# burritojustice/reporter

Measured on AMD Instinct MI355X. Metric: GPS points matched/sec (whole node) at 1/2/4/8 MI355X; % segment-ID agreement vs meili, higher is better.
Workload: dtype f32

## Files before the change

### reporter_amd/csrc/engine.cpp

```cpp
#include "engine.h"

#include "flush.h"

#include <algorithm>
#include <chrono>
#include <cmath>
#include <cstdlib>

#include <cstring>

namespace otm {

#define HIPCHK(x)                                                              \
  do {                                                                         \
    hipError_t e_ = (x);                                                       \
    if (e_ != hipSuccess) {                                                    \
      *err = std::string(#x) + ": " + hipGetErrorString(e_);                   \
      return OTM_EDEVICE;                                                      \
    }                                                                          \
  } while (0)

#define TRY(x)                    \
  do {                            \
    if (int rc_ = (x)) return rc_; \
// ... 374 lines not shown
  HIPCHK(hipMemcpyAsync(cnt.data(), row_cnt, (size_t)N * 4, hipMemcpyDeviceToHost, s));
  HIPCHK(hipStreamSynchronize(s));
  E->graph_allocs.push_back(rows_b.release());
  E->graph_allocs.push_back(slot_b.release());
  E->graph_allocs.push_back(src_b.release());
  for (int32_t c : cnt) {
    out.incomplete += c < 0;
    out.entries += c > 0 ? c : 0;
  }
  out.slots = total;
  out.X.rmax = *r;
  out.X.cmax = index_cost_bound(*r);
  out.X.row = rows;
  out.X.src = src;
  out.src_bytes = (int64_t)E->g.n_edges * (int64_t)sizeof(SrcRec);
  out.X.slot = slot;
  out.X.load_pct = pct;
  return OTM_OK;
}

size_t index_budget() {
  if (const char* bm = std::getenv("OTM_INDEX_BUDGET_MB")) return (size_t)std::strtoull(bm, nullptr, 0) << 20;
  size_t fr = 0, tot = 0;
  if (hipMemGetInfo(&fr, &tot) != hipSuccess) return 0;
  return fr / 2;
}
}

int build_index(otm_engine* E, std::string* err) {
  E->idx = DevIndex{};
  for (auto& x : E->idxn) x = DevIndex{};
  E->idx.rmax = 0.0f;
  if (E->index_rmax < 0.0f) E->index_rmax = auto_index_radius(E);
  E->index_rmax = std::min(E->index_rmax, INDEX_RMAX_CAP);
  if (!(E->index_rmax > 0.0f)) return OTM_OK;
  hipStream_t s = E->stream;
  hipEvent_t a, z;
  HIPCHK(hipEventCreate(&a));
  HIPCHK(hipEventCreate(&z));
  HIPCHK(hipEventRecord(a, s));
  IndexBuilt full;
  TRY(build_index_at(E, &E->index_rmax, true, index_budget(), full, err));
  E->idx = full.X;
  E->index_entries = full.entries;
  E->index_slots = full.slots;
  E->index_src_bytes = full.src_bytes;
  E->index_incomplete_rows = full.incomplete;
  std::vector<float> radii;
  if (E->index_near_set) {
    radii = E->index_near_m;
  } else if ((double)full.slots * IDX_SLOT_BYTES >= OTM_INDEX_NEAR_MIN_GB * 1e9) {
    for (float f : std::initializer_list<float> OTM_INDEX_NEAR_FRACS) radii.push_back(E->index_rmax * f);
  }
  for (float& r : radii) r = (float)(std::floor(r / 50.0) * 50.0);
  std::sort(radii.begin(), radii.end());
  radii.erase(std::unique(radii.begin(), radii.end()), radii.end());
  int nl = 0;
  for (float rn : radii) {
    if (nl == NEAR_LEVELS || !(E->idx.rmax > 0.0f) || rn < 100.0f || rn >= E->idx.rmax) continue;
    IndexBuilt near;
    TRY(build_index_at(E, &rn, false, index_budget(), near, err));
    if (rn > 0.0f) {
      E->index_near_level_entries[nl] = near.entries;
      E->index_near_slots += near.slots;
      E->index_src_bytes += near.src_bytes;
      E->idxn[nl++] = near.X;
    }
  }
  HIPCHK(hipEventRecord(z, s));
  HIPCHK(hipEventSynchronize(z));
  HIPCHK(hipEventElapsedTime(&E->index_build_ms, a, z));
  (void)hipEventDestroy(a);
  (void)hipEventDestroy(z);
  return OTM_OK;
}

void engine_free(otm_engine* E) {
  if (E->device >= 0) (void)hipSetDevice(E->device);
  for (void* p : E->graph_allocs) (void)hipFree(p);
  E->graph_allocs.clear();
  pairs_drop(E);
  if (E->win_counts) (void)hipFree(E->win_counts);
  if (E->win_sums) (void)hipFree(E->win_sums);
  E->win_counts = E->win_sums = nullptr;
  E->win_open = false;
  if (E->sync_ev) (void)hipEventDestroy(E->sync_ev);
  E->sync_ev = nullptr;
  for (hipEvent_t ev : E->req_ev) (void)hipEventDestroy(ev);
  E->req_ev.clear();
  if (E->req_copy) (void)hipStreamDestroy(E->req_copy);
  E->req_copy = nullptr;
  for (auto& e : E->kev) {
    if (e) (void)hipEventDestroy(e);
    e = nullptr;
  }
  if (E->stream) (void)hipStreamDestroy(E->stream);
  E->stream = nullptr;
}

static int max_log2(const char* env, int dflt) {
  const char* v = std::getenv(env);
  return v ? std::min(dflt, std::atoi(v)) : dflt;
}


static int ensure_cand(otm_engine* E, DevWork& w, std::string* err) {
  const size_t n = E->cand_log2 > 0 ? (size_t)CAND_BIG_SLOTS << E->cand_log2 : 0;
  w.cand_final = E->cand_final;
  w.cand_log2 = E->cand_log2;
  TRY(bind_grow(w.cbig_key, E->cbig_key, n, err));
  TRY(bind_grow(w.cbig_val, E->cbig_val, n, err));
  TRY(bind_grow(w.cbig_skey, E->cbig_skey, n / 2, err));
  return OTM_OK;
}

static int ensure_huge(otm_engine* E, DevWork& w, std::string* err) {
  const size_t n = E->huge_log2 > 0 ? (size_t)HUGE_SLOTS << E->huge_log2 : 0;
  w.huge_log2 = E->huge_log2;
  w.huge_final = E->huge_final;
  TRY(bind_grow(w.huge_key, E->huge_key, n, err));
  TRY(bind_grow(w.huge_lab, E->huge_lab, n, err));
  TRY(bind_grow(w.huge_inq, E->huge_inq, n, err));
  TRY(bind_grow(w.huge_fr, E->huge_fr, n * 2, err));
  TRY(bind_grow(w.huge_ins, E->huge_ins, n ? (size_t)HUGE_SLOTS * huge_limit(E->huge_log2) : 0, err));
  TRY(bind_grow(w.huge_prev, E->huge_prev, n ? (size_t)HUGE_SLOTS : 0, err));
  if (n && E->huge_ready_log2 != E->huge_log2) {
    E->huge_ready_log2 = E->huge_log2;
    HIPCHK(hipMemsetAsync(w.huge_key, 0xFF, n * sizeof *w.huge_key, E->stream));
    HIPCHK(hipMemsetAsync(w.huge_lab, 0xFF, n * sizeof *w.huge_lab, E->stream));
    HIPCHK(hipMemsetAsync(w.huge_inq, 0, n * sizeof *w.huge_inq, E->stream));
    HIPCHK(hipMemsetAsync(w.huge_prev, 0xFF, (size_t)HUGE_SLOTS * sizeof *w.huge_prev, E->stream));
  }
  return OTM_OK;
}

static int ensure_big(otm_engine* E, DevWork& w, std::string* err) {
  const size_t n = (size_t)BIG_SLOTS * BIG_TABLE_CAP;
  bool fresh;
  TRY(bind_buf(w.big_key, E->big_key, n, err));
  TRY(bind_buf(w.big_lab, E->big_lab, n, err));
  TRY(bind_buf(w.big_inq, E->big_inq, n, err));
  TRY(bind_buf(w.big_fr, E->big_fr, n * 2, err));
  TRY(bind_buf(w.big_ins, E->big_ins, (size_t)BIG_SLOTS * SEARCH_LIMIT, err));
  TRY(bind_buf(w.big_prev, E->big_prev, (size_t)BIG_SLOTS, err, &fresh));
  if (fresh) {
    HIPCHK(hipMemsetAsync(w.big_key, 0xFF, n * sizeof *w.big_key, E->stream));
    HIPCHK(hipMemsetAsync(w.big_lab, 0xFF, n * sizeof *w.big_lab, E->stream));
    HIPCHK(hipMemsetAsync(w.big_inq, 0, n * sizeof *w.big_inq, E->stream));
    HIPCHK(hipMemsetAsync(w.big_prev, 0, (size_t)BIG_SLOTS * sizeof *w.big_prev, E->stream));
  }
  return OTM_OK;
}

static int bind_point_work(otm_engine* E, int64_t NP, int32_t NT, DevWork& w, std::string* err) {
  const size_t Pn = (size_t)NP + 1;
  TRY(bind_buf(w.pt_trace, E->pt_trace, Pn, err));
  TRY(bind_buf(w.is_col, E->is_col, Pn, err));
  TRY(bind_buf(w.prevc, E->prevc, Pn, err));
  TRY(bind_buf(w.nextc, E->nextc, Pn, err));
  TRY(bind_buf(w.gc, E->gc, Pn, err));
  TRY(bind_buf(w.ncand, E->ncand, Pn, err));
  TRY(bind_buf(w.cand_eo, E->cand_eo, Pn * KIN, err));
  TRY(bind_buf(w.cand_em, E->cand_em, Pn * KIN, err));
  TRY(bind_buf(w.cand_xeo, E->cand_xeo, Pn * KX, err));
  TRY(bind_buf(w.cand_xem, E->cand_xem, Pn * KX, err));
  TRY(bind_buf(w.probe, E->probe, Pn, err));
  TRY(bind_buf(w.col_prev, E->col_prev, Pn, err));
  TRY(bind_buf(w.kq_prev, E->kq_prev, Pn, err));
  TRY(bind_buf(w.vmeta, E->vmeta, Pn, err));
  TRY(bind_buf(w.colrec, E->colrec, Pn, err));
  TRY(bind_buf(w.colrec_pos, E->colrec_pos, Pn, err));
  TRY(bind_buf(w.trans_off, E->trans_off, Pn, err));
  TRY(bind_buf(w.bp, E->bp, Pn * KMAX, err));
  TRY(bind_buf(w.state, E->state, Pn, err));
  TRY(bind_buf(w.chosen, E->chosen, Pn, err));
  TRY(bind_buf(w.chain_start, E->chain_start, Pn, err));
  TRY(bind_buf(w.route_dist, E->route_dist, Pn, err));
  TRY(bind_buf(w.ipos, E->ipos, Pn, err));
  TRY(bind_buf(w.path_off, E->path_off, Pn, err));
  TRY(bind_buf(w.path_len, E->path_len, Pn, err));
  TRY(bind_buf(w.trace_err, E->trace_err, (size_t)NT + 1, err));
  TRY(bind_buf(w.spill_list1, E->spill_list1, Pn, err));
  TRY(bind_buf(w.spill_list2, E->spill_list2, Pn, err));
  TRY(bind_buf(w.spill_list3, E->spill_list3, Pn, err));
  TRY(bind_buf(w.counters_i32, E->counters_i32, CTR_WORDS, err));
  TRY(E->snap.ensure(1, err));
  w.snap = &E->snap.p->stage[0][0];
  TRY(bind_buf(w.abort, E->abort_flag, 4, err));
  if (!E->caps_read) {
    E->caps_read = true;
    if (const char* v = std::getenv("OTM_TRANS_CAP")) E->trans_cap = std::max<int64_t>(1, std::atoll(v)), E->caps_pinned = true;
    if (const char* v = std::getenv("OTM_POOL_CAP")) E->pool_cap = (int32_t)std::max(1, std::atoi(v)), E->caps_pinned = true;
  }
  if (!E->caps_pinned) {
    E->trans_cap = std::max<int64_t>(E->trans_cap, (int64_t)Pn * 48 + 4096);
    E->pool_cap = std::max<int32_t>(E->pool_cap, (int32_t)std::min<size_t>(Pn * 8, (size_t)1 << 30));
  }
  TRY(E->scan_tmp.ensure(scan_tmp_bytes(NP > NT ? NP : NT) + 256, err));
  TRY(bind_buf(w.path_pool, E->path_pool, (size_t)E->pool_cap, err));
  w.pool_cap = E->pool_cap;
  w.idx = E->idx;
  for (int l = 0; l < NEAR_LEVELS; ++l) w.idxn[l] = E->idxn[l];
  return OTM_OK;
}

static int bind_order(otm_engine* E, int64_t NP, bool ordered, DevOrder& ord, std::string* err) {
  const size_t Pn = (size_t)NP + 1;
  TRY(bind_buf(ord.tile, E->ord_tile, Pn, err));
  TRY(bind_buf(ord.tile_cnt, E->ord_cnt, ORDER_TILES, err));
  TRY(bind_buf(ord.cursor, E->ord_cursor, ORDER_TILES, err));
  TRY(bind_buf(ord.grp, E->ord_grp, ORDER_GROUPS + 1, err));
  TRY(bind_buf(ord.item, E->ord_item, Pn, err));
  if (!ordered) ord.tile_cnt = nullptr;
  return OTM_OK;
}

static int bind_trans(otm_engine* E, DevWork& w, hipStream_t s, std::string* err) {
  bool fresh;
  TRY(bind_buf(w.trans, E->trans, (size_t)E->trans_cap + 1, err, &fresh));
  if (fresh) HIPCHK(hipMemsetAsync(E->trans.p, 0, E->trans.bytes(), s));
  w.trans_cap = E->trans_cap;
  return OTM_OK;
}

static size_t out_region_cap(const otm_engine* E, int64_t NP) { return 2 * (size_t)NP + (size_t)E->pool_cap + 1; }

static int bind_out(otm_engine* E, int32_t NT, int64_t NP, DevOut& o, std::string* err) {
  const size_t Tn = (size_t)NT + 1, cap = out_region_cap(E, NP);
  TRY(bind_buf(o.traces, E->o_traces, Tn, err));
  TRY(bind_buf(o.seg_cnt, E->o_seg_cnt, Tn, err));
  TRY(bind_buf(o.way_cnt, E->o_way_cnt, Tn, err));
  TRY(bind_buf(o.seg_base, E->seg_ub, Tn, err));
  TRY(bind_buf(o.segments, E->o_segments, cap, err));
  TRY(bind_buf(o.seg_gidx, E->o_seg_gidx, cap, err));
  TRY(bind_buf(o.reports, E->o_reports, cap, err));
  TRY(bind_buf(o.way_ids, E->o_way_ids, cap, err));
  TRY(bind_buf(o.rep_cnt, E->o_rep_cnt, Tn, err));
  return OTM_OK;
}

static int bind_trav(otm_engine* E, int32_t NT, int64_t NP, DevTrav& tv, std::string* err) {
  TRY(bind_buf(tv.rec, E->tv_rec, out_region_cap(E, NP), err));
  TRY(bind_buf(tv.cnt, E->tv_cnt, (size_t)NT + 1, err));
  return OTM_OK;
}

static int bind_scores(otm_engine* E, int32_t NT, int64_t NP, DevScores& sc, std::string* err) {
  const size_t Pn = (size_t)NP + 1;
  TRY(bind_buf(sc.rec, E->scores.dev, Pn, err));
  TRY(bind_buf(sc.alpha, E->sc_alpha, Pn * KIN, err));
  TRY(bind_buf(sc.alpha_x, E->sc_alpha_x, Pn * KX, err));
  TRY(bind_buf(sc.rej, E->sc_rej, (size_t)NT + 2, err));
  sc.rej_n = sc.rej + NT + 1;
  return OTM_OK;
}

static int engine_match_once(otm_engine* E, const DevBatch& b, hipStream_t s, std::string* err,
                             int from = RESUME_ALL) {
  const int64_t NP = b.n_points;
  const int32_t NT = b.n_traces;
  end_records(E, REC_BATCH_BEGINS);
  DevWork w{};
  TRY(bind_point_work(E, NP, NT, w, err));

  DevParams dp = E->dp;
  if (NP < E->small_points) {
    dp.order_mask = 0;
    dp.cand_wave_all = 1;
  }
  {
    const char* ce = std::getenv("OTM_CAND_CHUNK");
    const int ch = ce ? std::atoi(ce) : 64;
    dp.cand_chunk = ch < 1 ? 1 : (ch > 64 ? 64 : ch);
  }
  w.ctr = E->counting ? E->ctr.p : nullptr;
  if (E->counting && from == RESUME_ALL) HIPCHK(hipMemsetAsync(E->ctr.p, 0, sizeof(DevCounters), s));
  Marks mk;
  mk.ev = E->timing ? E->kev : nullptr;
  TRY(bind_order(E, NP, dp.order_mask != 0, w.ord, err));
  if (from == RESUME_ALL) {
    launch_columns(E->g, b, dp, w, s, mk);
    if (dp.order_mask) {
      launch_order(b, w, s, mk);
    } else if (E->timing) {
      mk.begin(KN_ORDER, s);
      mk.end(KN_ORDER, s);
    }
  }
  TRY(ensure_cand(E, w, err));
  if (from <= RESUME_CAND_BIG) launch_candidates(E->g, b, dp, w, s, mk, from);
  if (from <= RESUME_CAND_BIG) {
    launch_links(b, dp, w, s, mk);
    mk.begin(KN_SCAN_TRANS, s);
    scan_i64(w.trans_off, NP, E->scan_tmp.p, E->scan_tmp.cap(), s);
    mk.end(KN_SCAN_TRANS, s);
  }
  TRY(bind_trans(E, w, s, err));
  TRY(ensure_big(E, w, err));
  TRY(ensure_huge(E, w, err));
  if (from <= RESUME_TRANS_HUGE) launch_transitions(E->g, b, dp, w, s, mk, E->trans_lanes, from);
  if (from <= RESUME_TRANS_HUGE) launch_viterbi(b, w, s, mk);
  launch_route(E->g, b, dp, w, s, mk, from);

  if (out_region_cap(E, NP) >= (size_t)INT32_MAX) {
    *err = "batch too large for one launch (segment regions exceed 2^31)";
    return OTM_EINVAL;
  }
  DevOut o{};
  TRY(bind_out(E, NT, NP, o, err));
  {
    otm_engine* H = E->parent ? const_cast<otm_engine*>(E->parent) : E;
    std::lock_guard<std::mutex> lk(H->hist_mu);
    o.hist = H->hist;
    o.speed_sum = H->speed_sum;
    o.nbins = H->nbins;
    o.bin_kph = H->bin_kph;
    o.pairs = H->pairs_tab;
  }
  HIPCHK(hipMemsetAsync(o.seg_base, 0, ((size_t)NT + 1) * sizeof *o.seg_base, s));
  launch_seg_bound(E->g, b, dp, w, o.seg_base, s, mk);
  mk.begin(KN_SEG_SCAN, s);
  scan_i64(o.seg_base, NT, E->scan_tmp.p, E->scan_tmp.cap(), s);
  mk.end(KN_SEG_SCAN, s);
  launch_segments(E->g, b, w, o, s, mk);
  if (E->queue_kph > 0.0f) launch_queue(b, w, o, E->queue_kph, s);
  end_records(E, REC_BATCH_OUTPUTS);
  if (records_wanted(E, E->points)) {
    TRY(E->points.dev.ensure((size_t)NP + 1, err));
    launch_points(E->g, b, dp, w, E->points.dev.p, s);
    E->points.n = NP;
  }
  if (records_wanted(E, E->scores)) {
    DevScores sc{};
    TRY(bind_scores(E, NT, NP, sc, err));
    launch_scores(b, w, sc, s);
    E->scores.n = NP;
  }
  const bool for_route = records_wanted(E, E->route), for_shape = records_wanted(E, E->shape);
  if (for_route || for_shape) {
    DevTrav tv{};
    TRY(bind_trav(E, NT, NP, tv, err));
    HIPCHK(hipMemsetAsync(tv.cnt + NT, 0, sizeof *tv.cnt, s));
    launch_traversals(E->g, b, w, o, tv, s);
    if (for_route) E->tv_T = NT;
    if (for_shape) E->sh_T = NT;
  }
  launch_report(b, E->drc, w, o, s, mk);
  HIPCHK(hipGetLastError());
  E->last_T = NT;
  E->last_P = NP;
  E->last_S = -1;
  E->last_W = -1;
  return OTM_OK;
}

int engine_match(otm_engine* E, const DevBatch& b, hipStream_t s, std::string* err) {
  if (!s) s = E->stream;
  const int64_t NP = b.n_points;
  struct OomGuard {
    otm_engine* E;
    bool huge = false, cand = false;
    ~OomGuard() {
      if (huge) E->huge_final = 0;
      if (cand) E->cand_final = 0;
    }
  } oom{E};
  struct FailGuard {
    otm_engine* E;
    bool ok = false;
    ~FailGuard() {
      if (!ok) end_records(E, REC_BATCH_FAILED);
    }
  } failed{E};
  int from = RESUME_ALL;
  DevWork grown{};
  E->last_resumes = 0;
  for (int attempt = 0;; ++attempt) {
    TRY(engine_match_once(E, b, s, err, from));
    TRY(E->h_status.ensure(1, err));
    BatchStatus* dst = &E->snap.p->status;
    launch_status(E->abort_flag.p, E->trans_off.p + NP, E->counters_i32.p, dst, s);
    HIPCHK(hipMemcpyAsync(E->h_status.p, dst, sizeof(BatchStatus), hipMemcpyDeviceToHost, s));
    HIPCHK(wait_batch(E, s, NP));
    const BatchStatus st = *E->h_status.p;
    const int32_t ab = st.abort;
    const int64_t ttotal = st.ttotal;
    E->last_trans = ttotal;
    E->last_attempts = attempt + 1;
    if (!ab) break;
    if (attempt == 16) {
      *err = "batch capacities could not be sized";
      return OTM_EDEVICE;
    }
    if (ttotal > E->trans_cap) E->trans_cap = ttotal + ttotal / 4 + 4096;
    if (st.grow & GROW_HUGE) {
      const int32_t next = E->huge_log2 ? E->huge_log2 + 2 : 19;
      const int32_t prev = E->huge_log2;
      if (next > max_log2("OTM_HUGE_MAX_LOG2", HUGE_MAX_LOG2)) {
        E->huge_final = 1;
      } else {
        E->huge_log2 = next;
        if (ensure_huge(E, grown, err) != OTM_OK) {
          E->huge_log2 = prev;
          E->huge_final = 1;
          oom.huge = true;
          E->huge_ready_log2 = 0;
          err->clear();
        }
      }
    }
    if (st.grow & GROW_CAND) {
      const int32_t next = E->cand_log2 ? E->cand_log2 + 2 : 13;
      const int32_t prev = E->cand_log2;
      if (next > max_log2("OTM_CAND_MAX_LOG2", CAND_MAX_LOG2)) {
        E->cand_final = 1;
      } else {
        E->cand_log2 = next;
        if (ensure_cand(E, grown, err) != OTM_OK) {
          E->cand_log2 = prev;
          E->cand_final = 1;
          oom.cand = true;
          err->clear();
        }
      }
    }
    if (st.pool_over)
      E->pool_cap = (int32_t)std::min<size_t>((size_t)st.pool_used * 2 + 1024, (size_t)INT32_MAX / 2);
    const char* nr = std::getenv("OTM_NO_RESUME");
    const bool whole = ttotal > E->trans_cap || st.pool_over || !(st.grow & (GROW_HUGE | GROW_CAND)) ||
                       (nr && *nr && *nr != '0');
    from = whole ? RESUME_ALL
                 : (st.grow & GROW_CAND) ? RESUME_CAND_BIG : (st.route_huge ? RESUME_ROUTE_HUGE : RESUME_TRANS_HUGE);
    if (from != RESUME_ALL) {
      const SnapId snap = from == RESUME_CAND_BIG ? SNAP_AFTER_CAND
                                                  : (from == RESUME_TRANS_HUGE ? SNAP_AFTER_TRANS : SNAP_AFTER_ROUTE);
      int32_t* ctr = E->counters_i32.p;
      HIPCHK(hipMemcpyAsync(ctr, E->snap.p->stage[snap], CTR_STAGE_WORDS * sizeof(int32_t),
                            hipMemcpyDeviceToDevice, s));
      HIPCHK(hipMemsetAsync(ctr + CTR_GROW_HUGE, 0, 4, s));
      HIPCHK(hipMemsetAsync(ctr + CTR_GROW_CAND, 0, 4, s));
      HIPCHK(hipMemsetAsync(E->abort_flag.p, 0, 4, s));
      E->last_resumes += 1;
    }
  }
  if (E->timing) {
    HIPCHK(hipEventSynchronize(E->kev[2 * KN_REPORT + 1]));
    for (int k = 0; k < KN_COUNT; ++k)
      HIPCHK(hipEventElapsedTime(&E->kernel_ms[k], E->kev[2 * k], E->kev[2 * k + 1]));
    const int first[8] = {KN_COLUMNS, KN_ORDER, KN_LINKS, KN_TRANS_INDEX, KN_VITERBI, KN_ROUTE_INDEX, KN_SEG_BOUND,
                          KN_SEG_WRITE};
    const int last[8] = {KN_COLUMNS, KN_CAND_WAVE, KN_SCAN_TRANS, KN_TRANS_GLOBAL, KN_VITERBI, KN_ROUTE_GLOBAL,
                         KN_SEG_SCAN, KN_REPORT};
    for (int k = 0; k < 8; ++k) {
      E->stage_ms[k] = 0.0f;
      for (int q = first[k]; q <= last[k]; ++q) E->stage_ms[k] += E->kernel_ms[q];
    }
  }
  failed.ok = true;
  return OTM_OK;
}

static hipError_t big_copy(void* dst, const void* src, size_t n, hipMemcpyKind k, hipStream_t s) {
  return hipMemcpyAsync(dst, src, n, k, s);
}

static int validate_offsets(int32_t NT, const int64_t* trace_off, int64_t n_points, std::string* err) {
  const int64_t NP = trace_off[NT];
  if (trace_off[0] != 0 || NP < 0 || (n_points && n_points != NP)) {
    *err = "batch trace_off inconsistent with n_points";
    return OTM_EINVAL;
  }
  for (int32_t t = 0; t < NT; ++t)
    if (trace_off[t + 1] < trace_off[t]) {
      *err = "batch trace_off not monotonic";
      return OTM_EINVAL;
    }
  return OTM_OK;
}

int engine_match_host(otm_engine* E, const otm_batch* in, std::string* err) {
  const int32_t NT = in->n_traces;
  if (NT < 0 || !in->trace_off) {
    *err = "invalid batch";
    return OTM_EINVAL;
  }
  TRY(validate_offsets(NT, in->trace_off, in->n_points, err));
  const int64_t NP = in->trace_off[NT];
  DevBatch b;
  b.n_traces = NT;
  b.n_points = NP;
  TRY(bind_buf(b.trace_off, E->in_off, (size_t)NT + 1, err));
  TRY(bind_buf(b.lat, E->in_lat, (size_t)NP, err));
  TRY(bind_buf(b.lon, E->in_lon, (size_t)NP, err));
  TRY(bind_buf(b.time, E->in_time, (size_t)NP, err));
  TRY(bind_buf(b.acc, E->in_acc, (size_t)NP, err));
  hipStream_t s = E->stream;
  const size_t b_off = ((size_t)NT + 1) * 8, b_pt = (size_t)NP * 4, b_tm = (size_t)NP * 8;
  if (NP <= (int64_t)1 << 18) {
    const size_t total = b_off + b_tm + 3 * b_pt;
    TRY(E->h_in.ensure(total, err));
    TRY(E->in_blob.ensure(total, err));
    char* h = E->h_in.p;
    std::memcpy(h, in->trace_off, b_off);
    if (NP) {
      std::memcpy(h + b_off, in->time, b_tm);
      std::memcpy(h + b_off + b_tm, in->lat, b_pt);
      std::memcpy(h + b_off + b_tm + b_pt, in->lon, b_pt);
      std::memcpy(h + b_off + b_tm + 2 * b_pt, in->accuracy, b_pt);
    }
    HIPCHK(hipMemcpyAsync(E->in_blob.p, h, total, hipMemcpyHostToDevice, s));
    const char* d = E->in_blob.p;
    b.trace_off = (const int64_t*)d;
    b.time = (const double*)(d + b_off);
    b.lat = (const float*)(d + b_off + b_tm);
    b.lon = (const float*)(d + b_off + b_tm + b_pt);
    b.acc = (const float*)(d + b_off + b_tm + 2 * b_pt);
    return engine_match(E, b, s, err);
  }
  const hipMemcpyKind h2d = hipMemcpyHostToDevice;
  HIPCHK(hipMemcpyAsync(E->in_off.p, in->trace_off, b_off, hipMemcpyHostToDevice, s));
  HIPCHK(big_copy(E->in_lat.p, in->lat, b_pt, h2d, s));
  HIPCHK(big_copy(E->in_lon.p, in->lon, b_pt, h2d, s));
  HIPCHK(big_copy(E->in_time.p, in->time, b_tm, h2d, s));
  HIPCHK(big_copy(E->in_acc.p, in->accuracy, b_pt, h2d, s));
  return engine_match(E, b, s, err);
}

int validate_compact(const otm_batch_compact* in, int64_t* np, std::string* err) {
  const int32_t NT = in->n_traces;
  if (NT < 0 || !in->trace_off || (NT > 0 && !in->time_base)) {
    *err = "invalid batch";
    return OTM_EINVAL;
  }
  TRY(validate_offsets(NT, in->trace_off, in->n_points, err));
  const int64_t NP = in->trace_off[NT];
// ... 232 lines not shown
  TRY(E->f_traces.ensure((size_t)NT + 1, err));
  if (NT) {
    DevOut o{};
    TRY(bind_out(E, NT, E->last_P, o, err));
    launch_compact(NT, o, so, wo, ro, E->f_segs.p, E->f_ways.p, E->f_reps.p, E->f_traces.p, s);
    HIPCHK(hipGetLastError());
  }
  E->last_S = NS;
  E->last_W = NW;
  *NS_ = NS;
  *NW_ = NW;
  *NR_ = NR;
  return OTM_OK;
}

int engine_fetch(otm_engine* E, otm_results* out, std::string* err) {
  hipStream_t s = E->stream;
  const int32_t NT = E->last_T;
  int32_t NS, NW, NR;
  TRY(fetch_compact(E, &NS, &NW, &NR, err));
  TRY(bind_buf(out->traces, E->h_traces, (size_t)NT + 1, err));
  TRY(bind_buf(out->segments, E->h_segs, (size_t)NS + 1, err));
  TRY(bind_buf(out->reports, E->h_reps_dense, (size_t)NR + 1, err));
  TRY(bind_buf(out->way_ids, E->h_ways, (size_t)NW + 1, err));
  const hipMemcpyKind d2h = hipMemcpyDeviceToHost;
  hipStream_t c = s;
  if (NT) HIPCHK(big_copy(E->h_traces.p, E->f_traces.p, (size_t)NT * sizeof(otm_trace_result), d2h, c));
  if (NS) HIPCHK(big_copy(E->h_segs.p, E->f_segs.p, (size_t)NS * sizeof(otm_segment), d2h, c));
  if (NR) HIPCHK(big_copy(E->h_reps_dense.p, E->f_reps.p, (size_t)NR * sizeof(otm_report_rec), d2h, c));
  if (NW) HIPCHK(big_copy(E->h_ways.p, E->f_ways.p, (size_t)NW * 8, d2h, c));
  HIPCHK(wait_batch(E, c, E->last_P));
  out->n_traces = NT;
  out->n_segments = NS;
  out->n_reports = NR;
  out->n_way_ids = NW;
  return OTM_OK;
}

int engine_write_responses(otm_engine* E, const int64_t** off, const uint8_t** host,
                           const otm_trace_result** traces, int64_t* total, std::string* err) {
  hipStream_t s = E->stream;
  const int32_t NT = E->last_T;
  int32_t NS, NW, NR;
  TRY(fetch_compact(E, &NS, &NW, &NR, err));
  const size_t hdr_b = (size_t)NT * RESP_HDR_SLOT + 64, seg_b = resp_seg_scratch(NS, NW),
               rep_b = (size_t)NR * RESP_REP_SLOT + 64;
  RespWork w{};
  TRY(bind_buf(w.hdr, E->resp_hdr, hdr_b, err));
  TRY(bind_buf(w.seg, E->resp_seg, seg_b, err));
  TRY(bind_buf(w.rep, E->resp_rep, rep_b, err));
  TRY(bind_buf(w.hlen, E->resp_hlen, (size_t)NT + 1, err));
  TRY(bind_buf(w.slen, E->resp_slen, (size_t)NS + 1, err));
  TRY(bind_buf(w.rlen, E->resp_rlen, (size_t)NR + 1, err));
  TRY(bind_buf(w.blen, E->resp_blen, (size_t)NT + 1, err));
  TRY(bind_buf(w.host, E->resp_host, (size_t)NT + 1, err));
  const size_t blob_b = hdr_b + seg_b + rep_b + (size_t)NT * 97 + (size_t)NS + (size_t)NR;
  TRY(E->resp_blob.ensure(blob_b, err));
  TRY(E->scan_tmp.ensure(scan_tmp_bytes(NT) + 256, err));
  const RespIn in{NT, NS, NR, E->f_traces.p, E->f_segs.p, E->f_ways.p, E->f_reps.p};
  if (NT) {
    launch_resp_items(in, w, s);
    launch_resp_len(in, w, s);
    scan_i64(w.blen, NT, E->scan_tmp.p, E->scan_tmp.cap(), s);
    launch_resp_copy(in, w, w.blen, E->resp_blob.p, s);
  }
  const size_t off_b = ((size_t)NT + 1) * 8;
  TRY(E->h_resp_meta.ensure(off_b + (size_t)NT + 8, err));
  TRY(bind_buf(*traces, E->h_traces, (size_t)NT + 1, err));
  char* meta = E->h_resp_meta.p;
  std::memset(meta, 0, off_b);
  if (NT) {
    HIPCHK(hipMemcpyAsync(meta, w.blen, off_b, hipMemcpyDeviceToHost, s));
    HIPCHK(hipMemcpyAsync(meta + off_b, w.host, (size_t)NT, hipMemcpyDeviceToHost, s));
    HIPCHK(big_copy(E->h_traces.p, E->f_traces.p, (size_t)NT * sizeof(otm_trace_result), hipMemcpyDeviceToHost, s));
  }
  HIPCHK(hipGetLastError());
  HIPCHK(wait_batch(E, s, E->last_P));
  *total = ((const int64_t*)meta)[NT];
  *off = (const int64_t*)meta;
  *host = (const uint8_t*)(meta + off_b);
  return OTM_OK;
}

int engine_copy_responses(otm_engine* E, char* dst, int64_t total, const char** blob, std::string* err) {
  if (!dst) {
    TRY(E->h_resp.ensure((size_t)total + 16, err));
    dst = E->h_resp.p;
  }
  if (total) {
    HIPCHK(big_copy(dst, E->resp_blob.p, (size_t)total, hipMemcpyDeviceToHost, E->stream));
    HIPCHK(wait_batch(E, E->stream, E->last_P));
  }
  *blob = dst;
  return OTM_OK;
}

int engine_report_segments(otm_engine* E, int32_t T, const int64_t* trace_off, const double* time,
                           const int32_t* seg_off, const otm_segment* segs, otm_trace_result* traces,
                           otm_report_rec* reports, std::string* err) {
  const int64_t NP = trace_off[T];
  const int32_t NS = seg_off[T];
  for (int32_t t = 0; t < T; ++t)
    if (trace_off[t + 1] <= trace_off[t]) {
      *err = "every trace needs at least one point (its end time)";
      return OTM_EINVAL;
    }
  const size_t b_off = ((size_t)T + 1) * 8, b_sb = ((size_t)T + 1) * 8, b_tm = (size_t)NP * 8;
  const size_t b_seg = ((size_t)NS + 1) * sizeof(otm_segment), b_cnt = ((size_t)T + 1) * 4;
  const size_t b_gidx = ((size_t)NS + 1) * 4, b_err = b_cnt, b_ab = 16;
  const size_t b_tr = ((size_t)T + 1) * sizeof(otm_trace_result), b_rep = ((size_t)NS + 1) * sizeof(otm_report_rec);
  size_t off[12];
  size_t tot = 0;
  const size_t sz[11] = {b_off, b_sb, b_tm, b_seg, b_cnt, b_gidx, b_err, b_ab, b_tr, b_rep, b_cnt};
  for (int k = 0; k < 11; ++k) {
    off[k] = tot;
    tot += (sz[k] + 255) & ~(size_t)255;
  }
  off[11] = tot;
  TRY(E->rs_blob.ensure(tot, err));
  std::vector<char> h(off[8], 0);
  std::memcpy(h.data() + off[0], trace_off, b_off);
  int64_t* sb = (int64_t*)(h.data() + off[1]);
  int32_t* cnt = (int32_t*)(h.data() + off[4]);
  for (int32_t t = 0; t < T; ++t) {
    sb[t] = seg_off[t];
    cnt[t] = seg_off[t + 1] - seg_off[t];
  }
  if (NP) std::memcpy(h.data() + off[2], time, b_tm);
  if (NS) std::memcpy(h.data() + off[3], segs, (size_t)NS * sizeof(otm_segment));
  int32_t* gidx = (int32_t*)(h.data() + off[5]);
  for (int32_t k = 0; k < NS; ++k) gidx[k] = -1;
  hipStream_t s = E->stream;
  char* d = E->rs_blob.p;
  HIPCHK(hipMemcpyAsync(d, h.data(), off[8], hipMemcpyHostToDevice, s));
  DevBatch b{};
  b.n_traces = T;
  b.n_points = NP;
  b.trace_off = (const int64_t*)(d + off[0]);
  b.time = (const double*)(d + off[2]);
  DevWork w{};
  w.trace_err = (int32_t*)(d + off[6]);
  w.abort = (int32_t*)(d + off[7]);
  w.ctr = nullptr;
  DevOut o{};
  o.traces = (otm_trace_result*)(d + off[8]);
  o.seg_cnt = (int32_t*)(d + off[4]);
  o.rep_cnt = (int32_t*)(d + off[10]);
  o.seg_base = (int64_t*)(d + off[1]);
  o.segments = (otm_segment*)(d + off[3]);
  o.seg_gidx = (int32_t*)(d + off[5]);
  o.reports = (otm_report_rec*)(d + off[9]);
  o.hist = nullptr;
  o.speed_sum = nullptr;
  launch_report(b, E->drc, w, o, s, Marks{});
  HIPCHK(hipGetLastError());
  if (T) HIPCHK(hipMemcpyAsync(traces, d + off[8], (size_t)T * sizeof(otm_trace_result), hipMemcpyDeviceToHost, s));
  if (NS) HIPCHK(hipMemcpyAsync(reports, d + off[9], (size_t)NS * sizeof(otm_report_rec), hipMemcpyDeviceToHost, s));
  HIPCHK(hipStreamSynchronize(s));
  return OTM_OK;
}

int engine_debug_fetch(otm_engine* E, int what, void* dst, size_t bytes, size_t* needed, std::string* err) {
  const size_t Pn = (size_t)E->last_P;
  const void* src = nullptr;
  size_t n = 0;
  auto of = [&](const auto& buf, size_t count) {
    src = buf.p;
    n = count * sizeof(*buf.p);
  };
  switch (what) {
    case 0: of(E->ncand, Pn); break;
    case 1:
    case 2:
    case 3: {
      n = Pn * KMAX * 4;
      if (needed) *needed = n;
      if (!dst) return OTM_OK;
      if (bytes < n) {
        *err = "debug buffer too small";
        return OTM_EINVAL;
      }
      if (!n) return OTM_OK;
      const bool rec = what != 3;
      const size_t el = rec ? sizeof(*E->cand_eo.p) : sizeof(*E->cand_em.p);
      std::vector<char> in(Pn * KIN * el), ov(Pn * KX * el);
      const void *din = E->cand_em.p, *dov = E->cand_xem.p;
      if (rec) din = E->cand_eo.p, dov = E->cand_xeo.p;
      HIPCHK(hipMemcpyAsync(in.data(), din, in.size(), hipMemcpyDeviceToHost, E->stream));
      HIPCHK(hipMemcpyAsync(ov.data(), dov, ov.size(), hipMemcpyDeviceToHost, E->stream));
      HIPCHK(hipStreamSynchronize(E->stream));
      int32_t* d = (int32_t*)dst;
      for (size_t p = 0; p < Pn; ++p)
        for (int j = 0; j < KMAX; ++j) {
          const int32_t* src = j < KIN ? (const int32_t*)in.data() + (rec ? 2 : 1) * (p * KIN + j)
                                       : (const int32_t*)ov.data() + (rec ? 2 : 1) * (p * KX + (j - KIN));
          d[p * KMAX + j] = rec ? src[what - 1] : src[0];
        }
      return OTM_OK;
    }
    case 4: of(E->trans_off, Pn + 1); break;
    case 5: of(E->trans, (size_t)E->last_trans); break;
    case 6: of(E->state, Pn); break;
    case 7: of(E->col_prev, Pn); break;
    case 8: of(E->route_dist, Pn); break;
    case 9: of(E->gc, Pn); break;
    case 10: of(E->ipos, Pn); break;
    case 11: of(E->in_off, (size_t)E->last_T + 1); break;
    case 12: of(E->in_lat, Pn); break;
    case 13: of(E->in_lon, Pn); break;
    case 14: of(E->in_time, Pn); break;
    case 15: of(E->in_acc, Pn); break;
    case 16: of(E->chain_start, Pn); break;
    case 17: of(E->is_col, Pn); break;
    case 18: {
      int32_t total = 0;
      if (E->ord_grp.p && E->ord_item.p) {
        HIPCHK(hipMemcpyAsync(&total, E->ord_grp.p + ORDER_GROUPS, 4, hipMemcpyDeviceToHost, E->stream));
        HIPCHK(hipStreamSynchronize(E->stream));
      }
      of(E->ord_item, total < 0 || (size_t)total > Pn ? 0 : (size_t)total);
      break;
    }
    case 19: of(E->ord_tile, E->ord_tile.p ? Pn : 0); break;
    case 20: of(E->ord_grp, E->ord_grp.p ? ORDER_GROUPS + 1 : 0); break;
    default: *err = "unknown debug buffer"; return OTM_EINVAL;
  }
  if (needed) *needed = n;
  if (!dst) return OTM_OK;
  if (bytes < n) {
    *err = "debug buffer too small";
    return OTM_EINVAL;
  }
  if (n) HIPCHK(hipMemcpyAsync(dst, src, n, hipMemcpyDeviceToHost, E->stream));
  HIPCHK(hipStreamSynchronize(E->stream));
  return OTM_OK;
}

template <class Rec>
static void end_if(BatchRecords<Rec>& r, RecEvent event) {
  if (kRecDesc<Rec>.ends & event) r.n = r.joined_n = -1;
}

void end_records(otm_engine* E, RecEvent event) {
  end_if(E->points, event);
  end_if(E->route, event);
  end_if(E->scores, event);
  end_if(E->shape, event);
  if (kRecDesc<otm_traversal>.ends & event) E->tv_T = E->tv_off_T = -1;
  if (kRecDesc<otm_shape_vertex>.ends & event) E->sh_T = -1;
}

template <class Rec>
int engine_fetch_records(otm_engine* E, BatchRecords<Rec>& r, Rec* dst, int64_t cap, int64_t* n, std::string* err) {
  constexpr const RecDesc& d = kRecDesc<Rec>;
  if (!r.on) {
    *err = d.off;
    return OTM_EINVAL;
  }
  if (r.n < 0) {
    *err = d.none;
    return OTM_EINVAL;
  }
  if (n) *n = r.n;
  if (!dst && cap == 0) return OTM_OK;
  if (!dst || cap < r.n) {
    *err = d.cap;
    return OTM_EINVAL;
  }
  const size_t bytes = (size_t)r.n * sizeof(Rec);
  if (!bytes) return OTM_OK;
  TRY(r.pin.ensure((size_t)r.n, err));
  HIPCHK(big_copy(r.pin.p, r.dev.p, bytes, hipMemcpyDeviceToHost, E->stream));
  HIPCHK(wait_batch(E, E->stream, r.n));
  std::memcpy(dst, r.pin.p, bytes);
  return OTM_OK;
}
template int engine_fetch_records(otm_engine*, BatchRecords<otm_matched_point>&, otm_matched_point*, int64_t, int64_t*,
                                  std::string*);
template int engine_fetch_records(otm_engine*, BatchRecords<otm_traversal>&, otm_traversal*, int64_t, int64_t*,
                                  std::string*);
template int engine_fetch_records(otm_engine*, BatchRecords<otm_point_score>&, otm_point_score*, int64_t, int64_t*,
                                  std::string*);

static int trav_offsets(otm_engine* E, int32_t NT, std::string* err, bool wait = true) {
  if (E->tv_off_T == NT) return OTM_OK;
  hipStream_t s = E->stream;
  TRY(E->tv_off.ensure((size_t)NT + 1, err));
  TRY(E->h_tv_off.ensure((size_t)NT + 1, err));
  HIPCHK(hipMemcpyAsync(E->tv_off.p, E->tv_cnt.p, ((size_t)NT + 1) * 8, hipMemcpyDeviceToDevice, s));
  if (NT) scan_i64(E->tv_off.p, NT, E->scan_tmp.p, E->scan_tmp.cap(), s);
  HIPCHK(hipMemcpyAsync(E->h_tv_off.p, E->tv_off.p, ((size_t)NT + 1) * 8, hipMemcpyDeviceToHost, s));
  if (!wait) return OTM_OK;
  HIPCHK(wait_batch(E, s, E->last_P));
  E->tv_off_T = NT;
  return OTM_OK;
}

int engine_traversals_dense(otm_engine* E, std::string* err) {
  if (!E->route.on) {
    *err = kRecDesc<otm_traversal>.off;
    return OTM_EINVAL;
  }
  if (E->tv_T < 0) {
    *err = kRecDesc<otm_traversal>.none;
    return OTM_EINVAL;
  }
  if (E->route.n >= 0) return OTM_OK;
// ... 678 lines not shown
```

### reporter_amd/csrc/kernels.h

```cpp
#pragma once
#include <hip/hip_runtime.h>

#include <cstddef>
#include <cstdint>

#include "otmatch.h"
#include "pairs.h"

namespace otm {

constexpr int KMAX = 32;
constexpr int KIN = 8;
static_assert(KIN == 4 || KIN == 8, "inline blocks of 4 or 8 slots (whole 16-B emission pieces)");
constexpr int KX = KMAX - KIN;
constexpr int MAX_HITS = 256;
constexpr int SEARCH_LIMIT = 98304;
constexpr int LDS_TABLE_CAP = 256;
constexpr int LDS_TABLE_LIMIT = 192;
constexpr int BIG_TABLE_LOG2 = 17;
constexpr int BIG_TABLE_CAP = 1 << BIG_TABLE_LOG2;
#ifndef OTM_BIG_SLOTS
#define OTM_BIG_SLOTS 512
#endif
constexpr int BIG_SLOTS = OTM_BIG_SLOTS;
// ... 10 lines not shown
  const int32_t* e_shape_off;
  const int64_t* e_way;
  const int32_t *e_seg, *e_seg_pos;
  const uint8_t* e_flags;
  const float *s_lat, *s_lon, *s_cum;
  const uint64_t* g_id;
  const float* g_len;
  const uint32_t* cell_off;
  const uint32_t* cell_ent;
  const float4* ent_geo;
  const uint16_t *e_head_out, *e_head_in;
  const uint32_t* e_len64;
  const uint4* e_rec;
  const int2* e_fl;
  const int4* e_proj;
  const float4* s_pt;
  const int64_t* way_tab;
  int32_t n_nodes, n_edges, n_segments, grid_rows, grid_cols;
  double lat0, lon0, cell;
  float bb_lat0, bb_lon0, bb_inv_h, bb_inv_w;
};

#ifndef OTM_ORDER_BITS
#define OTM_ORDER_BITS 6
#endif
constexpr int ORDER_BITS = OTM_ORDER_BITS;
constexpr int ORDER_SIDE = 1 << ORDER_BITS;
constexpr int ORDER_TILES = ORDER_SIDE * ORDER_SIDE;
constexpr int ORDER_GROUPS = 8;
struct DevOrder {
  int32_t* item;
  int32_t* grp;
  uint16_t* tile;
  int32_t* tile_cnt;
  int32_t* cursor;
};

struct IdxRow {
  int64_t off;
  int32_t cnt;
  uint32_t cap;
};
#ifndef OTM_SRC_REC_BYTES
#define OTM_SRC_REC_BYTES 48
#endif
struct alignas(16) SrcRec {
  IdxRow edge;
  IdxRow node;
  int32_t from;
  int32_t len;
  int32_t pad[(OTM_SRC_REC_BYTES - 40) / 4];
};
static_assert(sizeof(SrcRec) == OTM_SRC_REC_BYTES && (OTM_SRC_REC_BYTES == 48 || OTM_SRC_REC_BYTES == 64),
              "source records of 48 or 64 bytes");
struct DevIndex {
  float rmax;
  uint32_t cmax;
  const IdxRow* row;
  const SrcRec* src;
  const uint4* slot;
  int load_pct;
};
constexpr int IDX_SLOT_BYTES = 16;
constexpr float INDEX_RMAX_CAP = 200000.0f;
constexpr uint32_t NODE_KEY = 0x80000000u;
constexpr uint32_t NONE_PRED = 0xFFFFFFFFu;
constexpr int NEAR_LEVELS = 3;
#ifndef OTM_INDEX_NEAR_FRACS
#define OTM_INDEX_NEAR_FRACS {0.45f}
#endif
#ifndef OTM_INDEX_NEAR_MIN_GB
#define OTM_INDEX_NEAR_MIN_GB 16.0
#endif
constexpr int INDEX_BUILD_LOG2 = 11;
constexpr int INDEX_BUILD_CAP = 1 << INDEX_BUILD_LOG2;
constexpr int INDEX_BUILD_LIMIT = 1536;
__host__ __device__ inline uint32_t index_cost_bound(float B) { return (uint32_t)floor((double)B * 64.0); }

constexpr int ORDER_CAND = 1, ORDER_TRANS = 2, ORDER_ROUTE = 4;
constexpr int TURN_TABLE = 181;
constexpr uint32_t TURN_UNITS_MAX = 0xFFFFFFu;
constexpr uint32_t NO_TURNS = 0xFFFFFFFFu;
struct DevParams {
  float sigma_z, beta, factor, breakage, interp, search_radius, max_search_radius, gps_accuracy;
  const uint32_t* turn_units;
  int max_candidates;
  int order_mask;
  int cand_wave_all;
  int cand_chunk;
};

struct DevReportCfg {
  int n_report, n_transition;
  int64_t report_levels[16];
  int64_t transition_levels[16];
  double threshold_sec;
};

struct DevBatch {
  int32_t n_traces;
  int64_t n_points;
  const int64_t* trace_off;
  const float *lat, *lon;
  const double* time;
  const float* acc;
};

struct DevCounters {
  unsigned long long points, columns, cells_visited, cell_entries_scanned, candidates;
  unsigned long long searches, nodes_settled, edges_relaxed, transitions;
  unsigned long long route_searches, route_nodes_settled, route_edges_relaxed, route_edges;
  unsigned long long segments_out, reports_out;
};

enum CtrSlot : int {
  CTR_UNUSED = 0,
  CTR_POOL_USED = 1,
  CTR_POOL_OVER = 2,
  CTR_SEARCH_GLOBAL = 3,
  CTR_INDEX_MISS = 4,
  CTR_CAND_WAVE = 5,
  CTR_TRANS_WIDE = 6,
  CTR_SEG_LARGE = 8,
  CTR_VIT_16 = 20,
  CTR_TRANS_HUGE = 21,
  CTR_ROUTE_HUGE = 22,
  CTR_GROW_HUGE = 23,
  CTR_CAND_BIG = 24,
  CTR_GROW_CAND = 25,
  CTR_VIT_WAVE = 26,
};
constexpr int CTR_STAGE_WORDS = 16;
constexpr int CTR_ZEROED_WORDS = 32;
constexpr int CTR_WORDS = 64;
enum SnapId : int { SNAP_AFTER_CAND = 0, SNAP_AFTER_TRANS = 1, SNAP_AFTER_ROUTE = 2, SNAP_COUNT = 3 };
constexpr int ctr_list(CtrSlot c) {
  switch (c) {
    case CTR_INDEX_MISS: case CTR_CAND_WAVE: case CTR_SEG_LARGE: case CTR_VIT_16: return 1;
    case CTR_SEARCH_GLOBAL: case CTR_TRANS_WIDE: case CTR_VIT_WAVE: return 2;
    case CTR_TRANS_HUGE: case CTR_ROUTE_HUGE: case CTR_CAND_BIG: return 3;
    default: return 0;
  }
}
constexpr bool ctr_per_stage(CtrSlot c) { return c >= 0 && c < CTR_STAGE_WORDS; }
constexpr bool ctr_per_batch(CtrSlot c) { return c >= CTR_STAGE_WORDS && c < CTR_ZEROED_WORDS; }
static_assert(ctr_per_stage(CTR_UNUSED) && ctr_per_stage(CTR_POOL_USED) && ctr_per_stage(CTR_POOL_OVER) &&
                  ctr_per_stage(CTR_SEARCH_GLOBAL) && ctr_per_stage(CTR_INDEX_MISS) && ctr_per_stage(CTR_CAND_WAVE) &&
                  ctr_per_stage(CTR_TRANS_WIDE) && ctr_per_stage(CTR_SEG_LARGE),
              "per-stage slots lie in the snapshot range");
static_assert(ctr_per_batch(CTR_VIT_16) && ctr_per_batch(CTR_TRANS_HUGE) && ctr_per_batch(CTR_ROUTE_HUGE) &&
                  ctr_per_batch(CTR_GROW_HUGE) && ctr_per_batch(CTR_CAND_BIG) && ctr_per_batch(CTR_GROW_CAND) &&
                  ctr_per_batch(CTR_VIT_WAVE),
              "per-batch slots lie past the snapshot range, within what K1 zeroes");

struct DevWork {
  int32_t* pt_trace;
  uint8_t* is_col;
  int32_t* prevc;
  int32_t* nextc;
  float* gc;
  int32_t* ncand;
  float4* probe;
  int2* cand_eo;
  float* cand_em;
  int2* cand_xeo;
  float* cand_xem;
  int32_t* col_prev;
  int32_t* kq_prev;
  uint8_t* vmeta;
  int64_t* trans_off;
  float* trans;
  uint8_t* bp;
  int32_t* state;
  int2* chosen;
  uint8_t* chain_start;
  float* route_dist;
  float* ipos;
  int32_t* path_off;
  int32_t* path_len;
  int32_t* path_pool;
  int32_t pool_cap;
  int32_t* trace_err;
  int32_t* spill_list1;
  int32_t* spill_list2;
  int32_t* snap;
  int32_t* counters_i32;
  int32_t* abort;
  int64_t trans_cap;
  int4* colrec;
  int32_t* colrec_pos;
  DevIndex idx;
  DevIndex idxn[NEAR_LEVELS];
  DevOrder ord;
  uint32_t* big_key;
  unsigned long long* big_lab;
  uint32_t* big_inq;
  uint32_t* big_fr;
  uint32_t* big_ins;
  int32_t* big_prev;
  uint32_t* huge_key;
  unsigned long long* huge_lab;
  uint32_t* huge_inq;
  uint32_t* huge_fr;
  uint32_t* huge_ins;
  int32_t* huge_prev;
  int32_t huge_log2;
  int32_t huge_final;
  uint32_t* cbig_key;
  unsigned long long* cbig_val;
  unsigned long long* cbig_skey;
  int32_t cand_log2;
  int32_t cand_final;
  int32_t* spill_list3;
  DevCounters* ctr;
};
struct SpillRef {
  int32_t* list;
  int32_t* count;
};
template <CtrSlot C>
__host__ __device__ __forceinline__ int32_t* spill_list(const DevWork& w) {
  constexpr int L = ctr_list(C);
  static_assert(L != 0, "this slot counts no list");
  return L == 1 ? w.spill_list1 : (L == 2 ? w.spill_list2 : w.spill_list3);
}
template <CtrSlot C>
__host__ __device__ __forceinline__ SpillRef spill_of(const DevWork& w) {
  return SpillRef{spill_list<C>(w), w.counters_i32 + C};
}

struct DevOut {
  otm_trace_result* traces;
  int32_t* seg_cnt;
  int32_t* way_cnt;
  int32_t* rep_cnt;
  int64_t* seg_base;
  otm_segment* segments;
  int32_t* seg_gidx;
  int64_t* way_ids;
  otm_report_rec* reports;
  uint32_t* hist;
  unsigned long long* speed_sum;
  int nbins;
  float bin_kph;
  PairTab pairs;
};

struct DevTrav {
  otm_traversal* rec;
  int64_t* cnt;
};

struct DevShape {
  const int64_t* trav_off;
  int64_t* vtx_off;
  int64_t* poly_off;
  otm_shape_vertex* vtx;
  otm_shape_span* span;
  char* poly;
};

enum KernelId {
  KN_COLUMNS,
  KN_ORDER,
  KN_CAND_LANE,
  KN_CAND_WAVE,
  KN_LINKS,
  KN_SCAN_TRANS,
  KN_TRANS_INDEX,
  KN_TRANS_WIDE,
  KN_TRANS_WAVE,
  KN_TRANS_GLOBAL,
  KN_VITERBI,
  KN_ROUTE_INDEX,
  KN_ROUTE_WAVE,
  KN_ROUTE_GLOBAL,
  KN_SEG_BOUND,
  KN_SEG_SCAN,
  KN_SEG_WRITE,
  KN_REPORT,
  KN_COUNT
};
extern const char* const kKernelNames[KN_COUNT];
struct Marks {
  hipEvent_t* ev = nullptr;
  void begin(int k, hipStream_t s) const {
    if (ev) (void)hipEventRecord(ev[2 * k], s);
  }
  void end(int k, hipStream_t s) const {
    if (ev) (void)hipEventRecord(ev[2 * k + 1], s);
  }
};

void launch_columns(const DevGraph& g, const DevBatch& b, const DevParams& p, DevWork& w, hipStream_t s,
                    const Marks& mk);
enum Resume { RESUME_ALL = 0, RESUME_CAND_BIG = 1, RESUME_TRANS_HUGE = 2, RESUME_ROUTE_HUGE = 3 };
void launch_candidates(const DevGraph& g, const DevBatch& b, const DevParams& p, DevWork& w, hipStream_t s,
                       const Marks& mk, int from = RESUME_ALL);
void launch_links(const DevBatch& b, const DevParams& p, DevWork& w, hipStream_t s, const Marks& mk);
void launch_transitions(const DevGraph& g, const DevBatch& b, const DevParams& p, DevWork& w, hipStream_t s,
                        const Marks& mk, int sub, int from = RESUME_ALL);
void launch_viterbi(const DevBatch& b, DevWork& w, hipStream_t s, const Marks& mk);
void launch_route(const DevGraph& g, const DevBatch& b, const DevParams& p, DevWork& w, hipStream_t s,
                  const Marks& mk, int from = RESUME_ALL);
void launch_segments(const DevGraph& g, const DevBatch& b, DevWork& w, DevOut& o, hipStream_t s, const Marks& mk);
void launch_queue(const DevBatch& b, DevWork& w, DevOut& o, float kph, hipStream_t s);
void launch_points(const DevGraph& g, const DevBatch& b, const DevParams& p, DevWork& w, otm_matched_point* out,
                   hipStream_t s);
void launch_traversals(const DevGraph& g, const DevBatch& b, DevWork& w, DevOut& o, const DevTrav& tv, hipStream_t s);
void launch_trav_compact(int32_t n_traces, const int64_t* seg_base, const int64_t* off, const otm_traversal* reg,
                         otm_traversal* dst, hipStream_t s);
struct DevScores {
  otm_point_score* rec;
  float* alpha;
  float* alpha_x;
  int32_t* rej;
  int32_t* rej_n;
};
void launch_scores(const DevBatch& b, DevWork& w, const DevScores& sc, hipStream_t s);
void launch_shape(const DevGraph& g, int32_t n_traces, const int64_t* seg_base, const DevTrav& tv, const DevShape& sh,
                  bool write, hipStream_t s);
void launch_report(const DevBatch& b, const DevReportCfg& rc, DevWork& w, DevOut& o, hipStream_t s, const Marks& mk);
void launch_order(const DevBatch& b, DevWork& w, hipStream_t s, const Marks& mk);
void launch_seg_bound(const DevGraph& g, const DevBatch& b, const DevParams& p, DevWork& w, int64_t* tb, hipStream_t s,
                      const Marks& mk);
void launch_compact(int32_t n_traces, const DevOut& o, const int32_t* seg_off, const int32_t* way_off,
                    const int32_t* rep_off, otm_segment* segs_out, int64_t* ways_out, otm_report_rec* reps_out,
                    otm_trace_result* traces_out,
                    hipStream_t s);
void launch_index_build(const DevGraph& g, const uint32_t* turn_units, uint32_t cmax, int32_t* row_cnt,
                        const IdxRow* rows, uint4* slot, bool write, hipStream_t s);
int index_load_fast();
int index_load_dense();
void launch_row_sizes(const int32_t* row_cnt, int64_t* row_sizes, int32_t n, int pct, hipStream_t s);
constexpr int32_t GROW_HUGE = 1, GROW_CAND = 2;
struct BatchStatus {
  int32_t abort, grow;
  int64_t ttotal;
  int32_t pool_used, pool_over;
  int32_t route_huge;
};
struct SnapBuf {
  int32_t stage[SNAP_COUNT][CTR_STAGE_WORDS];
  BatchStatus status;
};
static_assert(offsetof(SnapBuf, status) == 192 && sizeof(SnapBuf) == 192 + 32, "snapshot buffer layout");
void launch_expand_compact(const int64_t* trace_off, const int64_t* tbase, const int32_t* dt, const int16_t* acc16,
                           double* time, float* acc, int32_t n_traces, hipStream_t s);
void launch_status(const int32_t* abort, const int64_t* ttotal, const int32_t* counters, BatchStatus* out,
                   hipStream_t s);
void launch_row_pack(const int32_t* row_cnt, const int64_t* row_off, IdxRow* rows, int32_t n, hipStream_t s);
void launch_src_pack(const DevGraph& g, const IdxRow* rows, SrcRec* src, hipStream_t s);
size_t req_sparse_slots(int32_t n, size_t bytes);
void launch_req_read(const unsigned char* blob, const int64_t* off, int32_t r0, int32_t r1, int32_t n, int64_t* cnt,
                     uint8_t* ok, const DevBatch& sparse, hipStream_t s);
void launch_req_compact(const int64_t* off, int32_t n, const int64_t* pre, const uint8_t* ok, const DevBatch& sparse,
                        const DevBatch& out, int64_t* trace_off, hipStream_t s);
constexpr int RESP_HDR_SLOT = 512;
constexpr int RESP_SEG_SLOT = 320;
constexpr int RESP_REP_SLOT = 192;
struct RespIn {
  int32_t nt, ns, nr;
  const otm_trace_result* traces;
  const otm_segment* segs;
  const int64_t* ways;
  const otm_report_rec* reps;
};
struct RespWork {
  char *hdr, *seg, *rep;
  int32_t *hlen, *slen, *rlen;
  int64_t* blen;
  uint8_t* host;
};
size_t resp_seg_scratch(int32_t ns, int32_t nw);
void launch_resp_items(const RespIn& in, const RespWork& w, hipStream_t s);
void launch_resp_len(const RespIn& in, const RespWork& w, hipStream_t s);
void launch_resp_copy(const RespIn& in, const RespWork& w, const int64_t* boff, char* blob, hipStream_t s);
void scan_i64(int64_t* d, int64_t n, void* tmp, size_t tmp_bytes, hipStream_t s);
constexpr int FETCH_SCAN_MAX = 1 << 16;
void launch_fetch_scan(int32_t n, const int32_t* c0, const int32_t* c1, const int32_t* c2, int32_t* o0, int32_t* o1,
                       int32_t* o2, hipStream_t s);
void scan_i32(int32_t* d, int64_t n, void* tmp, size_t tmp_bytes, hipStream_t s);
size_t scan_tmp_bytes(int64_t n);

}
```

### reporter_amd/csrc/kernels.hip

```cpp
#include <hip/hip_runtime.h>

#include <algorithm>
#include <cstdlib>
#include <type_traits>

#include <hipcub/hipcub.hpp>

#include "kernels.h"
#include "otmatch.h"

namespace otm {

namespace {

#define MPD_F 111319.4954833f
constexpr uint32_t EMPTY = 0xFFFFFFFFu;
constexpr unsigned long long LAB_NONE = ~0ull;
constexpr int TB = 64;
__device__ __forceinline__ void wave_sync() {
  __builtin_amdgcn_wave_barrier();
  asm volatile("" ::: "memory");
}

__device__ __forceinline__ float cos_deg(float deg) {
// ... 127 lines not shown
  bool at_end;
  project(g, e, k, lat, lon, ls, sqd, off_out, at_end);
}
__device__ __forceinline__ float probe_radius(const DevParams& P, float acc) {
  const float a = acc > 0.0f ? acc : P.gps_accuracy;
  const float r = a > P.search_radius ? a : P.search_radius;
  return r < P.max_search_radius ? r : P.max_search_radius;
}

__device__ __forceinline__ uint32_t fbits(float f) { return __float_as_uint(f); }
__device__ __forceinline__ float bitsf(uint32_t u) { return __uint_as_float(u); }
__device__ __forceinline__ uint32_t hash32(uint32_t x) { return x * 2654435761u; }

__device__ __forceinline__ void cadd(unsigned long long* c, unsigned long long v) {
  if (c && v) atomicAdd(c, v);
}

__device__ __forceinline__ int2 crec(const DevWork& w, int64_t p, int j) {
  return j < KIN ? w.cand_eo[p * KIN + j] : w.cand_xeo[p * KX + (j - KIN)];
}
__device__ __forceinline__ float cemis(const DevWork& w, int64_t p, int j) {
  return j < KIN ? w.cand_em[p * KIN + j] : w.cand_xem[p * KX + (j - KIN)];
}
__device__ __forceinline__ void cput(const DevWork& w, int64_t p, int j, int32_t e, float off, float em) {
  if (j < KIN) {
    w.cand_eo[p * KIN + j] = make_int2(e, __float_as_int(off));
    w.cand_em[p * KIN + j] = em;
  } else {
    w.cand_xeo[p * KX + (j - KIN)] = make_int2(e, __float_as_int(off));
    w.cand_xem[p * KX + (j - KIN)] = em;
  }
}

__device__ __forceinline__ uint32_t turn_deg(uint32_t hin, uint32_t hout) {
  int d = (int)hout - (int)hin;
  d += d < 0 ? 360 : 0;
  return (uint32_t)(d <= 180 ? d : 360 - d);
}
__device__ __forceinline__ float trans_cost(uint32_t units, float r, float gcv, float beta) {
  units = units > TURN_UNITS_MAX ? TURN_UNITS_MAX : units;
  const float tc = (float)units * 0.015625f;
  const float diff = fabsf(r - gcv);
  return (tc + diff) / beta;
}

constexpr uint32_t NO_HEAD = 0xFFFFu;
__device__ __forceinline__ bool cand_node(float off) { return off == 0.0f; }
__device__ __forceinline__ int32_t src_node(const DevGraph& g, int32_t e, float off) {
  return cand_node(off) ? g.e_from[e] : g.e_to[e];
}
__device__ __forceinline__ float src_start(const DevGraph& g, int32_t e, float off) {
  return cand_node(off) ? 0.0f : g.e_len[e] - off;
}
__device__ __forceinline__ uint32_t src_head(const DevGraph& g, int32_t e, float off) {
  return cand_node(off) ? NO_HEAD : (uint32_t)g.e_head_in[e];
}
__device__ __forceinline__ uint32_t dst_head(const DevGraph& g, int32_t e, float off) {
  return cand_node(off) ? NO_HEAD : (uint32_t)g.e_head_out[e];
}
__device__ __forceinline__ bool same_edge_step(int32_t ei, float oi, int32_t ej, float oj) {
  return ei == ej && (oj >= oi || (!cand_node(oj) && !cand_node(oi)));
}
__device__ __forceinline__ float same_edge_dist(float oi, float oj) { return oj >= oi ? oj - oi : 0.0f; }
__device__ __forceinline__ uint32_t turn_units(const uint32_t* TU, uint32_t hin, uint32_t hout) {
  return (hin == NO_HEAD || hout == NO_HEAD) ? 0u : TU[turn_deg(hin, hout)];
}

__device__ __forceinline__ int wave_incl_scan(int v, int lane) {
#pragma unroll
  for (int o = 1; o < 64; o <<= 1) {
    int n = __shfl_up(v, o, 64);
    if (lane >= o) v += n;
  }
  return v;
}

__device__ __forceinline__ void fold_snap(DevWork& w, int k, bool reset) {
  for (int t = 0; t < CTR_STAGE_WORDS; ++t) {
    w.snap[CTR_STAGE_WORDS * k + t] = w.counters_i32[t];
    if (reset) w.counters_i32[t] = 0;
  }
}
template <CtrSlot C>
__device__ __forceinline__ void spill_push(const DevWork& w, int32_t p) {
  const SpillRef s = spill_of<C>(w);
  s.list[atomicAdd(s.count, 1)] = p;
}
__device__ __forceinline__ bool trans_over_cap(const DevBatch& b, const DevWork& w) {
  if (w.trans_off[b.n_points] <= w.trans_cap) return false;
  *w.abort = 1;
  return true;
}

__device__ __forceinline__ int hilbert_d(int x, int y) {
  int d = 0;
  for (int sft = ORDER_SIDE / 2; sft > 0; sft >>= 1) {
    const int rx = (x & sft) > 0;
    const int ry = (y & sft) > 0;
    d += sft * sft * ((3 * rx) ^ ry);
    if (ry == 0) {
      if (rx == 1) {
        x = ORDER_SIDE - 1 - x;
        y = ORDER_SIDE - 1 - y;
      }
      const int tmp = x;
      x = y;
      y = tmp;
    }
  }
  return d;
}

__device__ __forceinline__ int tile_of(const DevGraph& g, float lat, float lon) {
  int ty = (int)((lat - g.bb_lat0) * g.bb_inv_h);
  int tx = (int)((lon - g.bb_lon0) * g.bb_inv_w);
  ty = ty < 0 ? 0 : (ty >= ORDER_SIDE ? ORDER_SIDE - 1 : ty);
  tx = tx < 0 ? 0 : (tx >= ORDER_SIDE ? ORDER_SIDE - 1 : tx);
  return hilbert_d(tx, ty);
}

struct AggMatch {
  int leader;
  int rank;
  int count;
};
__device__ __forceinline__ AggMatch agg_match(int key, bool active) {
  const int lane = threadIdx.x & 63;
  unsigned long long pending = __ballot(active);
  AggMatch m{lane, 0, 0};
  while (pending) {
    const int leader = __ffsll((long long)pending) - 1;
    const int k = __shfl(key, leader, 64);
    const unsigned long long grp = __ballot(((pending >> lane) & 1ull) && key == k);
    if ((grp >> lane) & 1ull) {
      m.leader = leader;
      m.rank = (int)__popcll(grp & ((1ull << lane) - 1ull));
      m.count = (int)__popcll(grp);
    }
    pending &= ~grp;
  }
  return m;
}
__device__ __forceinline__ int wave_agg_slot(int32_t* ctr, int key, bool active) {
  const AggMatch m = agg_match(key, active);
  int base = 0;
  if (active && m.leader == (int)(threadIdx.x & 63)) base = atomicAdd(&ctr[key], m.count);
  return __shfl(base, m.leader, 64) + m.rank;
}
__device__ __forceinline__ void wave_agg_count(int32_t* ctr, int key, bool active) {
  const AggMatch m = agg_match(key, active);
  if (active && m.leader == (int)(threadIdx.x & 63)) atomicAdd(&ctr[key], m.count);
}

__global__ __launch_bounds__(1024) void k_order_plan(const int32_t* tile_cnt, int32_t* cursor, int32_t* grp) {
  __shared__ int32_t part[1024];
  __shared__ int32_t cut[ORDER_GROUPS + 1];
  constexpr int PER = ORDER_TILES / 1024;
  const int tid = threadIdx.x;
  int32_t v[PER], sum = 0;
  for (int k = 0; k < PER; ++k) {
    v[k] = tile_cnt[tid * PER + k];
    sum += v[k];
  }
  part[tid] = sum;
  if (tid <= ORDER_GROUPS) cut[tid] = 0x7fffffff;
  __syncthreads();
  for (int o = 1; o < 1024; o <<= 1) {
    const int32_t x = tid >= o ? part[tid - o] : 0;
    __syncthreads();
    part[tid] += x;
    __syncthreads();
  }
  const int32_t total = part[1023];
  int32_t run = part[tid] - sum;
  int32_t prev_start = tid == 0 ? -1 : run - tile_cnt[tid * PER - 1];
  for (int k = 0; k < PER; ++k) {
    cursor[tid * PER + k] = run;
    for (int gi = 1; gi < ORDER_GROUPS; ++gi) {
      const int64_t want = ((int64_t)total * gi + ORDER_GROUPS - 1) / ORDER_GROUPS;
      if (run >= want && prev_start < want) cut[gi] = run;
    }
    prev_start = run;
    run += v[k];
  }
  __syncthreads();
  if (tid == 0) {
    grp[0] = 0;
    int32_t prev = 0;
    for (int gi = 1; gi < ORDER_GROUPS; ++gi) {
      const int32_t c = cut[gi] > total ? total : cut[gi];
      prev = c > prev ? c : prev;
      grp[gi] = prev;
    }
    grp[ORDER_GROUPS] = total;
  }
}

__global__ __launch_bounds__(256) void k_order_scatter(DevBatch b, DevWork w, const uint16_t* tile, int32_t* cursor,
                                                       int32_t* item) {
  for (int64_t p0 = (int64_t)blockIdx.x * 256; p0 < b.n_points; p0 += (int64_t)gridDim.x * 256) {
    const int64_t p = p0 + threadIdx.x;
    const bool col = p < b.n_points && w.is_col[p];
    const int t = col ? (int)tile[p] : 0;
    const int pos = wave_agg_slot(cursor, t, col);
    if (col) item[pos] = (int32_t)p;
    if (col && w.colrec_pos) w.colrec_pos[p] = pos;
  }
}

#ifndef OTM_COL_PTS
#define OTM_COL_PTS 256
#endif
constexpr int COL_PTS = OTM_COL_PTS;
__global__ __launch_bounds__(TB) void k_columns(DevGraph g, DevBatch b, DevParams P, DevWork w) {
  __shared__ float sLat[COL_PTS], sLon[COL_PTS], sGc[COL_PTS];
  __shared__ int32_t sPrev[COL_PTS];
  __shared__ uint8_t sCol[COL_PTS];
  const int lane = threadIdx.x;
  if (blockIdx.x == 0) {
    if (lane < CTR_ZEROED_WORDS) w.counters_i32[lane] = 0;
    if (lane == 0) *w.abort = 0;
  }
  for (int32_t t = blockIdx.x; t < b.n_traces; t += gridDim.x) {
    const int64_t a = b.trace_off[t], e = b.trace_off[t + 1];
    const int n = (int)(e - a);
    int ncols = 0;
    if (n > COL_PTS) {
      if (lane == 0) {
        int64_t last = -1;
        for (int64_t p = a; p < e; ++p) {
          float gcv = 0.0f;
          if (last >= 0) gcv = gc_dist(b.lat[last], b.lon[last], b.lat[p], b.lon[p]);
          const bool col = last < 0 || gcv >= P.interp;
          w.is_col[p] = col ? 1 : 0;
          w.gc[p] = col ? gcv : 0.0f;
          w.prevc[p] = (int32_t)last;
          if (col) {
            last = p;
            ++ncols;
            if (w.ord.tile_cnt) {
              const int tl = tile_of(g, b.lat[p], b.lon[p]);
              w.ord.tile[p] = (uint16_t)tl;
              atomicAdd(&w.ord.tile_cnt[tl], 1);
            }
          }
        }
      }
      for (int64_t p = a + lane; p < e; p += TB) {
        w.probe[p] = make_float4(b.lat[p], b.lon[p], b.acc[p], 0.0f);
        w.pt_trace[p] = t;
        w.ncand[p] = 0;
        w.route_dist[p] = 0.0f;
        w.ipos[p] = -1.0f;
        w.nextc[p] = -1;
      }
    } else {
      for (int pl = lane; pl < n; pl += TB) {
        sLat[pl] = b.lat[a + pl];
        sLon[pl] = b.lon[a + pl];
      }
      __syncthreads();
      bool near = false;
      for (int pl = lane; pl < n; pl += TB) {
        const float d = pl > 0 ? gc_dist(sLat[pl - 1], sLon[pl - 1], sLat[pl], sLon[pl]) : 0.0f;
        sGc[pl] = d;
        near = near || (pl > 0 && !(d >= P.interp));
      }
      __syncthreads();
      if (__ballot(near) == 0ull) {
        for (int pl = lane; pl < n; pl += TB) {
          sCol[pl] = 1;
          sPrev[pl] = pl > 0 ? (int32_t)(a + pl - 1) : -1;
        }
        ncols = n;
      } else if (lane == 0) {
        int last = -1;
        for (int pl = 0; pl < n; ++pl) {
          float gcv = 0.0f;
          if (last >= 0) gcv = last == pl - 1 ? sGc[pl] : gc_dist(sLat[last], sLon[last], sLat[pl], sLon[pl]);
          const bool col = last < 0 || gcv >= P.interp;
          sCol[pl] = col ? 1 : 0;
          sGc[pl] = col ? gcv : 0.0f;
          sPrev[pl] = last >= 0 ? (int32_t)(a + last) : -1;
          if (col) {
            last = pl;
            ++ncols;
          }
        }
      }
      __syncthreads();
      for (int c0 = 0; c0 < n; c0 += TB) {
        const int pl = c0 + lane;
        const bool in = pl < n;
        const bool col = in && sCol[pl];
        if (in) {
          const int64_t p = a + pl;
          w.probe[p] = make_float4(sLat[pl], sLon[pl], b.acc[p], 0.0f);
          w.pt_trace[p] = t;
          w.is_col[p] = sCol[pl];
          w.gc[p] = sGc[pl];
          w.prevc[p] = sPrev[pl];
          w.ncand[p] = 0;
          w.route_dist[p] = 0.0f;
          w.ipos[p] = -1.0f;
          w.nextc[p] = -1;
        }
        if (w.ord.tile_cnt) {
          const int tl = col ? tile_of(g, sLat[pl], sLon[pl]) : 0;
          if (col) w.ord.tile[a + pl] = (uint16_t)tl;
          wave_agg_count(w.ord.tile_cnt, tl, col);
        }
      }
      __syncthreads();
    }
    if (lane == 0) {
      w.trace_err[t] = 0;
      if (w.ctr) {
        cadd(&w.ctr->points, (unsigned long long)n);
        cadd(&w.ctr->columns, (unsigned long long)ncols);
      }
    }
  }
}

struct ItemRange {
  int64_t i0, i1, stride;
  bool ordered;
};
__device__ __forceinline__ ItemRange item_range(const DevWork& w, const DevBatch& b, bool ordered, int per_block) {
  ItemRange r;
  r.ordered = ordered;
  const int tid = per_block > 1 ? (int)threadIdx.x : 0;
  if (ordered) {
    const int grp = blockIdx.x % ORDER_GROUPS;
    r.i0 = w.ord.grp[grp] + (int64_t)(blockIdx.x / ORDER_GROUPS) * per_block + tid;
    r.i1 = w.ord.grp[grp + 1];
    r.stride = (int64_t)(gridDim.x / ORDER_GROUPS) * per_block;
  } else {
    r.i0 = (int64_t)blockIdx.x * per_block + tid;
    r.i1 = b.n_points;
    r.stride = (int64_t)gridDim.x * per_block;
  }
  return r;
}

constexpr int HCAP = 512;
constexpr uint32_t NODE_ENT = 0x80000000u;
#ifndef OTM_CAND_LANE_CAP
#define OTM_CAND_LANE_CAP 8
#endif
constexpr int CAND_LANE_CAP = OTM_CAND_LANE_CAP;
#ifndef OTM_CAND_TB
#define OTM_CAND_TB 256
#endif
#ifndef OTM_CAND_WAVES
#define OTM_CAND_WAVES 8
#endif
constexpr int CAND_TB = OTM_CAND_TB;
#ifndef OTM_CAND_INFL
#define OTM_CAND_INFL 2
#endif
constexpr int CAND_INFL = OTM_CAND_INFL;
#ifndef OTM_SNAP_B
#define OTM_SNAP_B 2
#endif
constexpr int SNAP_B = OTM_SNAP_B;
__device__ __forceinline__ void wave_cadd(unsigned long long* c, unsigned long long v) {
  for (int o = 32; o > 0; o >>= 1) v += __shfl_xor(v, o, 64);
  if ((threadIdx.x & 63) == 0 && v) atomicAdd(c, v);
}

template <bool CTR>
__global__ __launch_bounds__(CAND_TB, OTM_CAND_WAVES) void k_cand_lane(DevGraph g, DevBatch b, DevParams P, DevWork w) {
  __shared__ uint32_t sE[CAND_LANE_CAP * CAND_TB];
  __shared__ float sQ[CAND_LANE_CAP * CAND_TB];
  uint32_t* E = sE + threadIdx.x;
  float* Q = sQ + threadIdx.x;
  static_assert(CAND_LANE_CAP <= 8 && CAND_LANE_CAP % SNAP_B == 0, "3-bit slots; whole snap steps");
  constexpr int S = CAND_TB;
  unsigned long long c_cells = 0, c_ent = 0, c_cand = 0;
  const ItemRange R = item_range(w, b, (P.order_mask & ORDER_CAND) != 0, CAND_TB);
  for (int64_t it = R.i0; it < R.i1; it += R.stride) {
    const int64_t p = R.ordered ? (int64_t)w.ord.item[it] : it;
    if (!R.ordered && !w.is_col[p]) continue;
    if (P.cand_wave_all) {
      spill_push<CTR_CAND_WAVE>(w, (int32_t)p);
      continue;
    }
    const float4 pr = w.probe[p];
    const float lat = pr.x, lon = pr.y;
    const float r = probe_radius(P, pr.z);
    const float r2 = r * r;
    const float ls = MPD_F * cos_deg(lat);
    const float dlat = r / MPD_F;
    const float dlon = r / ls;
    const double la_lo = ((double)lat - (double)dlat - g.lat0) / g.cell;
    const double la_hi = ((double)lat + (double)dlat - g.lat0) / g.cell;
    const double lo_lo = ((double)lon - (double)dlon - g.lon0) / g.cell;
    const double lo_hi = ((double)lon + (double)dlon - g.lon0) / g.cell;
    const double R = g.grid_rows, Cn = g.grid_cols;
    int r0 = 0, r1 = -1, c0 = 0, c1 = -1;
    if (!(la_hi < 0.0 || lo_hi < 0.0 || la_lo >= R || lo_lo >= Cn)) {
      r0 = la_lo < 0.0 ? 0 : (int)floor(la_lo);
      r1 = la_hi >= R ? (int)R - 1 : (int)floor(la_hi);
      c0 = lo_lo < 0.0 ? 0 : (int)floor(lo_lo);
      c1 = lo_hi >= Cn ? (int)Cn - 1 : (int)floor(lo_hi);
    }
    int n = 0;
    bool spill = false;
    const unsigned long long cells = (unsigned long long)(r1 - r0 + 1) * (unsigned long long)(c1 - c0 + 1);
    unsigned long long ents = 0;
    auto insert = [&](uint32_t ent, float sqd) {
      const uint32_t e = ent >> 4;
      uint32_t ev[CAND_LANE_CAP];
#pragma unroll
      for (int m = 0; m < CAND_LANE_CAP; ++m) ev[m] = E[m * S];
      int f = -1;
#pragma unroll
      for (int m = 0; m < CAND_LANE_CAP; ++m) f = (m < n && (ev[m] >> 4) == e) ? m : f;
      if (f < 0) {
        if (n == CAND_LANE_CAP) {
          spill = true;
          return;
        }
        E[n * S] = ent;
        Q[n * S] = sqd;
        ++n;
      } else {
        const float qf = Q[f * S];
        if (sqd < qf || (sqd == qf && (ent & 15u) < (E[f * S] & 15u))) {
          Q[f * S] = sqd;
          E[f * S] = ent;
        }
      }
    };
    const float2_t pll = {lat, lon}, psc = {MPD_F, ls};
    const uint32_t W = (((uint32_t)P.cand_chunk - 1u) & 63u) + 1u;
    for (int rg = r0; rg <= r1 && !spill; rg += 3) {
      uint32_t qa[3], qb[3];
#pragma unroll
      for (int j = 0; j < 3; ++j) {
        const size_t rbase = (size_t)(rg + j <= r1 ? rg + j : r1) * (size_t)g.grid_cols;
        qa[j] = g.cell_off[rbase + c0];
        qb[j] = g.cell_off[rbase + c1 + 1];
      }
      const uint32_t e1 = qb[0] - qa[0];
      const uint32_t e2 = e1 + (rg + 1 <= r1 ? qb[1] - qa[1] : 0u);
      const uint32_t tot = e2 + (rg + 2 <= r1 ? qb[2] - qa[2] : 0u);
      const uint32_t b2 = qa[2] - e2, d1 = qa[1] - e1 - b2, d0 = qa[0] - (qa[1] - e1);
      if (CTR) ents += (unsigned long long)tot;
      auto entry_of = [&](uint32_t i) { return (size_t)(uint32_t)(i + b2 + (i < e2 ? d1 : 0u) + (i < e1 ? d0 : 0u)); };
      for (uint32_t done = 0, cn; done < tot && !spill; done += cn) {
        cn = tot - done < W ? tot - done : W;
        unsigned long long hit = 0ull;
        for (uint32_t k = 0; k < cn; k += CAND_INFL) {
          float4 G[CAND_INFL];
#pragma unroll
          for (int u = 0; u < CAND_INFL; ++u) G[u] = g.ent_geo[entry_of(done + k + (u == 0 || k + u < cn ? u : 0))];
          __builtin_amdgcn_sched_barrier(0);
          uint32_t bits = 0u;
#pragma unroll
          for (int u = 0; u < CAND_INFL; ++u) {
            const float sq = seg_sqdist_pk(G[u], pll, psc);
            bits |= ((uint32_t)(u == 0 || k + u < cn) & (uint32_t)(sq <= r2)) << u;
          }
          hit |= (unsigned long long)bits << k;
        }
        while (hit != 0ull && !spill) {
          const size_t qx = entry_of(done + (uint32_t)(__ffsll(hit) - 1));
// ... 133 lines not shown
    }
  }
  if (CTR) {
    wave_cadd(&w.ctr->cells_visited, c_cells);
    wave_cadd(&w.ctr->cell_entries_scanned, c_ent);
    wave_cadd(&w.ctr->candidates, c_cand);
  }
}

template <bool BIG>
struct Mem;
template <>
struct Mem<false> {
  template <class T>
  __device__ static T ld(const T* p) {
    return *p;
  }
  template <class T>
  __device__ static void st(T* p, T v) {
    *p = v;
  }
};
template <>
struct Mem<true> {
  template <class T>
  __device__ static T ld(const T* p) {
    return __hip_atomic_load(p, __ATOMIC_RELAXED, __HIP_MEMORY_SCOPE_AGENT);
  }
  template <class T>
  __device__ static void st(T* p, T v) {
    __hip_atomic_store(p, v, __ATOMIC_RELAXED, __HIP_MEMORY_SCOPE_AGENT);
  }
};

template <bool BIG>
__global__ __launch_bounds__(TB) void k_candidates(DevGraph g, DevBatch b, DevParams P, DevWork w) {
  __shared__ uint32_t l_hkey[BIG ? 1 : HCAP];
  __shared__ unsigned long long l_hval[BIG ? 1 : HCAP];
  __shared__ unsigned long long l_skey[BIG ? 1 : MAX_HITS];
  __shared__ int64_t cstart[64];
  __shared__ int cexcl[64];
  __shared__ int s_count, s_over, s_n;
  const int lane = threadIdx.x;
  const SpillRef work = BIG ? spill_of<CTR_CAND_BIG>(w) : spill_of<CTR_CAND_WAVE>(w);
  const int64_t nwork = *work.count;
  const int32_t* list = work.list;
  if (BIG && nwork > 0 && w.cand_log2 == 0) {
    for (int64_t it = (int64_t)blockIdx.x * TB + lane; it < nwork; it += (int64_t)gridDim.x * TB) {
      w.ncand[list[it]] = 0;
      if (w.cand_final) atomicCAS(&w.trace_err[w.pt_trace[list[it]]], 0, OTM_TERR_CAND_OVERFLOW);
    }
    if (!w.cand_final && blockIdx.x == 0 && lane == 0) {
      w.counters_i32[CTR_GROW_CAND] = 1;
      *w.abort = 1;
    }
    return;
  }
  const int hlog2 = BIG ? w.cand_log2 : 9;
  const int hcap = 1 << hlog2;
  const int max_hits = hcap / 2;
  uint32_t* hkey = BIG ? w.cbig_key + (size_t)blockIdx.x * hcap : l_hkey;
  unsigned long long* hval = BIG ? w.cbig_val + (size_t)blockIdx.x * hcap : l_hval;
  unsigned long long* skey = BIG ? w.cbig_skey + (size_t)blockIdx.x * max_hits : l_skey;
  for (int64_t it = blockIdx.x; it < nwork; it += gridDim.x) {
    const int64_t p = list[it];
    const float4 pr = w.probe[p];
    const float lat = pr.x, lon = pr.y;
    const float r = probe_radius(P, pr.z);
    const float r2 = r * r;
    const float ls = MPD_F * cos_deg(lat);
    const float dlat = r / MPD_F;
    const float dlon = r / ls;
    const double la_lo = ((double)lat - (double)dlat - g.lat0) / g.cell;
    const double la_hi = ((double)lat + (double)dlat - g.lat0) / g.cell;
    const double lo_lo = ((double)lon - (double)dlon - g.lon0) / g.cell;
    const double lo_hi = ((double)lon + (double)dlon - g.lon0) / g.cell;
    const double R = g.grid_rows, Cn = g.grid_cols;
    int r0 = 0, r1 = -1, c0 = 0, c1 = -1;
    if (!(la_hi < 0.0 || lo_hi < 0.0 || la_lo >= R || lo_lo >= Cn)) {
      r0 = la_lo < 0.0 ? 0 : (int)floor(la_lo);
      r1 = la_hi >= R ? (int)R - 1 : (int)floor(la_hi);
      c0 = lo_lo < 0.0 ? 0 : (int)floor(lo_lo);
      c1 = lo_hi >= Cn ? (int)Cn - 1 : (int)floor(lo_hi);
    }
    const int ncols = c1 - c0 + 1;
    const int ncells = (r1 - r0 + 1) * ncols;
    for (int i = lane; i < hcap; i += TB) {
      Mem<BIG>::st(&hkey[i], (uint32_t)EMPTY);
      Mem<BIG>::st(&hval[i], (unsigned long long)LAB_NONE);
    }
    if (lane == 0) {
      s_count = 0;
      s_over = 0;
      s_n = 0;
    }
    __syncthreads();
    unsigned long long scanned = 0;
    for (int cb = 0; cb < ncells; cb += TB) {
      const int c = cb + lane;
      int cnt = 0;
      int64_t cs = 0;
      if (c < ncells) {
        const int rr = r0 + c / ncols, cc = c0 + c % ncols;
        const size_t cidx = (size_t)rr * (size_t)g.grid_cols + (size_t)cc;
        cs = g.cell_off[cidx];
        cnt = (int)(g.cell_off[cidx + 1] - cs);
      }
      const int incl = wave_incl_scan(cnt, lane);
      const int total = __shfl(incl, 63, 64);
      cexcl[lane] = incl - cnt;
      cstart[lane] = cs;
      __syncthreads();
      const int nc_here = min(TB, ncells - cb);
      for (int gi = lane; gi < total; gi += TB) {
        int lo = 0, hi = nc_here - 1;
        while (lo < hi) {
          const int mid = (lo + hi + 1) >> 1;
          if (cexcl[mid] <= gi) lo = mid;
          else hi = mid - 1;
        }
        const int64_t q = cstart[lo] + (gi - cexcl[lo]);
        const uint32_t ent = g.cell_ent[q];
        const float4 G = g.ent_geo[q];
        const int32_t e = (int32_t)(ent >> 4), k = (int32_t)(ent & 15u);
        const float sqd = seg_sqdist(G.x, G.y, G.z, G.w, lat, lon, ls);
        if (!(sqd <= r2)) continue;
        uint32_t slot = hash32((uint32_t)e) >> (32 - hlog2);
        bool placed = false;
        for (int probe = 0; probe < hcap; ++probe) {
          const uint32_t old = atomicCAS(&hkey[slot], EMPTY, (uint32_t)e);
          if (old == EMPTY) {
            if (atomicAdd(&s_count, 1) >= max_hits) s_over = 1;
            placed = true;
            break;
          }
          if (old == (uint32_t)e) {
            placed = true;
            break;
          }
          slot = (slot + 1) & (uint32_t)(hcap - 1);
        }
        if (!placed) {
          s_over = 1;
          continue;
        }
        atomicMin(&hval[slot], ((unsigned long long)fbits(sqd) << 32) | (unsigned long long)k);
      }
      scanned += (unsigned long long)total;
      __syncthreads();
    }
    if (s_over) {
      if (lane == 0) {
        if (!BIG) {
          spill_push<CTR_CAND_BIG>(w, (int32_t)p);
        } else if (w.cand_final) {
          w.ncand[p] = 0;
          atomicCAS(&w.trace_err[w.pt_trace[p]], 0, OTM_TERR_CAND_OVERFLOW);
        } else {
          w.ncand[p] = 0;
          w.counters_i32[CTR_GROW_CAND] = 1;
          *w.abort = 1;
        }
      }
      __syncthreads();
      continue;
    }
    for (int i = lane; i < hcap; i += TB) {
      const uint32_t hk = Mem<BIG>::ld(&hkey[i]);
      if (hk != EMPTY) {
        const unsigned long long hv = Mem<BIG>::ld(&hval[i]);
        const int idx = atomicAdd(&s_n, 1);
        Mem<BIG>::st(&skey[idx],
                     (hv & 0xFFFFFFFF00000000ull) | ((unsigned long long)hk << 5) | ((hv & 15ull) << 1));
      }
    }
    __syncthreads();
    for (int i = lane; i < hcap; i += TB) {
      Mem<BIG>::st(&hkey[i], (uint32_t)EMPTY);
      Mem<BIG>::st(&hval[i], (unsigned long long)LAB_NONE);
    }
    if (lane == 0) s_count = 0;
    __syncthreads();
    const int n0 = s_n;
    for (int idx = lane; idx < n0; idx += TB) {
      const unsigned long long key = Mem<BIG>::ld(&skey[idx]);
      const int32_t e = (int32_t)(((uint32_t)key) >> 5);
      float sqd, off;
      bool at_end;
      const ProjIn pin = proj_load(g, e, (int32_t)((key >> 1) & 15ull));
      proj_calc(pin, lat, lon, ls, sqd, off, at_end);
      const int32_t v = snap_rep(pin, off, at_end);
      if (v < 0) {
        Mem<BIG>::st(&skey[idx], key | 1ull);
        atomicAdd(&s_count, 1);
      } else {
        Mem<BIG>::st(&skey[idx], (unsigned long long)LAB_NONE);
        const uint32_t rep = (uint32_t)v;
        uint32_t slot = hash32(rep) >> (32 - hlog2);
        while (true) {
          const uint32_t old = atomicCAS(&hkey[slot], EMPTY, rep);
          if (old == EMPTY || old == rep) break;
          slot = (slot + 1) & (uint32_t)(hcap - 1);
        }
        atomicMin(&hval[slot], (key & 0xFFFFFFFF00000000ull) | (unsigned long long)idx);
      }
    }
    __syncthreads();
    for (int i = lane; i < hcap; i += TB) {
      const uint32_t hk = Mem<BIG>::ld(&hkey[i]);
      if (hk != EMPTY) {
        const unsigned long long hv = Mem<BIG>::ld(&hval[i]);
        Mem<BIG>::st(&skey[(int)(hv & 0xFFFFFFFFull)], (hv & 0xFFFFFFFF00000000ull) | ((unsigned long long)hk << 5));
        atomicAdd(&s_count, 1);
      }
    }
    __syncthreads();
    const int ns = n0;
    const int n = s_count;
    int N = 1;
    while (N < ns) N <<= 1;
    for (int i = ns + lane; i < N; i += TB) Mem<BIG>::st(&skey[i], (unsigned long long)LAB_NONE);
    __syncthreads();
    for (int kk = 2; kk <= N; kk <<= 1) {
      for (int j = kk >> 1; j > 0; j >>= 1) {
        for (int i = lane; i < N; i += TB) {
          const int ixj = i ^ j;
          if (ixj > i) {
            const unsigned long long x = Mem<BIG>::ld(&skey[i]), y = Mem<BIG>::ld(&skey[ixj]);
            const bool up = (i & kk) == 0;
            if ((x > y) == up) {
              Mem<BIG>::st(&skey[i], y);
              Mem<BIG>::st(&skey[ixj], x);
            }
          }
        }
        __syncthreads();
      }
    }
    const int K = n < P.max_candidates ? n : P.max_candidates;
    if (lane < K) {
      const unsigned long long key = Mem<BIG>::ld(&skey[lane]);
      const int32_t e = (int32_t)(((uint32_t)key) >> 5);
      float sqd = bitsf((uint32_t)(key >> 32)), off = 0.0f;
      if (key & 1ull) project(g, e, (int32_t)((key >> 1) & 15ull), lat, lon, ls, sqd, off);
      const float ds = (2.0f * P.sigma_z) * P.sigma_z;
      cput(w, p, lane, e, off, sqd / ds);
    } else if (lane < KIN) {
      cput(w, p, lane, -1, 0.0f, INFINITY);
    }
    if (lane == 0) {
      w.ncand[p] = K;
      if (w.ctr) {
        cadd(&w.ctr->cells_visited, (unsigned long long)ncells);
        cadd(&w.ctr->cell_entries_scanned, scanned);
        cadd(&w.ctr->candidates, (unsigned long long)K);
      }
    }
    __syncthreads();
  }
}

__global__ __launch_bounds__(256) void k_links(DevBatch b, DevParams P, DevWork w) {
  const int64_t p = (int64_t)blockIdx.x * blockDim.x + threadIdx.x;
  if (p > b.n_points) return;
  if (p == b.n_points) {
    w.trans_off[p] = 0;
    fold_snap(w, SNAP_AFTER_CAND, true);
    return;
  }
  int32_t cp = -1, kq = 0;
  int64_t cnt = 0;
  if (w.is_col[p]) {
    const int32_t q = w.prevc[p];
    if (q >= 0 && p - q > 1) w.nextc[q] = (int32_t)p;
    if (q >= 0 && w.ncand[p] > 0 && w.ncand[q] > 0 && w.gc[p] <= P.breakage) {
      cp = q;
      kq = w.ncand[q];
      cnt = (int64_t)kq * (int64_t)w.ncand[p];
    }
  }
  w.col_prev[p] = cp;
  w.kq_prev[p] = kq;
  w.trans_off[p] = cnt;
  if (w.colrec && (P.order_mask & ORDER_TRANS) && w.is_col[p])
    w.colrec[w.colrec_pos[p]] = make_int4((int32_t)p, cp, kq | (w.ncand[p] << 8), __float_as_int(w.gc[p]));
  w.vmeta[p] = (uint8_t)((w.is_col[p] ? (w.ncand[p] | 0x40) : 0) | (cp >= 0 ? 0x80 : 0));
}

__global__ void k_status(const int32_t* abort, const int64_t* ttotal, const int32_t* counters, BatchStatus* out) {
  if (threadIdx.x == 0) {
    out->abort = *abort;
    out->grow = (counters[CTR_GROW_HUGE] != 0 ? GROW_HUGE : 0) | (counters[CTR_GROW_CAND] != 0 ? GROW_CAND : 0);
    out->ttotal = *ttotal;
    out->pool_used = counters[CTR_POOL_USED];
    out->pool_over = counters[CTR_POOL_OVER];
    out->route_huge = counters[CTR_ROUTE_HUGE];
  }
}

struct Table {
  uint32_t* key;
  unsigned long long* lab;
  uint32_t* inq;
  uint32_t* fr0;
  uint32_t* fr1;
  int cap_log2;
  int limit;
  uint32_t* ins = nullptr;
  int32_t* prev = nullptr;
};

struct SearchShared {
  int nfr, nnext, count, over;
};

template <bool BIG>
__device__ __forceinline__ int table_find(const Table& T, uint32_t v) {
  const uint32_t mask = (1u << T.cap_log2) - 1u;
  uint32_t slot = hash32(v) >> (32 - T.cap_log2);
  for (int i = 0; i <= (int)mask; ++i) {
    const uint32_t k = Mem<BIG>::ld(&T.key[slot]);
    if (k == v) return (int)slot;
    if (k == EMPTY) return -1;
    slot = (slot + 1) & mask;
  }
  return -1;
}

template <bool BIG>
__device__ __forceinline__ void ta_relax(const Table& T, SearchShared& S, uint32_t* nxt, uint32_t key,
                                         unsigned long long nl) {
  const uint32_t mask = (1u << T.cap_log2) - 1u;
  uint32_t slot = hash32(key) >> (32 - T.cap_log2);
  int found = -1;
  for (int i = 0; i <= (int)mask; ++i) {
    const uint32_t old = atomicCAS(&T.key[slot], EMPTY, key);
    if (old == EMPTY) {
      const int c = atomicAdd(&S.count, 1);
      if (c >= T.limit) S.over = 1;
      else if (BIG) Mem<true>::st(&T.ins[c], slot);
      found = (int)slot;
      break;
    }
    if (old == key) {
      found = (int)slot;
      break;
    }
    slot = (slot + 1) & mask;
  }
  if (found < 0) {
    S.over = 1;
    return;
  }
  const unsigned long long old = atomicMin(&T.lab[found], nl);
  if (!(key & NODE_KEY) && nl < old && (uint32_t)(old >> 32) != (uint32_t)(nl >> 32)) {
    if (atomicExch(&T.inq[found], 1u) == 0u) {
      const int idx = atomicAdd(&S.nnext, 1);
      Mem<BIG>::st(&nxt[idx], (uint32_t)found);
    }
  }
}

template <bool BIG>
__device__ int ta_search(const DevGraph& g, const uint32_t* TU, const Table& T, SearchShared& S, int32_t u,
                         uint32_t hin, uint32_t cmax, int lane) {
  const int cap = 1 << T.cap_log2;
  const int pc = BIG ? Mem<true>::ld(T.prev) : -1;
  if (pc < 0) {
    for (int i = lane; i < cap; i += TB) {
      Mem<BIG>::st(&T.key[i], EMPTY);
      Mem<BIG>::st(&T.lab[i], LAB_NONE);
      Mem<BIG>::st(&T.inq[i], 0u);
    }
  } else {
    for (int i = lane; i < pc; i += TB) {
      const uint32_t sl = Mem<true>::ld(&T.ins[i]);
      Mem<BIG>::st(&T.key[sl], EMPTY);
      Mem<BIG>::st(&T.lab[sl], LAB_NONE);
      Mem<BIG>::st(&T.inq[sl], 0u);
    }
  }
  if (lane == 0) {
    S.nfr = 0;
    S.nnext = 0;
    S.count = 0;
    S.over = 0;
  }
  __syncthreads();
  uint32_t* cur = T.fr0;
  uint32_t* nxt = T.fr1;
  if (lane == 0) ta_relax<BIG>(T, S, nxt, NODE_KEY | (uint32_t)u, (unsigned long long)NONE_PRED);
  const int32_t e0 = g.out_off[u], e1 = g.out_off[u + 1];
  for (int32_t e = e0 + lane; e < e1; e += TB) {
    const uint32_t c = turn_units(TU, hin, g.e_head_out[e]);
    if (c <= cmax) ta_relax<BIG>(T, S, nxt, (uint32_t)e, ((unsigned long long)c << 32) | NONE_PRED);
  }
  __syncthreads();
  while (true) {
    if (lane == 0) {
      S.nfr = S.nnext;
      S.nnext = 0;
    }
    uint32_t* tmp = cur;
    cur = nxt;
    nxt = tmp;
    __syncthreads();
    const int nfr = S.nfr;
    if (nfr == 0 || S.over) break;
    for (int f = lane; f < nfr; f += TB) {
      const uint32_t sl = Mem<BIG>::ld(&cur[f]);
      if (BIG) atomicExch(&T.inq[sl], 0u);
      else T.inq[sl] = 0u;
      const int32_t e = (int32_t)Mem<BIG>::ld(&T.key[sl]);
      const unsigned long long ca =
          (unsigned long long)(uint32_t)(Mem<BIG>::ld(&T.lab[sl]) >> 32) + (unsigned long long)g.e_len64[e];
      if (ca > cmax) continue;
      const int32_t v = g.e_to[e];
      ta_relax<BIG>(T, S, nxt, NODE_KEY | (uint32_t)v, (ca << 32) | (uint32_t)e);
      const uint32_t hv = g.e_head_in[e];
      for (int32_t h = g.out_off[v]; h < g.out_off[v + 1]; ++h) {
        const unsigned long long c = ca + turn_units(TU, hv, g.e_head_out[h]);
        if (c <= cmax) ta_relax<BIG>(T, S, nxt, (uint32_t)h, (c << 32) | (uint32_t)e);
      }
    }
    __syncthreads();
  }
  const bool over = S.over != 0;
  const int count = S.count;
  if (BIG && lane == 0) Mem<true>::st(T.prev, over || count > T.limit ? -1 : count);
  __syncthreads();
  return over ? -1 : count;
}

template <bool BIG>
__device__ void ta_counts(const DevGraph& g, const Table& T, uint32_t cmax, int lane, unsigned long long& settled,
                          unsigned long long& relaxed) {
  unsigned long long st = 0, rl = 0;
  const int cap = 1 << T.cap_log2;
  for (int i = lane; i < cap; i += TB) {
    const uint32_t k = Mem<BIG>::ld(&T.key[i]);
    if (k == EMPTY || (k & NODE_KEY)) continue;
    ++st;
    const unsigned long long ca = (Mem<BIG>::ld(&T.lab[i]) >> 32) + (unsigned long long)g.e_len64[k];
    if (ca <= cmax) rl += (unsigned long long)(g.out_off[g.e_to[k] + 1] - g.out_off[g.e_to[k]]);
  }
  for (int o = 32; o > 0; o >>= 1) {
    st += __shfl_xor(st, o, 64);
    rl += __shfl_xor(rl, o, 64);
  }
  settled = st;
// ... 414 lines not shown
      cadd(&w.ctr->searches, c_search);
      cadd(&w.ctr->nodes_settled, c_settled);
      cadd(&w.ctr->edges_relaxed, c_relaxed);
      cadd(&w.ctr->transitions, c_trans);
    }
  }
}

#ifndef OTM_ROUTE_WAVES
#define OTM_ROUTE_WAVES 1
#endif
__global__ __launch_bounds__(256, OTM_ROUTE_WAVES) void k_route_index(DevGraph g, DevBatch b, DevParams P, DevWork w) {
  if (*w.abort) return;
  const DevIndex& X = w.idx;
  unsigned long long c_search = 0, c_settled = 0, c_relaxed = 0, c_edges = 0;
  const ItemRange R = item_range(w, b, (P.order_mask & ORDER_ROUTE) != 0, 256);
  const bool rec = R.ordered && w.colrec && (P.order_mask & ORDER_TRANS);
  for (int64_t it = R.i0; it < R.i1; it += R.stride) {
    int64_t p;
    int32_t q = -1;
    float gcv = 0.0f;
    if (rec) {
      const int4 A = w.colrec[it];
      p = A.x;
      q = A.y;
      gcv = __int_as_float(A.w);
    } else {
      p = R.ordered ? (int64_t)w.ord.item[it] : it;
    }
    if (!R.ordered && !w.is_col[p]) continue;
    w.route_dist[p] = 0.0f;
    w.path_len[p] = 0;
    w.path_off[p] = 0;
    const int2 cq0 = w.chosen[q >= 0 ? q : p];
    if (w.state[p] < 0 || w.chain_start[p]) continue;
    if (!rec) {
      q = w.col_prev[p];
      gcv = w.gc[p];
    }
    const int2 ci = rec ? cq0 : w.chosen[q], cj = w.chosen[p];
    const int32_t ei = ci.x, ej = cj.x;
    const float oi = __int_as_float(ci.y), oj = __int_as_float(cj.y);
    if (same_edge_step(ei, oi, ej, oj)) {
      w.route_dist[p] = same_edge_dist(oi, oj);
      continue;
    }
    const float bound = P.factor * gcv;
    const uint32_t cq = index_cost_bound(bound);
    IdxRow Rw{};
    int64_t sv = -1;
    uint4 lab{};
    int lvl = -1;
#pragma unroll
    for (int l = NEAR_LEVELS - 1; l >= 0; --l)
      if (w.idxn[l].rmax > 0.0f && cq <= w.idxn[l].cmax) lvl = l;
    const DevIndex& Xc = lvl >= 0 ? w.idxn[lvl] : X;
    int32_t leni = 0;
    if (X.rmax > 0.0f && cq <= X.cmax) {
      Rw = src_row(Xc.src, ei, cand_node(oi));
      leni = Xc.src[ei].len;
      sv = idx_find(Xc.slot, Rw, dst_key(g, ej, oj), lab);
    }
    if (sv < 0 || idx_slot_cost(lab) > cq) {
      spill_push<CTR_INDEX_MISS>(w, (int32_t)p);
      continue;
    }
    int len = 0;
    for (int32_t ps = idx_slot_pred(lab); ps >= 0 && len <= Rw.cnt; ps = idx_slot_pred(Xc.slot[Rw.off + ps])) ++len;
    const int off = len ? atomicAdd(&w.counters_i32[CTR_POOL_USED], len) : 0;
    if (off + len > w.pool_cap) {
      w.counters_i32[CTR_POOL_OVER] = 1;
      *w.abort = 1;
      w.path_len[p] = -1;
    } else {
      int k = len;
      for (int32_t ps = idx_slot_pred(lab); ps >= 0 && k > 0;) {
        const uint4 sl = Xc.slot[Rw.off + ps];
        w.path_pool[off + (--k)] = (int32_t)sl.x;
        ps = idx_slot_pred(sl);
      }
      w.path_off[p] = off;
      w.path_len[p] = len;
    }
    const float start = cand_node(oi) ? 0.0f : __int_as_float(leni) - oi;
    const float sd = start + bitsf(lab.z);
    w.route_dist[p] = sd + oj;
    if (w.ctr) {
      unsigned long long st = 0, rl = 0;
      for (int64_t k = 0; k < (int64_t)Rw.cap; ++k) {
        const uint4 sl = Xc.slot[Rw.off + k];
        if (sl.x == EMPTY || (sl.x & NODE_KEY) || idx_slot_cost(sl) > cq) continue;
        ++st;
        if ((unsigned long long)idx_slot_cost(sl) + g.e_len64[sl.x] <= cq) {
          const int32_t v = g.e_to[sl.x];
          rl += (unsigned long long)(g.out_off[v + 1] - g.out_off[v]);
        }
      }
      ++c_search;
      c_settled += st;
      c_relaxed += rl;
      c_edges += (unsigned long long)len;
    }
  }
  if (w.ctr) {
    cadd(&w.ctr->route_searches, c_search);
    cadd(&w.ctr->route_nodes_settled, c_settled);
    cadd(&w.ctr->route_edges_relaxed, c_relaxed);
    cadd(&w.ctr->route_edges, c_edges);
  }
}

template <int TIER>
__device__ __forceinline__ Table tier_table(const DevWork& w, uint32_t* lkey, unsigned long long* llab, uint32_t* linq,
                                            uint32_t* lfr0, uint32_t* lfr1) {
  if (TIER == 1) {
    const size_t base = (size_t)blockIdx.x * BIG_TABLE_CAP;
    return Table{w.big_key + base, w.big_lab + base, w.big_inq + base, w.big_fr + 2 * base,
                 w.big_fr + 2 * base + BIG_TABLE_CAP, BIG_TABLE_LOG2, SEARCH_LIMIT,
                 w.big_ins + (size_t)blockIdx.x * SEARCH_LIMIT, w.big_prev + blockIdx.x};
  }
  if (TIER == 2) {
    const size_t cap = (size_t)1 << w.huge_log2;
    const size_t base = (size_t)blockIdx.x * cap;
    const int lim = huge_limit(w.huge_log2);
    return Table{w.huge_key + base, w.huge_lab + base, w.huge_inq + base, w.huge_fr + 2 * base,
                 w.huge_fr + 2 * base + cap, w.huge_log2, lim, w.huge_ins + (size_t)blockIdx.x * lim,
                 w.huge_prev + blockIdx.x};
  }
  return Table{lkey, llab, linq, lfr0, lfr1, 8, LDS_TABLE_LIMIT};
}
__device__ __forceinline__ bool huge_unready(DevWork& w, int64_t nwork, const int32_t* list) {
  if (nwork <= 0 || w.huge_log2 > 0) return false;
  if (w.huge_final) {
    for (int64_t it = (int64_t)blockIdx.x * blockDim.x + threadIdx.x; it < nwork; it += (int64_t)gridDim.x * blockDim.x)
      atomicCAS(&w.trace_err[w.pt_trace[list[it]]], 0, OTM_TERR_SEARCH_OVERFLOW);
  } else if (blockIdx.x == 0 && threadIdx.x == 0) {
    w.counters_i32[CTR_GROW_HUGE] = 1;
    *w.abort = 1;
  }
  return true;
}
__device__ __forceinline__ void huge_overflow(DevWork& w, int64_t p) {
  if (w.huge_final) {
    atomicCAS(&w.trace_err[w.pt_trace[p]], 0, OTM_TERR_SEARCH_OVERFLOW);
  } else {
    w.counters_i32[CTR_GROW_HUGE] = 1;
    *w.abort = 1;
  }
}

template <int TIER>
__global__ __launch_bounds__(TB) void k_transitions(DevGraph g, DevBatch b, DevParams P, DevWork w) {
  constexpr bool BIG = TIER > 0;
  if (*w.abort || trans_over_cap(b, w)) return;
  __shared__ uint32_t lkey[BIG ? 1 : LDS_TABLE_CAP];
  __shared__ unsigned long long llab[BIG ? 1 : LDS_TABLE_CAP];
  __shared__ uint32_t linq[BIG ? 1 : LDS_TABLE_CAP];
  __shared__ uint32_t lfr0[BIG ? 1 : LDS_TABLE_CAP];
  __shared__ uint32_t lfr1[BIG ? 1 : LDS_TABLE_CAP];
  __shared__ int32_t cbuf[CHAIN_BUF * TB];
  __shared__ uint32_t TU[TURN_TABLE];
  __shared__ int32_t eq[KMAX], ep[KMAX];
  __shared__ float oq[KMAX], op[KMAX];
  __shared__ SearchShared S;
  const int lane = threadIdx.x;
  for (int k = lane; k < TURN_TABLE; k += TB) TU[k] = P.turn_units[k];
  Table T = tier_table<TIER>(w, lkey, llab, linq, lfr0, lfr1);
  auto predof = [&](uint32_t e) {
    const int sx = table_find<BIG>(T, e);
    return sx < 0 ? NONE_PRED : (uint32_t)(Mem<BIG>::ld(&T.lab[sx]) & 0xFFFFFFFFull);
  };
  const SpillRef work = TIER == 2 ? spill_of<CTR_TRANS_HUGE>(w)
                                  : (BIG ? spill_of<CTR_SEARCH_GLOBAL>(w) : spill_of<CTR_INDEX_MISS>(w));
  const int32_t* list = work.list;
  const int64_t nwork = (int64_t)*work.count;
  if (TIER == 2 && huge_unready(w, nwork, list)) return;
  __syncthreads();
  for (int64_t it = blockIdx.x; it < nwork; it += gridDim.x) {
    const int64_t p = (int64_t)list[it];
    const int32_t q = w.col_prev[p];
    if (q < 0) continue;
    const int Kq = w.ncand[q], Kp = w.ncand[p];
    const float gcv = w.gc[p];
    const float bound = P.factor * gcv;
    const uint32_t cq = index_cost_bound(bound);
    if (lane < Kq) {
      const int2 c = crec(w, q, lane);
      eq[lane] = c.x;
      oq[lane] = __int_as_float(c.y);
    }
    if (lane < Kp) {
      const int2 c = crec(w, p, lane);
      ep[lane] = c.x;
      op[lane] = __int_as_float(c.y);
    }
    __syncthreads();
    const int32_t u_l = lane < Kq ? src_node(g, eq[lane], oq[lane]) : -1;
    const uint32_t h_l = lane < Kq ? src_head(g, eq[lane], oq[lane]) : 0u;
    bool first = lane < Kq;
    for (int k = 0; k < Kq; ++k) {
      const int32_t uk = __shfl(u_l, k, 64);
      const uint32_t hk = __shfl(h_l, k, 64);
      if (k < lane && uk == u_l && hk == h_l) first = false;
    }
    unsigned long long srcmask = __ballot(first);
    float* Tm = w.trans + w.trans_off[p];
    bool failed = false;
    unsigned long long c_search = 0, c_settled = 0, c_relaxed = 0, c_trans = 0;
    while (srcmask) {
      const int sl = __ffsll((long long)srcmask) - 1;
      srcmask &= srcmask - 1;
      const int32_t u = __shfl(u_l, sl, 64);
      const uint32_t hin = __shfl(h_l, sl, 64);
      const int labels = ta_search<BIG>(g, TU, T, S, u, hin, cq, lane);
      if (labels < 0) {
        failed = true;
        break;
      }
      unsigned long long ntr = 0;
      for (int idx = lane; idx < Kq * Kp; idx += TB) {
        const int i = idx / Kp, j = idx - (idx / Kp) * Kp;
        if (src_node(g, eq[i], oq[i]) != u || src_head(g, eq[i], oq[i]) != hin) continue;
        const int32_t ei = eq[i], ej = ep[j];
        const float start = src_start(g, ei, oq[i]);
        float r = 0.0f;
        uint32_t units = 0;
        bool ok = true;
        if (same_edge_step(ei, oq[i], ej, op[j])) {
          r = same_edge_dist(oq[i], op[j]);
        } else {
          const uint32_t key = dst_key(g, ej, op[j]);
          const int slot = table_find<BIG>(T, key);
          if (slot < 0) {
            ok = false;
          } else {
            float d;
            int n;
            chain_sums(g, TU, predof, (uint32_t)(Mem<BIG>::ld(&T.lab[slot]) & 0xFFFFFFFFull), hin,
                       (key & NODE_KEY) ? NO_HEAD : (uint32_t)g.e_head_out[ej], cbuf + lane, d, units, n);
            const float sd = start + d;
            r = sd + op[j];
          }
        }
        float cost = INFINITY;
        if (ok && r <= bound) {
          cost = trans_cost(units, r, gcv, P.beta);
          ++ntr;
        }
        Tm[i * Kp + j] = cost;
      }
      if (w.ctr) {
        unsigned long long st, rl;
        ta_counts<BIG>(g, T, cq, lane, st, rl);
        for (int o = 32; o > 0; o >>= 1) ntr += __shfl_xor(ntr, o, 64);
        c_search += 1;
        c_settled += st;
        c_relaxed += rl;
        c_trans += ntr;
      }
      __syncthreads();
    }
    if (w.ctr && !failed && lane == 0) {
      cadd(&w.ctr->searches, c_search);
      cadd(&w.ctr->nodes_settled, c_settled);
      cadd(&w.ctr->edges_relaxed, c_relaxed);
      cadd(&w.ctr->transitions, c_trans);
    }
    if (failed && lane == 0) {
      if (TIER == 0) {
        spill_push<CTR_SEARCH_GLOBAL>(w, (int32_t)p);
      } else if (TIER == 1) {
        spill_push<CTR_TRANS_HUGE>(w, (int32_t)p);
      } else {
        huge_overflow(w, p);
      }
    }
    __syncthreads();
  }
}

__device__ __forceinline__ void wave_argmin(float v, int idx, float& bv, int& bi) {
  bv = v;
  bi = idx;
  for (int o = 32; o > 0; o >>= 1) {
    const float ov = __shfl_xor(bv, o, 64);
    const int oi = __shfl_xor(bi, o, 64);
    if (ov < bv || (ov == bv && oi < bi)) {
      bv = ov;
      bi = oi;
    }
  }
}

__device__ void viterbi_trace_global(int64_t a, int64_t e, DevWork& w) {
  const int lane = threadIdx.x;
  {
    float prev = INFINITY;
    bool open = false;
    int64_t last = -1;
    auto backtrack = [&](int64_t endp) {
      const int Ke = w.ncand[endp];
      float bv;
      int bi;
      wave_argmin(lane < Ke ? prev : INFINITY, lane, bv, bi);
      __syncthreads();
      if (lane == 0) {
        int64_t pp = endp;
        int jj = bi;
        while (true) {
          w.state[pp] = jj;
          w.chosen[pp] = crec(w, pp, jj);
          if (w.chain_start[pp]) break;
          jj = w.bp[pp * KMAX + jj];
          pp = w.col_prev[pp];
        }
      }
    };
    for (int64_t p = a; p < e; ++p) {
      if (!w.is_col[p]) continue;
      const int Kp = w.ncand[p];
      if (Kp == 0) {
        if (open) backtrack(last);
        open = false;
        continue;
      }
      bool started = false;
      float cur = INFINITY;
      if (open && w.col_prev[p] == (int32_t)last) {
        const int Kq = w.ncand[last];
        const float* Tm = w.trans + w.trans_off[p];
        float best = INFINITY;
        int bi = -1;
        for (int i = 0; i < Kq; ++i) {
          const float pi = __shfl(prev, i, 64);
          if (lane < Kp) {
            const float v = pi + Tm[i * Kp + lane];
            if (v < best) {
              best = v;
              bi = i;
            }
          }
        }
        const bool alive = lane < Kp && bi >= 0;
        if (lane < Kp) {
          cur = alive ? best + cemis(w, p, lane) : INFINITY;
          w.bp[p * KMAX + lane] = alive ? (uint8_t)bi : (uint8_t)0xFF;
        }
        if (__ballot(alive) == 0ull) {
          backtrack(last);
        } else {
          started = true;
        }
      } else if (open) {
        backtrack(last);
      }
      if (!started) {
        cur = lane < Kp ? cemis(w, p, lane) : INFINITY;
        if (lane == 0) w.chain_start[p] = 1;
      }
      prev = cur;
      open = true;
      last = p;
    }
    __syncthreads();
    if (open) backtrack(last);
    __syncthreads();
  }
}
#ifndef OTM_VIT_TW
#define OTM_VIT_TW 448
#endif
#ifndef OTM_VIT_BP
#define OTM_VIT_BP 768
#endif
#ifndef OTM_VIT_PTS
#define OTM_VIT_PTS 128
#endif
constexpr int VIT_PTS = OTM_VIT_PTS;
constexpr int VIT_BP = OTM_VIT_BP;
constexpr int VIT_TW = OTM_VIT_TW;
#ifndef OTM_VIT_EW
#define OTM_VIT_EW 256
#endif
constexpr int VIT_EW = OTM_VIT_EW;
static_assert(VIT_EW >= KMAX, "one column's emissions fit a window");

#ifndef OTM_VIT_WAVES
#define OTM_VIT_WAVES 8
#endif
__global__ __launch_bounds__(TB, OTM_VIT_WAVES) void k_viterbi(DevBatch b, DevWork w, const int32_t* list,
                                                               const int32_t* list_n, int snap) {
  if (snap && blockIdx.x == 0 && threadIdx.x == 0) fold_snap(w, SNAP_AFTER_TRANS, true);
  if (*w.abort) return;
  __shared__ float sT[VIT_TW];
  __shared__ float sEm[VIT_EW];
  __shared__ uint8_t sBp[VIT_BP];
  __shared__ int8_t sState[VIT_PTS];
  __shared__ uint8_t sCs[VIT_PTS];
  __shared__ int32_t sToff[VIT_PTS + 1];
  __shared__ int16_t sEoff[VIT_PTS + 1];
  __shared__ int16_t sCprev[VIT_PTS];
  __shared__ int8_t sKc[VIT_PTS];
  const int lane = threadIdx.x;
  const int32_t nwork = list ? *list_n : b.n_traces;
  for (int32_t it = blockIdx.x; it < nwork; it += gridDim.x) {
    const int32_t t = list ? list[it] : it;
    const int64_t a = b.trace_off[t], e = b.trace_off[t + 1];
    const int n = (int)(e - a);
    if (w.trace_err[t] != 0) {
      for (int64_t p = a + lane; p < e; p += TB) {
        w.state[p] = -1;
        w.chain_start[p] = 0;
      }
      continue;
    }
    const int64_t t0 = w.trans_off[a];
    int etot = 0;
    bool fits = n <= VIT_PTS;
    if (fits) {
      bool big = false;
      for (int c = 0; c < n; c += TB) {
        const int pl = c + lane;
        int kc = -1, cp = -1, to = 0;
        if (pl < n) {
          const int64_t p = a + pl;
          const uint8_t ic = w.is_col[p];
          const int32_t nc = w.ncand[p];
          const int32_t q = w.col_prev[p];
          const int64_t tp = w.trans_off[p];
          const int64_t tn = w.trans_off[p + 1];
          if (ic) {
// ... 641 lines not shown
        em_c[k] = pE[k];
        mw[k] = sM[g][c * CH + k];
      }
      wave_sync();
      lo_n = hi_c;
      hi_n = rng_end(c + 1);
      ld_data(c + 1, lo_n, hi_n);
      const bool big = hi_c - lo_c > win;
#pragma unroll
      for (int k = 0; k < CH; ++k) {
        const int pl = c * CH + k;
        const int mk = (int)(mw[k] & 0xFFu);
        const bool on = pl < n && (mk & 0x40);
        const int Kp = mk & 0x3F;
        const bool col = on && Kp > 0;
        const bool link = col && open && (mk & 0x80);
        const float em = em_c[k];
        if (fast && __builtin_amdgcn_ballot_w64(on && (!link || big)) == 0ull) {
          const unsigned long long lb = __builtin_amdgcn_ballot_w64(link);
          bool done = true;
          if (lb != 0ull) {
            float best = INFINITY;
            int bi = -1;
            const int pbits = __float_as_int(prev);
            const float* Tm = sTg + (link ? (int)(mw[k] >> 8) - lo_c : 0) + j;
            const int KpL = link ? Kp : 0;
            const int Kq = link ? lastK : 0;
            const bool g1 = __ballot(Kq > 4) != 0ull, g2 = __ballot(Kq > 8) != 0ull, g3 = __ballot(Kq > 12) != 0ull;
            float tv[16];
            vr_load<0>(Tm, KpL, tv);
            if (g1) vr_load<4>(Tm, KpL, tv);
            if (g2) vr_load<8>(Tm, KpL, tv);
            if (g3) vr_load<12>(Tm, KpL, tv);
            vr_four<0>(pbits, tv, best, bi);
            if (g1) vr_four<4>(pbits, tv, best, bi);
            if (g2) vr_four<8>(pbits, tv, best, bi);
            if (g3) vr_four<12>(pbits, tv, best, bi);
            const bool alive = link && j < Kp && bi >= 0;
            const unsigned long long ab = __builtin_amdgcn_ballot_w64(alive);
            const unsigned long long any = ((ab & 0x7FFF7FFF7FFF7FFFull) + 0x7FFF7FFF7FFF7FFFull) | ab;
            done = (lb & ~any & 0x8000800080008000ull) == 0ull;
            if (done) {
              const int nib = alive ? bi : 15;
              const int pair = __builtin_amdgcn_mov_dpp(nib, 0xB1, 0xF, 0xF, false);
              if (link && !(j & 1)) sBp[g][pl * (G / 2) + (j >> 1)] = (uint8_t)(nib | (pair << 4));
              const float cur = alive ? best + em : INFINITY;
              prev = link ? cur : prev;
              last = link ? pl : last;
              lastK = link ? Kp : lastK;
            }
          }
          if (done) continue;
        }
        if (on && open && !link) end_chain();
        int tb = link ? (int)(mw[k] >> 8) - lo_c : 0;
        if (__ballot(big && link) != 0ull) {
          if (big) {
            if (link) {
              const int64_t src = t0 + (int64_t)(mw[k] >> 8);
              for (int f = j; f < lastK * Kp; f += G) sTg[f] = w.trans[src + f];
            }
            tb = 0;
          }
          wave_sync();
        }
        bool started = false;
        float cur = INFINITY;
        const unsigned long long lb = __ballot(link);
        if (lb != 0ull) {
          float best = INFINITY;
          int bi = -1;
          const int pbits = __float_as_int(prev);
          const float* Tm = sTg + tb + j;
          const int KpL = link ? Kp : 0;
          const bool g1 = __ballot(link && lastK > 4) != 0ull, g2 = __ballot(link && lastK > 8) != 0ull,
                     g3 = __ballot(link && lastK > 12) != 0ull;
          float tv[16];
          vr_load<0>(Tm, KpL, tv);
          if (g1) vr_load<4>(Tm, KpL, tv);
          if (g2) vr_load<8>(Tm, KpL, tv);
          if (g3) vr_load<12>(Tm, KpL, tv);
          vr_four<0>(pbits, tv, best, bi);
          if (g1) vr_four<4>(pbits, tv, best, bi);
          if (g2) vr_four<8>(pbits, tv, best, bi);
          if (g3) vr_four<12>(pbits, tv, best, bi);
          const bool alive = link && j < Kp && bi >= 0;
          const int nib = alive ? bi : 15;
          const int pair = __builtin_amdgcn_mov_dpp(nib, 0xB1, 0xF, 0xF, false);
          if (link) {
            cur = alive ? best + em : INFINITY;
            if (!(j & 1)) sBp[g][pl * (G / 2) + (j >> 1)] = (uint8_t)(nib | (pair << 4));
            if (((__ballot(alive) >> gb) & 0xFFFFull) != 0ull) started = true;
            else end_chain();
          }
        }
        if (col && j == 0) sFl[g][pl] = (uint8_t)(started ? VG_COL : (VG_COL | VG_CS));
        cur = started ? cur : (j < Kp ? em : INFINITY);
        prev = col ? cur : prev;
        open = col || (open && !on);
        last = col ? pl : last;
        lastK = col ? Kp : lastK;
      }
      wave_sync();
    }
    if (act && open) end_chain();
    wave_sync();
    if (j == 0) {
      int sv = -1;
      for (int q = ((n + 3) >> 2) - 1; q >= 0; --q) {
        const uint32_t f4 = *(const uint32_t*)&sFl[g][q * 4];
        unsigned long long nb[4];
#pragma unroll
        for (int u = 0; u < 4; ++u) nb[u] = *(const unsigned long long*)&sBp[g][(q * 4 + u) * (G / 2)];
        uint32_t o4 = 0;
#pragma unroll
        for (int u = 3; u >= 0; --u) {
          const uint32_t f = (f4 >> (8 * u)) & 0xFFu;
          if (!(f & VG_COL)) continue;
          if (f & VG_END) sv = (int)(f >> 3);
          o4 |= ((f & VG_CS) | (uint32_t)((sv + 1) << 3)) << (8 * u);
          if (sv >= 0) sv = (f & VG_CS) ? -1 : (int)((nb[u] >> (4 * sv)) & 15ull);
        }
        *(uint32_t*)&sFl[g][q * 4] = o4;
      }
    }
    wave_sync();
    {
      int svs[VR_PTS / G];
      int2 ch[VR_PTS / G];
#pragma unroll
      for (int u = 0; u < VR_PTS / G; ++u) {
        const int pl = u * G + j;
        svs[u] = pl < n ? (int)(sFl[g][pl] >> 3) - 1 : -1;
        if (svs[u] >= 0) ch[u] = crec(w, a + pl, svs[u]);
      }
#pragma unroll
      for (int u = 0; u < VR_PTS / G; ++u) {
        const int pl = u * G + j;
        if (pl < n) {
          const int64_t p = a + pl;
          w.state[p] = svs[u];
          w.chain_start[p] = (uint8_t)((sFl[g][pl] & VG_CS) ? 1 : 0);
          if (svs[u] >= 0) w.chosen[p] = ch[u];
        }
      }
    }
    wave_sync();
  }
}

template <int TIER>
__global__ __launch_bounds__(TB) void k_route(DevGraph g, DevBatch b, DevParams P, DevWork w) {
  constexpr bool BIG = TIER > 0;
  if (*w.abort) return;
  __shared__ uint32_t lkey[BIG ? 1 : LDS_TABLE_CAP];
  __shared__ unsigned long long llab[BIG ? 1 : LDS_TABLE_CAP];
  __shared__ uint32_t linq[BIG ? 1 : LDS_TABLE_CAP];
  __shared__ uint32_t lfr0[BIG ? 1 : LDS_TABLE_CAP];
  __shared__ uint32_t lfr1[BIG ? 1 : LDS_TABLE_CAP];
  __shared__ int32_t cbuf[CHAIN_BUF * TB];
  __shared__ uint32_t TU[TURN_TABLE];
  __shared__ SearchShared S;
  const int lane = threadIdx.x;
  for (int k = lane; k < TURN_TABLE; k += TB) TU[k] = P.turn_units[k];
  Table T = tier_table<TIER>(w, lkey, llab, linq, lfr0, lfr1);
  auto predof = [&](uint32_t e) {
    const int sx = table_find<BIG>(T, e);
    return sx < 0 ? NONE_PRED : (uint32_t)(Mem<BIG>::ld(&T.lab[sx]) & 0xFFFFFFFFull);
  };
  const SpillRef work = TIER == 2 ? spill_of<CTR_ROUTE_HUGE>(w)
                                  : (BIG ? spill_of<CTR_SEARCH_GLOBAL>(w) : spill_of<CTR_INDEX_MISS>(w));
  const int32_t* list = work.list;
  const int64_t nwork = (int64_t)*work.count;
  if (TIER == 2 && huge_unready(w, nwork, list)) return;
  __syncthreads();
  for (int64_t it = blockIdx.x; it < nwork; it += gridDim.x) {
    const int64_t p = (int64_t)list[it];
    const int32_t q = w.col_prev[p];
    const int2 ci = w.chosen[q], cj = w.chosen[p];
    const int32_t ei = ci.x, ej = cj.x;
    const float oi = __int_as_float(ci.y), oj = __int_as_float(cj.y);
    if (same_edge_step(ei, oi, ej, oj)) {
      if (lane == 0) w.route_dist[p] = same_edge_dist(oi, oj);
      continue;
    }
    const float bound = P.factor * w.gc[p];
    const uint32_t cq = index_cost_bound(bound);
    const int32_t u = src_node(g, ei, oi);
    const uint32_t hin = src_head(g, ei, oi);
    const int labels = ta_search<BIG>(g, TU, T, S, u, hin, cq, lane);
    if (labels < 0) {
      if (lane == 0) {
        if (TIER == 0) {
          spill_push<CTR_SEARCH_GLOBAL>(w, (int32_t)p);
        } else if (TIER == 1) {
          spill_push<CTR_ROUTE_HUGE>(w, (int32_t)p);
        } else {
          huge_overflow(w, p);
        }
      }
      __syncthreads();
      continue;
    }
    unsigned long long st = 0, rl = 0;
    if (w.ctr) ta_counts<BIG>(g, T, cq, lane, st, rl);
    if (lane == 0) {
      const uint32_t key = dst_key(g, ej, oj);
      const int vs = table_find<BIG>(T, key);
      if (vs < 0) {
        atomicCAS(&w.trace_err[w.pt_trace[p]], 0, OTM_TERR_SEARCH_OVERFLOW);
      } else {
        const uint32_t pk = (uint32_t)(Mem<BIG>::ld(&T.lab[vs]) & 0xFFFFFFFFull);
        float d;
        uint32_t units;
        int n;
        chain_sums(g, TU, predof, pk, hin, NO_HEAD, cbuf, d, units, n);
        const int off = atomicAdd(&w.counters_i32[CTR_POOL_USED], n);
        if (off + n > w.pool_cap) {
          w.counters_i32[CTR_POOL_OVER] = 1;
          *w.abort = 1;
          w.path_len[p] = -1;
        } else {
          int k = n;
          for (uint32_t pe = pk; pe != NONE_PRED && k > 0; pe = predof(pe)) w.path_pool[off + (--k)] = (int32_t)pe;
          w.path_off[p] = off;
          w.path_len[p] = n;
        }
        const float start = src_start(g, ei, oi);
        const float sd = start + d;
        w.route_dist[p] = sd + oj;
        if (w.ctr) {
          cadd(&w.ctr->route_searches, 1);
          cadd(&w.ctr->route_nodes_settled, st);
          cadd(&w.ctr->route_edges_relaxed, rl);
          cadd(&w.ctr->route_edges, (unsigned long long)n);
        }
      }
    }
    __syncthreads();
  }
}

struct EAttr {
  float len;
  int32_t seg, seg_pos;
  uint32_t flags;
  int64_t way;
  uint64_t gid;
  float glen;
};

__device__ __forceinline__ uint4 edge_rec(const DevGraph& g, int32_t e) { return g.e_rec[e]; }
__device__ __forceinline__ float rec_len(const uint4& r) { return __uint_as_float(r.x); }
__device__ __forceinline__ int32_t rec_seg(const uint4& r) { return (int32_t)r.y; }
__device__ __forceinline__ int32_t rec_pos(const uint4& r) { return (int32_t)(r.z & 0xFFFFFFu); }
__device__ __forceinline__ uint32_t rec_flags(const uint4& r) { return r.z >> 24; }

__device__ __forceinline__ EAttr edge_attr(const DevGraph& g, int32_t e) {
  const uint4 r = edge_rec(g, e);
  EAttr a;
  a.len = rec_len(r);
  a.seg = rec_seg(r);
  a.seg_pos = a.seg >= 0 ? rec_pos(r) : 0;
  a.flags = rec_flags(r);
  a.way = g.way_tab[r.w];
  a.gid = a.seg >= 0 ? g.g_id[a.seg] : 0ull;
  a.glen = a.seg >= 0 ? g.g_len[a.seg] : 0.0f;
  return a;
}

struct Trav {
  int32_t edge;
  float off0, off1;
  double t0, t1;
  int32_t sh0, sh1;
  EAttr at;
};

template <bool WRITE>
struct SegEmitter {
  DevOut* o;
  int32_t seg_base, way_base;
  int32_t nseg = 0, nway = 0;
  bool has = false;
  Trav first, last;
  int32_t way_start = 0;
  int64_t last_way = 0;

  __device__ void add_way(const EAttr& at) {
    const int64_t way = at.way;
    if (nway > way_start && last_way == way) return;
    if (WRITE) o->way_ids[way_base + nway] = way;
    last_way = way;
    ++nway;
  }
  __device__ void flush() {
    if (!has) return;
    if (WRITE) {
      otm_segment s;
      const int32_t sg = first.at.seg;
      bool sv, ev;
      s.flags = 0u;
      if (sg >= 0) {
        sv = first.off0 == 0.0f && (first.at.flags & OTM_EDGE_SEG_BEGIN_D);
        ev = last.off1 == last.at.len && (last.at.flags & OTM_EDGE_SEG_END_D);
        s.segment_id = (int64_t)first.at.gid;
        s.length = (sv && ev) ? (int32_t)floor((double)first.at.glen + 0.5) : -1;
      } else {
        sv = first.off0 == 0.0f;
        ev = last.off1 == last.at.len;
        s.segment_id = -1;
        s.length = -1;
        if (first.at.flags & OTM_EDGE_INTERNAL_D) s.flags |= OTM_SEG_INTERNAL;
      }
      s.start_time = 0.0;
      s.end_time = 0.0;
      if (sv) {
        s.flags |= OTM_SEG_START_VALID;
        s.start_time = first.t0;
      }
      if (ev) {
        s.flags |= OTM_SEG_END_VALID;
        s.end_time = last.t1;
      }
      s.queue_length = 0;
      s.begin_shape_index = first.sh0;
      s.end_shape_index = last.sh1;
      s.way_off = way_base + way_start;
      s.way_cnt = nway - way_start;
      s.pad = 0u;
      ((otm_segment*)o->segments)[seg_base + nseg] = s;
      o->seg_gidx[seg_base + nseg] = sg;
    }
    ++nseg;
    has = false;
  }
  __device__ void push(const Trav& t) {
    bool join = false;
    if (has) {
      const int32_t s = t.at.seg, ps = last.at.seg;
      if (s >= 0) join = ps == s && t.at.seg_pos == last.at.seg_pos + 1;
      else join = ps < 0 && ((t.at.flags ^ last.at.flags) & OTM_EDGE_INTERNAL_D) == 0;
    }
    if (!join) {
      flush();
      has = true;
      first = t;
      way_start = nway;
    }
    last = t;
    add_way(t.at);
  }
  static constexpr uint32_t OTM_EDGE_INTERNAL_D = 0x01, OTM_EDGE_SEG_BEGIN_D = 0x02, OTM_EDGE_SEG_END_D = 0x04;
};

__device__ __forceinline__ double time_at(double ta, double tb, float x, float R) {
  if (R > 0.0f) return ta + (tb - ta) * ((double)x / (double)R);
  return ta;
}

__device__ __forceinline__ void step_bound(const DevBatch& b, const DevWork& w, int64_t a, int lp, int pl, float R,
                                           double ta, double tb, float x, double& t, int& sh) {
  if (pl - lp < 2) {
    t = time_at(ta, tb, x, R);
    sh = x >= R ? pl : lp;
    return;
  }
  int iL = lp, k = lp + 1;
  float xL = 0.0f, xN = R, run = 0.0f;
  double tL = ta, tN = tb;
  for (; k < pl; ++k) {
    const float v = w.ipos[a + k];
    if (!(v >= run)) continue;
    if (!(v <= x)) break;
    iL = k;
    xL = v;
    tL = b.time[a + k];
    run = v;
  }
  for (; k < pl; ++k) {
    const float v = w.ipos[a + k];
    if (v >= run) {
      xN = v;
      tN = b.time[a + k];
      break;
    }
  }
  sh = R <= x ? pl : iL;
  const float den = xN - xL;
  t = den > 0.0f ? tL + (tN - tL) * ((double)(x - xL) / (double)den) : tL;
}

// ... 630 lines not shown
  }
  if (mode != 2) return 0;
  const double r = floor(sum + 0.5);
  return r >= (double)length ? length : (int32_t)r;
}

__global__ __launch_bounds__(TB) void k_queue(DevBatch b, DevWork w, DevOut o, float kph) {
  if (*w.abort) return;
  const int lane = threadIdx.x;
  for (int32_t t = blockIdx.x; t < b.n_traces; t += gridDim.x) {
    if (w.trace_err[t] != 0) continue;
    const int64_t a = b.trace_off[t];
    const int n = (int)(b.trace_off[t + 1] - a);
    const int32_t ns = o.seg_cnt[t];
    otm_segment* SG = o.segments + (int32_t)o.seg_base[t];
    for (int si = lane; si < ns; si += TB) {
      const otm_segment s = SG[si];
      if (s.segment_id < 0 || s.length < 0 || n <= 0) continue;
      SG[si].queue_length =
          queue_walk(b, w, a, n, s.begin_shape_index, s.end_shape_index, s.start_time, s.end_time, s.length, (double)kph);
    }
  }
}

__device__ __forceinline__ bool in_lv(const int64_t* lv, int n, int64_t x) {
  for (int k = 0; k < n; ++k)
    if (lv[k] == x) return true;
  return false;
}

#ifndef OTM_REPORT_WAVES
#define OTM_REPORT_WAVES 1
#endif
constexpr int32_t REPW_MAX_TRACES = 2 * 8 * 4 * 256;
__device__ int report_walk(int32_t t, const DevBatch& b, const DevReportCfg& rc, const DevWork& w,
                           const otm_segment* S, otm_trace_result& r, otm_report_rec* REP) {
  r.code = 200;
  r.rep_cnt = 0;
  r.shape_used = -1;
  r.successful_count = r.unreported_count = r.discontinuities = r.invalid_speeds = r.unassociated = 0;
  r.successful_length = r.unreported_length = -1;
  if (r.error_kind != 0) {
    r.code = 500;
    return 0;
  }
  const double end_time = b.time[b.trace_off[t + 1] - 1];
  auto ST = [&](const otm_segment& s) { return (s.flags & OTM_SEG_START_VALID) ? s.start_time : -1.0; };
  auto ET = [&](const otm_segment& s) { return (s.flags & OTM_SEG_END_VALID) ? s.end_time : -1.0; };
  auto ST_INT = [&](const otm_segment& s) {
    return !(s.flags & OTM_SEG_START_VALID) || (s.flags & OTM_SEG_START_INT) != 0u;
  };
  auto ET_INT = [&](const otm_segment& s) { return !(s.flags & OTM_SEG_END_VALID) || (s.flags & OTM_SEG_END_INT) != 0u; };
  int last_idx = r.seg_cnt - 1;
  while (last_idx >= 0 && end_time - ST(S[last_idx]) < rc.threshold_sec) --last_idx;
  r.shape_used = last_idx >= 0 ? S[last_idx].begin_shape_index : -1;
  bool have = false, first = true;
  int prior = -1;
  int64_t prior_level = -1;
  int nrep = 0;
  int zerodiv = 0;
  for (int idx = 0; idx <= last_idx; ++idx) {
    const otm_segment& s = S[idx];
    const bool internal = (s.flags & OTM_SEG_INTERNAL) != 0;
    if (idx != 0 && ST(s) == -1.0 && ET(S[idx - 1]) == -1.0) r.discontinuities++;
    const int64_t level = s.segment_id >= 0 ? (s.segment_id & 7) : -1;
    if (have && S[prior].segment_id >= 0 && S[prior].length > 0 && !internal) {
      const otm_segment& ps = S[prior];
      if (in_lv(rc.report_levels, rc.n_report, prior_level)) {
        const bool trans = in_lv(rc.transition_levels, rc.n_transition, level);
        const double t0 = ST(ps);
        const double t1 = trans ? ST(s) : ET(ps);
        const bool t0_int = ST_INT(ps);
        const bool t1_int = trans ? ST_INT(s) : ET_INT(ps);
        const double den = t1 - t0;
        if (den == 0.0) {
          zerodiv = t0_int && t1_int ? OTM_TERR_ZERODIV_INT : OTM_TERR_ZERODIV;
          break;
        }
        const double speed = ((double)ps.length / den) * 3.6;
        if (speed < 200.0) {
          otm_report_rec rep;
          rep.id = ps.segment_id;
          rep.next_id = (trans && s.segment_id >= 0) ? s.segment_id : -1;
          rep.t0 = t0;
          rep.t1 = t1;
          rep.flags = (t1_int ? OTM_REP_T1_INT : 0u) | (t0_int ? OTM_REP_T0_INT : 0u);
          rep.length = ps.length;
          rep.queue_length = ps.queue_length;
          rep.pad = (uint32_t)prior;
          REP[nrep++] = rep;
          r.successful_count++;
          r.successful_length = ps.length;
        } else {
          r.invalid_speeds++;
        }
      } else {
        r.unreported_count++;
        r.unreported_length = ps.length;
      }
    }
    if (!(internal && !first)) {
      prior = idx;
      prior_level = level;
      have = true;
    }
    first = false;
    if (s.segment_id < 0 && !internal) r.unassociated++;
  }
  if (zerodiv) {
    r.code = 500;
    r.error_kind = zerodiv;
    r.shape_used = -1;
    r.successful_count = r.unreported_count = r.discontinuities = r.invalid_speeds = r.unassociated = 0;
    r.successful_length = r.unreported_length = -1;
    return 0;
  }
  return nrep;
}

__device__ __forceinline__ void report_hist(const DevOut& o, int32_t seg_off, otm_report_rec& rep) {
  const int32_t ps = (int32_t)rep.pad;
  rep.pad = 0u;
  if (!o.hist) return;
  const double speed = ((double)rep.length / (rep.t1 - rep.t0)) * 3.6;
  const bool t1_minus1 = (rep.flags & OTM_REP_T1_INT) && rep.t1 == -1.0;
  const int32_t gi = o.seg_gidx[seg_off + ps];
  if (t1_minus1 || !(speed >= 0.0) || gi < 0) return;
  int bin = (int)(speed / (double)o.bin_kph);
  bin = bin < 0 ? 0 : (bin >= o.nbins ? o.nbins - 1 : bin);
  atomicAdd(&o.hist[(size_t)gi * o.nbins + bin], 1u);
  if (o.speed_sum) {
    atomicAdd(&o.speed_sum[gi], (unsigned long long)(speed * 1000.0 + 0.5));
  }
}

__device__ __forceinline__ void report_pair(const DevOut& o, int32_t seg_off, int32_t seg_cnt, int32_t ps,
                                            const otm_report_rec& rep) {
  int32_t gn = -1;
  if (rep.next_id >= 0) {
    const otm_segment* S = o.segments + seg_off;
    int32_t j = ps + 1;
    while (j < seg_cnt && (S[j].flags & OTM_SEG_INTERNAL)) ++j;
    if (j < seg_cnt) gn = o.seg_gidx[seg_off + j];
  }
  pair_report(o.pairs, o.seg_gidx[seg_off + ps], gn, rep.t0, rep.t1, rep.length, rep.queue_length, rep.flags);
}

__device__ __forceinline__ void report_pass(const DevOut& o, int32_t seg_off, int32_t seg_cnt, otm_report_rec& rep) {
  const int32_t ps = (int32_t)rep.pad;
  report_hist(o, seg_off, rep);
  if (o.pairs.key) report_pair(o, seg_off, seg_cnt, ps, rep);
}

__global__ __launch_bounds__(256, OTM_REPORT_WAVES) void k_report(DevBatch b, DevReportCfg rc, DevWork w, DevOut o, int32_t n_seg_total) {
  if (*w.abort) return;
  const int32_t t = blockIdx.x * blockDim.x + threadIdx.x;
  if (t >= b.n_traces) return;
  otm_trace_result r;
  r.error_kind = w.trace_err[t];
  r.seg_off = (int32_t)o.seg_base[t];
  r.seg_cnt = o.seg_cnt[t];
  r.rep_off = r.seg_off;
  otm_report_rec* REP = o.reports + r.rep_off;
  const int nrep = report_walk(t, b, rc, w, o.segments + r.seg_off, r, REP);
  for (int k = 0; k < nrep; ++k) report_pass(o, r.seg_off, r.seg_cnt, REP[k]);
  r.rep_cnt = nrep;
  if (w.ctr && r.code == 200) {
    cadd(&w.ctr->segments_out, (unsigned long long)r.seg_cnt);
    cadd(&w.ctr->reports_out, (unsigned long long)nrep);
  }
  o.traces[t] = r;
  o.rep_cnt[t] = r.rep_cnt;
}

constexpr int REPW_CAP = 64;
__global__ __launch_bounds__(TB) void k_report_wave(DevBatch b, DevReportCfg rc, DevWork w, DevOut o, int32_t n_seg_total) {
  if (*w.abort) return;
  __shared__ unsigned long long sSeg[REPW_CAP * sizeof(otm_segment) / 8];
  __shared__ int32_t sN;
  static_assert(sizeof(otm_segment) % 8 == 0, "segment words");
  constexpr int SW = (int)(sizeof(otm_segment) / 8);
  const int lane = threadIdx.x;
  for (int32_t t = blockIdx.x; t < b.n_traces; t += gridDim.x) {
    otm_trace_result r;
    r.error_kind = w.trace_err[t];
    r.seg_off = (int32_t)o.seg_base[t];
    r.seg_cnt = o.seg_cnt[t];
    r.rep_off = r.seg_off;
    const otm_segment* G = o.segments + r.seg_off;
    otm_report_rec* REP = o.reports + r.rep_off;
    const bool fits = r.seg_cnt <= REPW_CAP;
    if (fits && r.error_kind == 0) {
      const unsigned long long* gw = (const unsigned long long*)G;
      for (int k = lane; k < r.seg_cnt * SW; k += TB) sSeg[k] = gw[k];
    }
    __syncthreads();
    if (lane == 0) {
      const int nrep = report_walk(t, b, rc, w, fits ? (const otm_segment*)sSeg : G, r, REP);
      r.rep_cnt = nrep;
      sN = nrep;
      if (w.ctr && r.code == 200) {
        cadd(&w.ctr->segments_out, (unsigned long long)r.seg_cnt);
        cadd(&w.ctr->reports_out, (unsigned long long)nrep);
      }
      o.traces[t] = r;
      o.rep_cnt[t] = nrep;
      __threadfence_block();
    }
    __syncthreads();
    const int nrep = sN;
    for (int k = lane; k < nrep; k += TB) report_pass(o, r.seg_off, r.seg_cnt, REP[k]);
    __syncthreads();
  }
}

struct RoutePiece {
  int32_t edge;
  float o0, o1, xs;
};
struct RoutePlace {
  float pos;
  int32_t edge;
  float off;
};
template <bool FOOT>
__device__ __forceinline__ RoutePlace place_on_route(const DevGraph& g, const DevBatch& b, const DevParams& P,
                                                     const DevWork& w, int64_t q, int64_t p, int64_t k) {
  const int2 ci = w.chosen[q], cj = w.chosen[p];
  const int32_t ei = ci.x, ej = cj.x;
  const float oi = __int_as_float(ci.y), oj = __int_as_float(cj.y);
  const int32_t poff = w.path_off[p], plen = w.path_len[p];
  const bool has0 = !cand_node(oi);
  const int npc = (has0 ? 1 : 0) + plen + (cand_node(oj) ? 0 : 1);
  const float start = src_start(g, ei, oi);
  const float ds = (2.0f * P.sigma_z) * P.sigma_z;
  const float lat = b.lat[k], lon = b.lon[k];
  const float ls = MPD_F * cos_deg(lat);
  const float gcd = gc_dist(b.lat[q], b.lon[q], lat, lon);
  float best = INFINITY, bpos = -1.0f, dd = 0.0f, bo = 0.0f;
  int32_t be = -1;
  for (int m = 0; m < npc; ++m) {
    RoutePiece pc;
    const int pk = m - (has0 ? 1 : 0);
    const bool mid = !(has0 && m == 0) && pk < plen;
    const int32_t e = has0 && m == 0 ? ei : (mid ? w.path_pool[poff + pk] : ej);
    const int4 er = g.e_proj[e];
    const float len = __int_as_float(er.z);
    if (has0 && m == 0) {
      pc = RoutePiece{e, oi, len, 0.0f};
    } else if (mid) {
      pc = RoutePiece{e, 0.0f, len, start + dd};
      dd = dd + len;
    } else {
      pc = RoutePiece{e, 0.0f, oj, start + dd};
    }
    float bsq, boff;
    project_edge(g, er, lat, lon, ls, bsq, boff);
    if (!(boff >= pc.o0 && boff <= pc.o1)) continue;
    const float pos = pc.xs + (boff - pc.o0);
    const float cost = bsq / ds + fabsf(pos - gcd) / P.beta;
    if (cost < best) {
      best = cost;
      if constexpr (FOOT) {
        be = pc.edge;
        bo = boff;
      } else {
        bpos = pos;
      }
    }
  }
  return RoutePlace{bpos, be, bo};
}

__device__ __forceinline__ bool interp_step(const DevWork& w, int64_t k, int32_t& q, int32_t& p) {
  q = w.prevc[k];
  p = q >= 0 ? w.nextc[q] : -1;
  return p >= 0 && w.col_prev[p] == q && !w.chain_start[p] && w.state[p] >= 0 && w.path_len[p] >= 0;
}

__global__ __launch_bounds__(256) void k_seg_bound(DevGraph g, DevBatch b, DevParams P, DevWork w, int64_t* tb) {
  const int64_t k = (int64_t)blockIdx.x * blockDim.x + threadIdx.x;
  if (k == b.n_points) fold_snap(w, SNAP_AFTER_ROUTE, false);
  if (*w.abort) return;
  const int lane = threadIdx.x & 63;
  int64_t v = 0;
  int32_t t = -1;
  if (k < b.n_points) {
    t = w.pt_trace[k];
    if (w.is_col[k]) {
      if (w.state[k] >= 0) {
        const int32_t pl = w.path_len[k];
        v = 2 + (pl > 0 ? pl : 0);
      }
    } else {
      int32_t q, p;
      if (interp_step(w, k, q, p) && w.trace_err[t] == 0) {
        const int2 ci = w.chosen[q], cj = w.chosen[p];
        if (!same_edge_step(ci.x, __int_as_float(ci.y), cj.x, __int_as_float(cj.y)))
          w.ipos[k] = place_on_route<false>(g, b, P, w, q, p, k).pos;
      }
    }
  }
#pragma unroll
  for (int d = 1; d < 64; d <<= 1) {
    const int64_t vn = __shfl_down(v, d, 64);
    const int32_t tn = __shfl_down(t, d, 64);
    if (lane + d < 64 && tn == t) v += vn;
  }
  const int32_t tp = __shfl_up(t, 1, 64);
  if (t >= 0 && (lane == 0 || tp != t) && v != 0) atomicAdd((unsigned long long*)&tb[t], (unsigned long long)v);
}

__global__ __launch_bounds__(TB) void k_compact(int32_t n_traces, DevOut o, const int32_t* seg_off, const int32_t* way_off,
                                                const int32_t* rep_off, otm_segment* so, int64_t* wo,
                                                otm_report_rec* ro, otm_trace_result* to) {
  const int lane = threadIdx.x;
  const otm_trace_result* TR = o.traces;
  const otm_segment* SI = o.segments;
  const otm_report_rec* RI = o.reports;
  for (int32_t t = blockIdx.x; t < n_traces; t += gridDim.x) {
    const int32_t base = TR[t].seg_off;
    const int32_t ns = o.seg_cnt[t], nw = o.way_cnt[t], nr = o.rep_cnt[t];
    const int32_t ds = seg_off[t], dw = way_off[t], dr = rep_off[t];
    for (int k = lane; k < ns; k += TB) {
      otm_segment x = SI[base + k];
      x.way_off = x.way_off - base + dw;
      so[ds + k] = x;
    }
    for (int k = lane; k < nw; k += TB) wo[dw + k] = o.way_ids[base + k];
// ... 646 lines not shown
}

template <bool WRITE>
__global__ __launch_bounds__(TB) void k_shape(DevGraph g, int32_t n_traces, const int64_t* seg_base, DevTrav tv,
                                              DevShape sh) {
  const int lane = threadIdx.x;
  for (int32_t t = blockIdx.x; t < n_traces; t += gridDim.x) {
    const otm_traversal* reg = tv.rec + seg_base[t];
    const int n = (int)tv.cnt[t];
    int64_t vb = 0, vcap = 0, pb = 0, pcap = 0, sb = 0;
    if (WRITE) {
      vb = sh.vtx_off[t];
      vcap = sh.vtx_off[t + 1] - vb;
      pb = sh.poly_off[t];
      pcap = sh.poly_off[t + 1] - pb;
      sb = sh.trav_off[t];
    }
    int64_t c_v = 0, c_b = 0;
    int c_lat = 0, c_lon = 0;
    for (int c0 = 0; c0 < n; c0 += TB) {
      const int r = c0 + lane;
      const bool in = r < n;
      int32_t s0 = 0, m = 0, i0 = 1, nint = 0;
      float bo = 0.0f, zo = 0.0f;
      bool cs = false;
      if (in) {
        const otm_traversal* q = reg + r;
        const int32_t e = q->edge;
        cs = (q->flags & OTM_TV_CHAIN_START) != 0;
        bo = q->begin_offset;
        zo = q->end_offset;
        s0 = g.e_shape_off[e];
        m = g.e_shape_off[e + 1] - s0 - 1;
        int i1 = 1;
        for (int i = 1; i < m; ++i) {
          const float c = g.s_cum[s0 + i];
          if (!(bo < c)) {
            i0 = i1 = i + 1;
            continue;
          }
          if (!(c < zo)) break;
          i1 = i + 1;
        }
        nint = i1 - i0;
      }
      const int nv = in ? (cs ? 1 : 0) + nint + 1 : 0;
      const int incl = wave_incl_scan(nv, lane);
      const int excl = incl - nv;
      const int total = __shfl(incl, 63, 64);
      if (WRITE && in) {
        const int32_t bv = (int32_t)(c_v + excl) - (cs ? 0 : 1), ev = (int32_t)(c_v + incl) - 1;
        ((int2*)sh.span)[sb + r] = make_int2(bv, ev);
      }
      for (int v0 = 0; v0 < total; v0 += TB) {
        const int j = v0 + lane;
        const bool act = j < total;
        int own = 0;
#pragma unroll
        for (int step = 32; step; step >>= 1) {
          const int val = __shfl(incl, own + step - 1, 64);
          if (val <= j) own += step;
        }
        const int o_s0 = __shfl(s0, own, 64), o_m = __shfl(m, own, 64), o_i0 = __shfl(i0, own, 64);
        const int o_nint = __shfl(nint, own, 64), o_ex = __shfl(excl, own, 64), o_cs = __shfl((int)cs, own, 64);
        const float o_b = __shfl(bo, own, 64), o_z = __shfl(zo, own, 64);
        int qlat = 0, qlon = 0;
        if (act) {
          int k = j - o_ex;
          double la, lo;
          if (o_cs && k == 0) {
            shape_coord(g, o_s0, o_m, o_b, la, lo);
          } else {
            k -= o_cs;
            if (k < o_nint) {
              la = (double)g.s_lat[o_s0 + o_i0 + k];
              lo = (double)g.s_lon[o_s0 + o_i0 + k];
            } else {
              shape_coord(g, o_s0, o_m, o_z, la, lo);
            }
          }
          qlat = (int32_t)rint(la * 1e6);
          qlon = (int32_t)rint(lo * 1e6);
        }
        int plat = __shfl_up(qlat, 1, 64), plon = __shfl_up(qlon, 1, 64);
        if (lane == 0) {
          plat = c_lat;
          plon = c_lon;
        }
        const int dla = qlat - plat, dlo = qlon - plon;
        const uint32_t za = ((uint32_t)dla << 1) ^ (uint32_t)(dla >> 31);
        const uint32_t zb = ((uint32_t)dlo << 1) ^ (uint32_t)(dlo >> 31);
        const int na = 1 + (31 - __clz((int)(za | 1u))) / 5, nb = 1 + (31 - __clz((int)(zb | 1u))) / 5;
        const int nby = act ? na + nb : 0;
        const int binc = wave_incl_scan(nby, lane);
        if (WRITE && act) {
          const int64_t vi = c_v + j, bp = c_b + binc - nby;
          if (vi < vcap) ((int2*)sh.vtx)[vb + vi] = make_int2(qlat, qlon);
          if (bp + nby <= pcap) shape_put(shape_put(sh.poly + pb + bp, za, na), zb, nb);
        }
        const int last = (total - v0 < TB ? total - v0 : TB) - 1;
        c_lat = __shfl(qlat, last, 64);
        c_lon = __shfl(qlon, last, 64);
        c_b += __shfl(binc, 63, 64);
      }
      c_v += total;
    }
    if (!WRITE && lane == 0) {
      sh.vtx_off[t] = c_v;
      sh.poly_off[t] = c_b;
    }
  }
}

int grid_for(int64_t n, int per_block, int cap) {
  int64_t g = (n + per_block - 1) / per_block;
  if (g < 1) g = 1;
  return (int)(g > cap ? cap : g);
}

constexpr int WAVE_GRID_CAP = 256 * 64;
#ifndef OTM_TRANS_GRID_CAP
#define OTM_TRANS_GRID_CAP 65536
#endif
constexpr int TRANS_GRID_CAP = OTM_TRANS_GRID_CAP;

}

void launch_fetch_scan(int32_t n, const int32_t* c0, const int32_t* c1, const int32_t* c2, int32_t* o0, int32_t* o1,
                       int32_t* o2, hipStream_t s) {
  hipLaunchKernelGGL(k_fetch_scan, dim3(1), dim3(1024), 0, s, n, c0, c1, c2, o0, o1, o2);
}


const char* const kKernelNames[KN_COUNT] = {
    "k_columns",       "spatial_order",  "k_cand_lane",    "k_candidates",     "k_links",         "scan_trans_off",  "k_trans_sub",
    "k_trans_wide",    "k_transitions",  "k_transitions_big", "k_viterbi",      "k_route_index",
    "k_route",         "k_route_big",    "k_seg_bound",      "scan_seg_bound",  "k_segments",       "k_report"};

namespace {
constexpr int SPILL_GRID = 4096;
#ifndef OTM_WIDE_GRID
#define OTM_WIDE_GRID 8192
#endif
constexpr int WIDE_GRID = OTM_WIDE_GRID;
}

#define TIMED(k, launch) \
  do {                   \
    mk.begin(k, s);      \
    launch;              \
    mk.end(k, s);        \
  } while (0)

void launch_columns(const DevGraph& g, const DevBatch& b, const DevParams& p, DevWork& w, hipStream_t s,
                    const Marks& mk) {
  if (w.ord.tile_cnt) (void)hipMemsetAsync(w.ord.tile_cnt, 0, ORDER_TILES * 4, s);
  TIMED(KN_COLUMNS, hipLaunchKernelGGL(k_columns, dim3(grid_for(b.n_traces, 1, WAVE_GRID_CAP)), dim3(TB), 0, s, g,
                                       b, p, w));
}
static int order_grid(int64_t n, int per_block, int cap) {
  const int64_t per_group = (n + ORDER_GROUPS - 1) / ORDER_GROUPS;
  int64_t gb = (per_group + per_group / 4 + per_block - 1) / per_block;
  if (gb < 1) gb = 1;
  int64_t gtot = gb * ORDER_GROUPS;
  if (gtot > cap) gtot = cap / ORDER_GROUPS * ORDER_GROUPS;
  return (int)gtot;
}

void launch_order(const DevBatch& b, DevWork& w, hipStream_t s, const Marks& mk) {
  mk.begin(KN_ORDER, s);
  hipLaunchKernelGGL(k_order_plan, dim3(1), dim3(1024), 0, s, w.ord.tile_cnt, w.ord.cursor, w.ord.grp);
  hipLaunchKernelGGL(k_order_scatter, dim3(grid_for(b.n_points, 256, 8192)), dim3(256), 0, s, b, w, w.ord.tile,
                     w.ord.cursor, w.ord.item);
  mk.end(KN_ORDER, s);
}

void launch_candidates(const DevGraph& g, const DevBatch& b, const DevParams& p, DevWork& w, hipStream_t s,
                       const Marks& mk, int from) {
  if (from < RESUME_CAND_BIG) {
    if (w.ctr)
      TIMED(KN_CAND_LANE, hipLaunchKernelGGL(k_cand_lane<true>, dim3(order_grid(b.n_points, CAND_TB, 1 << 30)),
                                             dim3(CAND_TB), 0, s, g, b, p, w));
    else
      TIMED(KN_CAND_LANE, hipLaunchKernelGGL(k_cand_lane<false>, dim3(order_grid(b.n_points, CAND_TB, 1 << 30)),
                                             dim3(CAND_TB), 0, s, g, b, p, w));
  }
  mk.begin(KN_CAND_WAVE, s);
#ifndef OTM_CAND_WAVE_GRID
#define OTM_CAND_WAVE_GRID 4096
#endif
  if (from < RESUME_CAND_BIG)
    hipLaunchKernelGGL(k_candidates<false>, dim3(OTM_CAND_WAVE_GRID), dim3(TB), 0, s, g, b, p, w);
  hipLaunchKernelGGL(k_candidates<true>, dim3(CAND_BIG_SLOTS), dim3(TB), 0, s, g, b, p, w);
  mk.end(KN_CAND_WAVE, s);
}
void launch_links(const DevBatch& b, const DevParams& p, DevWork& w, hipStream_t s, const Marks& mk) {
  TIMED(KN_LINKS, hipLaunchKernelGGL(k_links, dim3(grid_for(b.n_points + 1, 256, 1 << 30)), dim3(256), 0, s, b, p,
                                     w));
}
__global__ __launch_bounds__(256) void k_expand_compact(const int64_t* trace_off, const int64_t* tbase,
                                                        const int32_t* dt, const int16_t* acc16, double* time,
                                                        float* acc, int32_t n_traces) {
  const int wv = threadIdx.x >> 6, lane = threadIdx.x & 63;
  for (int64_t t = (int64_t)blockIdx.x * 4 + wv; t < n_traces; t += (int64_t)gridDim.x * 4) {
    const int64_t a = trace_off[t], e = trace_off[t + 1], base = tbase[t];
    for (int64_t i = a + lane; i < e; i += 64) {
      time[i] = (double)(base + (int64_t)dt[i]);
      acc[i] = (float)acc16[i];
    }
  }
}
void launch_expand_compact(const int64_t* trace_off, const int64_t* tbase, const int32_t* dt, const int16_t* acc16,
                           double* time, float* acc, int32_t n_traces, hipStream_t s) {
  if (n_traces <= 0) return;
  hipLaunchKernelGGL(k_expand_compact, dim3(grid_for(((int64_t)n_traces + 3) / 4, 1, 1 << 20)), dim3(256), 0, s,
                     trace_off, tbase, dt, acc16, time, acc, n_traces);
}
void launch_status(const int32_t* abort, const int64_t* ttotal, const int32_t* counters, BatchStatus* out,
                   hipStream_t s) {
  hipLaunchKernelGGL(k_status, dim3(1), dim3(64), 0, s, abort, ttotal, counters, out);
}
void launch_transitions(const DevGraph& g, const DevBatch& b, const DevParams& p, DevWork& w, hipStream_t s,
                        const Marks& mk, int sub, int from) {
  if (from >= RESUME_TRANS_HUGE) {
    mk.begin(KN_TRANS_GLOBAL, s);
    hipLaunchKernelGGL(k_transitions<2>, dim3(HUGE_SLOTS), dim3(TB), 0, s, g, b, p, w);
    mk.end(KN_TRANS_GLOBAL, s);
    return;
  }
  const int per = TB / sub;
  const int grid = order_grid((b.n_points + per - 1) / per, 1, TRANS_GRID_CAP);
  if (sub == 8) {
    TIMED(KN_TRANS_INDEX, hipLaunchKernelGGL((k_trans_sub<8, false>), dim3(grid), dim3(TB), 0, s, g, b, p, w));
    TIMED(KN_TRANS_WIDE, hipLaunchKernelGGL((k_trans_sub<16, true>), dim3(WIDE_GRID), dim3(TB), 0, s, g, b, p, w));
  } else {
    TIMED(KN_TRANS_INDEX, hipLaunchKernelGGL((k_trans_sub<16, false>), dim3(grid), dim3(TB), 0, s, g, b, p, w));
    mk.begin(KN_TRANS_WIDE, s);
    mk.end(KN_TRANS_WIDE, s);
  }
  TIMED(KN_TRANS_WAVE, hipLaunchKernelGGL(k_transitions<0>, dim3(SPILL_GRID), dim3(TB), 0, s, g, b, p, w));
  mk.begin(KN_TRANS_GLOBAL, s);
  hipLaunchKernelGGL(k_transitions<1>, dim3(BIG_SLOTS), dim3(TB), 0, s, g, b, p, w);
  hipLaunchKernelGGL(k_transitions<2>, dim3(HUGE_SLOTS), dim3(TB), 0, s, g, b, p, w);
  mk.end(KN_TRANS_GLOBAL, s);
}
void launch_viterbi(const DevBatch& b, DevWork& w, hipStream_t s, const Marks& mk) {
  const char* fe = std::getenv("OTM_VIT_FORM");
  const int forced = fe ? std::atoi(fe) : 0;
  constexpr int gmin = 32768;
  constexpr int rmin = 4096;
  const int form = forced ? forced : (b.n_traces >= gmin ? 8 : (b.n_traces >= rmin ? 4 : 64));
  const SpillRef to_16 = spill_of<CTR_VIT_16>(w), to_wave = spill_of<CTR_VIT_WAVE>(w);
  if (form == 4) {
    const char* we = std::getenv("OTM_VR_WIN");
    const int vt = OTM_VR_U * 16;
    int win = we ? std::atoi(we) : vt;
    win = win < 0 ? 0 : (win > vt ? vt : win);
    const char* fa = std::getenv("OTM_VR_FAST");
    const int fast = fa ? (std::atoi(fa) != 0 ? 1 : 0) : 1;
    mk.begin(KN_VITERBI, s);
    hipLaunchKernelGGL(k_viterbi_row, dim3(grid_for(b.n_traces, TB / 16, WAVE_GRID_CAP)), dim3(TB), 0, s, b, w,
                       to_wave.list, to_wave.count, win, fast, 1);
    hipLaunchKernelGGL(k_viterbi, dim3(grid_for(b.n_traces, 1, WAVE_GRID_CAP)), dim3(TB), 0, s, b, w,
                       (const int32_t*)to_wave.list, (const int32_t*)to_wave.count, 0);
    mk.end(KN_VITERBI, s);
    return;
  }
  if (form == 64) {
    TIMED(KN_VITERBI, hipLaunchKernelGGL(k_viterbi, dim3(grid_for(b.n_traces, 1, WAVE_GRID_CAP)), dim3(TB), 0, s, b,
                                         w, (const int32_t*)nullptr, (const int32_t*)nullptr, 1));
    return;
  }
  int32_t* l8 = to_16.list;
  int32_t* n8 = to_16.count;
  int32_t* l16 = to_wave.list;
  int32_t* n16 = to_wave.count;
  mk.begin(KN_VITERBI, s);
  if (form == 16) {
    hipLaunchKernelGGL(k_viterbi_g<16>, dim3(grid_for(b.n_traces, TB / 16, WAVE_GRID_CAP)), dim3(TB), 0, s, b, w,
                       (const int32_t*)nullptr, (const int32_t*)nullptr, l16, n16, 1);
  } else {
    hipLaunchKernelGGL(k_viterbi_g<8>, dim3(grid_for(b.n_traces, TB / 8, WAVE_GRID_CAP)), dim3(TB), 0, s, b, w,
                       (const int32_t*)nullptr, (const int32_t*)nullptr, l8, n8, 1);
    hipLaunchKernelGGL(k_viterbi_g<16>, dim3(grid_for(b.n_traces, TB / 16, WAVE_GRID_CAP)), dim3(TB), 0, s, b, w,
                       (const int32_t*)l8, (const int32_t*)n8, l16, n16, 0);
  }
  hipLaunchKernelGGL(k_viterbi, dim3(grid_for(b.n_traces / 64 + 1, 1, 1024)), dim3(TB), 0, s, b, w,
                     (const int32_t*)l16, (const int32_t*)n16, 0);
  mk.end(KN_VITERBI, s);
}
void launch_route(const DevGraph& g, const DevBatch& b, const DevParams& p, DevWork& w, hipStream_t s,
                  const Marks& mk, int from) {
  if (from >= RESUME_ROUTE_HUGE) {
    mk.begin(KN_ROUTE_GLOBAL, s);
    hipLaunchKernelGGL(k_route<2>, dim3(HUGE_SLOTS), dim3(TB), 0, s, g, b, p, w);
    mk.end(KN_ROUTE_GLOBAL, s);
    return;
  }
  TIMED(KN_ROUTE_INDEX, hipLaunchKernelGGL(k_route_index, dim3(order_grid(b.n_points, 256, 1 << 30)), dim3(256), 0,
                                           s, g, b, p, w));
  TIMED(KN_ROUTE_WAVE, hipLaunchKernelGGL(k_route<0>, dim3(SPILL_GRID), dim3(TB), 0, s, g, b, p, w));
  mk.begin(KN_ROUTE_GLOBAL, s);
  hipLaunchKernelGGL(k_route<1>, dim3(BIG_SLOTS), dim3(TB), 0, s, g, b, p, w);
  hipLaunchKernelGGL(k_route<2>, dim3(HUGE_SLOTS), dim3(TB), 0, s, g, b, p, w);
  mk.end(KN_ROUTE_GLOBAL, s);
}
void launch_segments(const DevGraph& g, const DevBatch& b, DevWork& w, DevOut& o, hipStream_t s, const Marks& mk) {
  const dim3 grid(grid_for(b.n_traces, 1, WAVE_GRID_CAP));
  const SpillRef large = spill_of<CTR_SEG_LARGE>(w);
  int32_t* lst = large.list;
  int32_t* cnt = large.count;
  mk.begin(KN_SEG_WRITE, s);
  hipLaunchKernelGGL((k_segments<SEGP_PTS_S, SEGP_TRAV_S>), grid, dim3(TB), 0, s, g, b, w, o, (const int32_t*)nullptr,
                     (const int32_t*)nullptr, lst, cnt);
  hipLaunchKernelGGL((k_segments<SEGP_PTS, SEGP_TRAV>), dim3(grid_for(b.n_traces, 1, 2048)), dim3(TB), 0, s, g, b, w,
                     o, (const int32_t*)lst, (const int32_t*)cnt, (int32_t*)nullptr, (int32_t*)nullptr);
  mk.end(KN_SEG_WRITE, s);
}
void launch_queue(const DevBatch& b, DevWork& w, DevOut& o, float kph, hipStream_t s) {
  hipLaunchKernelGGL(k_queue, dim3(grid_for(b.n_traces, 1, WAVE_GRID_CAP)), dim3(TB), 0, s, b, w, o, kph);
}
void launch_points(const DevGraph& g, const DevBatch& b, const DevParams& p, DevWork& w, otm_matched_point* out,
                   hipStream_t s) {
  hipLaunchKernelGGL(k_points, dim3(grid_for(b.n_traces, 1, WAVE_GRID_CAP)), dim3(TB), 0, s, g, b, p, w, out);
}
void launch_scores(const DevBatch& b, DevWork& w, const DevScores& sc, hipStream_t s) {
  if (b.n_traces <= 0 || b.n_points <= 0) return;
  const char* fe = std::getenv("OTM_SCORE_FORM");
  const int forced = fe ? std::atoi(fe) : 0;
  constexpr int rmin = 4096;
  const int form = forced == 1 || forced == 4 ? forced : (b.n_traces >= rmin ? 4 : 1);
  if (form == 1) {
    hipLaunchKernelGGL(k_scores<64>, dim3(grid_for(b.n_traces, 1, WAVE_GRID_CAP)), dim3(TB), 0, s, b, w, sc,
                       (const int32_t*)nullptr, (const int32_t*)nullptr, (int32_t*)nullptr, (int32_t*)nullptr);
    return;
  }
  (void)hipMemsetAsync(sc.rej_n, 0, sizeof *sc.rej_n, s);
  hipLaunchKernelGGL(k_scores<16>, dim3(grid_for(b.n_traces, TB / 16, WAVE_GRID_CAP)), dim3(TB), 0, s, b, w, sc,
                     (const int32_t*)nullptr, (const int32_t*)nullptr, sc.rej, sc.rej_n);
  hipLaunchKernelGGL(k_scores<64>, dim3(grid_for(b.n_traces, 1, WAVE_GRID_CAP)), dim3(TB), 0, s, b, w, sc,
                     (const int32_t*)sc.rej, (const int32_t*)sc.rej_n, (int32_t*)nullptr, (int32_t*)nullptr);
}
void launch_traversals(const DevGraph& g, const DevBatch& b, DevWork& w, DevOut& o, const DevTrav& tv, hipStream_t s) {
  hipLaunchKernelGGL(k_traversals, dim3(grid_for(b.n_traces, 1, WAVE_GRID_CAP)), dim3(TB), 0, s, g, b, w, o, tv);
}
void launch_trav_compact(int32_t n_traces, const int64_t* seg_base, const int64_t* off, const otm_traversal* reg,
                         otm_traversal* dst, hipStream_t s) {
  hipLaunchKernelGGL(k_trav_compact, dim3(grid_for(n_traces, 1, WAVE_GRID_CAP)), dim3(TB), 0, s, n_traces, seg_base, off,
                     reg, dst);
}
void launch_shape(const DevGraph& g, int32_t n_traces, const int64_t* seg_base, const DevTrav& tv, const DevShape& sh,
                  bool write, hipStream_t s) {
  const dim3 grid(grid_for(n_traces, 1, WAVE_GRID_CAP));
  if (write)
    hipLaunchKernelGGL(k_shape<true>, grid, dim3(TB), 0, s, g, n_traces, seg_base, tv, sh);
  else
    hipLaunchKernelGGL(k_shape<false>, grid, dim3(TB), 0, s, g, n_traces, seg_base, tv, sh);
}
void launch_seg_bound(const DevGraph& g, const DevBatch& b, const DevParams& p, DevWork& w, int64_t* tb, hipStream_t s,
                      const Marks& mk) {
  TIMED(KN_SEG_BOUND, hipLaunchKernelGGL(k_seg_bound, dim3(grid_for(b.n_points + 1, 256, 1 << 30)), dim3(256), 0, s,
                                         g, b, p, w, tb));
}
void launch_compact(int32_t n_traces, const DevOut& o, const int32_t* seg_off, const int32_t* way_off,
                    const int32_t* rep_off, otm_segment* segs_out, int64_t* ways_out, otm_report_rec* reps_out,
                    otm_trace_result* traces_out, hipStream_t s) {
  hipLaunchKernelGGL(k_compact, dim3(grid_for(n_traces, 1, WAVE_GRID_CAP)), dim3(TB), 0, s, n_traces, o, seg_off, way_off,
                     rep_off, segs_out, ways_out, reps_out, traces_out);
}
void launch_report(const DevBatch& b, const DevReportCfg& rc, DevWork& w, DevOut& o, hipStream_t s,
                   const Marks& mk) {
  constexpr int tb = 16;
  if (b.n_traces <= REPW_MAX_TRACES)
    TIMED(KN_REPORT, hipLaunchKernelGGL(k_report_wave, dim3(grid_for(b.n_traces, 1, WAVE_GRID_CAP)), dim3(TB), 0, s,
                                        b, rc, w, o, 0));
  else
    TIMED(KN_REPORT, hipLaunchKernelGGL(k_report, dim3(grid_for(b.n_traces, tb, 1 << 30)), dim3(tb), 0, s, b, rc, w,
                                        o, 0));
}
#undef TIMED

void launch_index_build(const DevGraph& g, const uint32_t* turn_units, uint32_t cmax, int32_t* row_cnt,
                        const IdxRow* rows, uint4* slot, bool write, hipStream_t s) {
  const int grid = grid_for((int64_t)g.n_edges + g.n_nodes, 1, 256 * 16);
  if (write)
    hipLaunchKernelGGL(k_index_build<true>, dim3(grid), dim3(TB), 0, s, g, turn_units, cmax, row_cnt, rows, slot);
  else
    hipLaunchKernelGGL(k_index_build<false>, dim3(grid), dim3(TB), 0, s, g, turn_units, cmax, row_cnt, rows, slot);
}
int index_load_fast() { return IDX_LOAD_FAST; }
int index_load_dense() { return IDX_LOAD_DENSE; }
void launch_row_sizes(const int32_t* row_cnt, int64_t* row_sizes, int32_t n, int pct, hipStream_t s) {
  hipLaunchKernelGGL(k_row_sizes, dim3(grid_for((int64_t)n + 1, 256, 1 << 30)), dim3(256), 0, s, row_cnt, row_sizes,
                     n, pct);
}
void launch_row_pack(const int32_t* row_cnt, const int64_t* row_off, IdxRow* rows, int32_t n, hipStream_t s) {
  hipLaunchKernelGGL(k_row_pack, dim3(grid_for((int64_t)n, 256, 1 << 30)), dim3(256), 0, s, row_cnt, row_off, rows, n);
}
void launch_src_pack(const DevGraph& g, const IdxRow* rows, SrcRec* src, hipStream_t s) {
  if (g.n_edges <= 0) return;
  hipLaunchKernelGGL(k_src_pack, dim3(grid_for((int64_t)g.n_edges, 256, 1 << 30)), dim3(256), 0, s, g, rows, src);
}

size_t scan_tmp_bytes(int64_t n) {
  size_t a = 0, c = 0;
  (void)hipcub::DeviceScan::ExclusiveSum(nullptr, a, (int64_t*)nullptr, (int64_t*)nullptr, (int)(n + 1));
  (void)hipcub::DeviceScan::ExclusiveSum(nullptr, c, (int32_t*)nullptr, (int32_t*)nullptr, (int)(n + 1));
  return a > c ? a : c;
}
void scan_i64(int64_t* d, int64_t n, void* tmp, size_t tmp_bytes, hipStream_t s) {
  (void)hipcub::DeviceScan::ExclusiveSum(tmp, tmp_bytes, d, d, (int)(n + 1), s);
}
void scan_i32(int32_t* d, int64_t n, void* tmp, size_t tmp_bytes, hipStream_t s) {
  (void)hipcub::DeviceScan::ExclusiveSum(tmp, tmp_bytes, d, d, (int)(n + 1), s);
}

}
```

Baseline: 1.735 billion.

## Cut per-batch launches: fold status, seg_base zeroing, and skip unused huge-tier kernels

```diff
diff --git a/reporter_amd/csrc/engine.cpp b/reporter_amd/csrc/engine.cpp
--- a/reporter_amd/csrc/engine.cpp
+++ b/reporter_amd/csrc/engine.cpp
@@ -550,7 +550,7 @@
   return OTM_OK;
 }
 
-static int bind_point_work(otm_engine* E, int64_t NP, int32_t NT, DevWork& w, std::string* err) {
+static int bind_point_work(otm_engine* E, int64_t NP, int32_t NT, DevWork& w, hipStream_t s, std::string* err) {
   const size_t Pn = (size_t)NP + 1;
   TRY(bind_buf(w.pt_trace, E->pt_trace, Pn, err));
   TRY(bind_buf(w.is_col, E->is_col, Pn, err));
@@ -584,7 +584,11 @@
   TRY(bind_buf(w.counters_i32, E->counters_i32, CTR_WORDS, err));
   TRY(E->snap.ensure(1, err));
   w.snap = &E->snap.p->stage[0][0];
-  TRY(bind_buf(w.abort, E->abort_flag, 4, err));
+  {
+    bool fresh;
+    TRY(bind_buf(w.abort, E->abort_flag, ABORT_WORDS, err, &fresh));
+    if (fresh) HIPCHK(hipMemsetAsync(E->abort_flag.p, 0, E->abort_flag.bytes(), s));
+  }
   if (!E->caps_read) {
     E->caps_read = true;
     if (const char* v = std::getenv("OTM_TRANS_CAP")) E->trans_cap = std::max<int64_t>(1, std::atoll(v)), E->caps_pinned = true;
@@ -659,7 +663,7 @@
   const int32_t NT = b.n_traces;
   end_records(E, REC_BATCH_BEGINS);
   DevWork w{};
-  TRY(bind_point_work(E, NP, NT, w, err));
+  TRY(bind_point_work(E, NP, NT, w, s, err));
 
   DevParams dp = E->dp;
   if (NP < E->small_points) {
@@ -677,7 +681,9 @@
   mk.ev = E->timing ? E->kev : nullptr;
   TRY(bind_order(E, NP, dp.order_mask != 0, w.ord, err));
   if (from == RESUME_ALL) {
-    launch_columns(E->g, b, dp, w, s, mk);
+    int64_t* seg_base;
+    TRY(bind_buf(seg_base, E->seg_ub, (size_t)NT + 1, err));
+    launch_columns(E->g, b, dp, w, seg_base, s, mk);
     if (dp.order_mask) {
       launch_order(b, w, s, mk);
     } else if (E->timing) {
@@ -686,6 +692,7 @@
     }
   }
   TRY(ensure_cand(E, w, err));
+  if (from < RESUME_CAND_BIG && !w.cand_log2 && !w.cand_final) w.skipped |= SKIP_CAND_BIG;
   if (from <= RESUME_CAND_BIG) launch_candidates(E->g, b, dp, w, s, mk, from);
   if (from <= RESUME_CAND_BIG) {
     launch_links(b, dp, w, s, mk);
@@ -696,6 +703,8 @@
   TRY(bind_trans(E, w, s, err));
   TRY(ensure_big(E, w, err));
   TRY(ensure_huge(E, w, err));
+  if (!w.huge_log2 && !w.huge_final)
+    w.skipped |= (from < RESUME_TRANS_HUGE ? SKIP_TRANS_HUGE : 0) | (from < RESUME_ROUTE_HUGE ? SKIP_ROUTE_HUGE : 0);
   if (from <= RESUME_TRANS_HUGE) launch_transitions(E->g, b, dp, w, s, mk, E->trans_lanes, from);
   if (from <= RESUME_TRANS_HUGE) launch_viterbi(b, w, s, mk);
   launch_route(E->g, b, dp, w, s, mk, from);
@@ -715,7 +724,7 @@
     o.bin_kph = H->bin_kph;
     o.pairs = H->pairs_tab;
   }
-  HIPCHK(hipMemsetAsync(o.seg_base, 0, ((size_t)NT + 1) * sizeof *o.seg_base, s));
+  if (from != RESUME_ALL) HIPCHK(hipMemsetAsync(o.seg_base, 0, ((size_t)NT + 1) * sizeof *o.seg_base, s));
   launch_seg_bound(E->g, b, dp, w, o.seg_base, s, mk);
   mk.begin(KN_SEG_SCAN, s);
   scan_i64(o.seg_base, NT, E->scan_tmp.p, E->scan_tmp.cap(), s);
@@ -743,7 +752,8 @@
     if (for_route) E->tv_T = NT;
     if (for_shape) E->sh_T = NT;
   }
-  launch_report(b, E->drc, w, o, s, mk);
+  TRY(E->h_status.ensure(1, err));
+  launch_report(b, E->drc, w, o, E->h_status.p, s, mk);
   HIPCHK(hipGetLastError());
   E->last_T = NT;
   E->last_P = NP;
@@ -775,10 +785,6 @@
   E->last_resumes = 0;
   for (int attempt = 0;; ++attempt) {
     TRY(engine_match_once(E, b, s, err, from));
-    TRY(E->h_status.ensure(1, err));
-    BatchStatus* dst = &E->snap.p->status;
-    launch_status(E->abort_flag.p, E->trans_off.p + NP, E->counters_i32.p, dst, s);
-    HIPCHK(hipMemcpyAsync(E->h_status.p, dst, sizeof(BatchStatus), hipMemcpyDeviceToHost, s));
     HIPCHK(wait_batch(E, s, NP));
     const BatchStatus st = *E->h_status.p;
     const int32_t ab = st.abort;
@@ -1317,7 +1323,7 @@
   o.reports = (otm_report_rec*)(d + off[9]);
   o.hist = nullptr;
   o.speed_sum = nullptr;
-  launch_report(b, E->drc, w, o, s, Marks{});
+  launch_report(b, E->drc, w, o, nullptr, s, Marks{});
   HIPCHK(hipGetLastError());
   if (T) HIPCHK(hipMemcpyAsync(traces, d + off[8], (size_t)T * sizeof(otm_trace_result), hipMemcpyDeviceToHost, s));
   if (NS) HIPCHK(hipMemcpyAsync(reports, d + off[9], (size_t)NS * sizeof(otm_report_rec), hipMemcpyDeviceToHost, s));
diff --git a/reporter_amd/csrc/kernels.h b/reporter_amd/csrc/kernels.h
--- a/reporter_amd/csrc/kernels.h
+++ b/reporter_amd/csrc/kernels.h
@@ -186,6 +186,15 @@
                   ctr_per_batch(CTR_GROW_HUGE) && ctr_per_batch(CTR_CAND_BIG) && ctr_per_batch(CTR_GROW_CAND) &&
                   ctr_per_batch(CTR_VIT_WAVE),
               "per-batch slots lie past the snapshot range, within what K1 zeroes");
+
+enum DoneSlot : int {
+  DONE_CAND_WAVE = 0, DONE_TRANS_GLOBAL = 1, DONE_ROUTE_GLOBAL = 2, DONE_WORDS = 4
+};
+constexpr int DONE_BASE = 32;
+constexpr int DONE_LINE = 32;
+constexpr int DONE_SHARDS = 64;
+constexpr int ABORT_WORDS = DONE_BASE + DONE_LINE * DONE_WORDS * (1 + DONE_SHARDS);
+enum SkipBit : int32_t { SKIP_CAND_BIG = 1, SKIP_TRANS_HUGE = 2, SKIP_ROUTE_HUGE = 4 };
 
 struct DevWork {
   int32_t* pt_trace;
@@ -214,6 +223,7 @@
   int32_t* path_len;
   int32_t* path_pool;
   int32_t pool_cap;
+  int32_t skipped;
   int32_t* trace_err;
   int32_t* spill_list1;
   int32_t* spill_list2;
@@ -326,8 +336,8 @@
   }
 };
 
-void launch_columns(const DevGraph& g, const DevBatch& b, const DevParams& p, DevWork& w, hipStream_t s,
-                    const Marks& mk);
+void launch_columns(const DevGraph& g, const DevBatch& b, const DevParams& p, DevWork& w, int64_t* seg_base,
+                    hipStream_t s, const Marks& mk);
 enum Resume { RESUME_ALL = 0, RESUME_CAND_BIG = 1, RESUME_TRANS_HUGE = 2, RESUME_ROUTE_HUGE = 3 };
 void launch_candidates(const DevGraph& g, const DevBatch& b, const DevParams& p, DevWork& w, hipStream_t s,
                        const Marks& mk, int from = RESUME_ALL);
@@ -354,7 +364,9 @@
 void launch_scores(const DevBatch& b, DevWork& w, const DevScores& sc, hipStream_t s);
 void launch_shape(const DevGraph& g, int32_t n_traces, const int64_t* seg_base, const DevTrav& tv, const DevShape& sh,
                   bool write, hipStream_t s);
-void launch_report(const DevBatch& b, const DevReportCfg& rc, DevWork& w, DevOut& o, hipStream_t s, const Marks& mk);
+struct BatchStatus;
+void launch_report(const DevBatch& b, const DevReportCfg& rc, DevWork& w, DevOut& o, BatchStatus* status,
+                   hipStream_t s, const Marks& mk);
 void launch_order(const DevBatch& b, DevWork& w, hipStream_t s, const Marks& mk);
 void launch_seg_bound(const DevGraph& g, const DevBatch& b, const DevParams& p, DevWork& w, int64_t* tb, hipStream_t s,
                       const Marks& mk);
@@ -376,13 +388,10 @@
 };
 struct SnapBuf {
   int32_t stage[SNAP_COUNT][CTR_STAGE_WORDS];
-  BatchStatus status;
-};
-static_assert(offsetof(SnapBuf, status) == 192 && sizeof(SnapBuf) == 192 + 32, "snapshot buffer layout");
+};
+static_assert(sizeof(SnapBuf) == 192, "snapshot buffer layout");
 void launch_expand_compact(const int64_t* trace_off, const int64_t* tbase, const int32_t* dt, const int16_t* acc16,
                            double* time, float* acc, int32_t n_traces, hipStream_t s);
-void launch_status(const int32_t* abort, const int64_t* ttotal, const int32_t* counters, BatchStatus* out,
-                   hipStream_t s);
 void launch_row_pack(const int32_t* row_cnt, const int64_t* row_off, IdxRow* rows, int32_t n, hipStream_t s);
 void launch_src_pack(const DevGraph& g, const IdxRow* rows, SrcRec* src, hipStream_t s);
 size_t req_sparse_slots(int32_t n, size_t bytes);
diff --git a/reporter_amd/csrc/kernels.hip b/reporter_amd/csrc/kernels.hip
--- a/reporter_amd/csrc/kernels.hip
+++ b/reporter_amd/csrc/kernels.hip
@@ -303,6 +303,41 @@
   if (active && m.leader == (int)(threadIdx.x & 63)) atomicAdd(&ctr[key], m.count);
 }
 
+__device__ __forceinline__ uint32_t* done_word(const DevWork& w, int slot) {
+  return (uint32_t*)(w.abort + DONE_BASE) + slot * DONE_LINE;
+}
+__device__ __forceinline__ void vmem_drain() { asm volatile("s_waitcnt vmcnt(0)" ::: "memory"); }
+__device__ __forceinline__ void acquire_agent() {
+  __builtin_amdgcn_fence(__ATOMIC_ACQUIRE, "agent");
+  vmem_drain();
+}
+__device__ __forceinline__ bool count_done(const DevWork& w, DoneSlot slot) {
+  const uint32_t nb = gridDim.x, sh = blockIdx.x % DONE_SHARDS;
+  uint32_t* shard = done_word(w, DONE_WORDS + slot * DONE_SHARDS + sh);
+  if (atomicAdd(shard, 1u) != (nb - sh + DONE_SHARDS - 1) / DONE_SHARDS - 1) return false;
+  *shard = 0;
+  uint32_t* top = done_word(w, slot);
+  if (atomicAdd(top, 1u) != (nb < DONE_SHARDS ? nb : DONE_SHARDS) - 1) return false;
+  *top = 0;
+  acquire_agent();
+  return true;
+}
+__device__ __forceinline__ bool last_wave_done(const DevWork& w, DoneSlot slot, int lane) {
+  vmem_drain();
+  int last = 0;
+  if (lane == 0) last = count_done(w, slot);
+  return __shfl(last, 0, 64) != 0;
+}
+
+template <CtrSlot LIST, CtrSlot GROW, DoneSlot DONE>
+__device__ __forceinline__ void tier_unlaunched(const DevWork& w, int lane, bool gated) {
+  if (!last_wave_done(w, DONE, lane)) return;
+  if (lane == 0 && w.counters_i32[LIST] > 0 && !(gated && *w.abort)) {
+    w.counters_i32[GROW] = 1;
+    *w.abort = 1;
+  }
+}
+
 __global__ __launch_bounds__(1024) void k_order_plan(const int32_t* tile_cnt, int32_t* cursor, int32_t* grp) {
   __shared__ int32_t part[1024];
   __shared__ int32_t cut[ORDER_GROUPS + 1];
@@ -363,14 +398,17 @@
 #define OTM_COL_PTS 256
 #endif
 constexpr int COL_PTS = OTM_COL_PTS;
-__global__ __launch_bounds__(TB) void k_columns(DevGraph g, DevBatch b, DevParams P, DevWork w) {
+__global__ __launch_bounds__(TB) void k_columns(DevGraph g, DevBatch b, DevParams P, DevWork w, int64_t* seg_base) {
   __shared__ float sLat[COL_PTS], sLon[COL_PTS], sGc[COL_PTS];
   __shared__ int32_t sPrev[COL_PTS];
   __shared__ uint8_t sCol[COL_PTS];
   const int lane = threadIdx.x;
   if (blockIdx.x == 0) {
     if (lane < CTR_ZEROED_WORDS) w.counters_i32[lane] = 0;
-    if (lane == 0) *w.abort = 0;
+    if (lane == 0) {
+      *w.abort = 0;
+      seg_base[b.n_traces] = 0;
+    }
   }
   for (int32_t t = blockIdx.x; t < b.n_traces; t += gridDim.x) {
     const int64_t a = b.trace_off[t], e = b.trace_off[t + 1];
@@ -466,6 +504,7 @@
     }
     if (lane == 0) {
       w.trace_err[t] = 0;
+      seg_base[t] = 0;
       if (w.ctr) {
         cadd(&w.ctr->points, (unsigned long long)n);
         cadd(&w.ctr->columns, (unsigned long long)ncols);
@@ -905,6 +944,7 @@
     if (s_over) {
       if (lane == 0) {
         if (!BIG) {
+          w.ncand[p] = 0;
           spill_push<CTR_CAND_BIG>(w, (int32_t)p);
         } else if (w.cand_final) {
           w.ncand[p] = 0;
@@ -1011,6 +1051,7 @@
     }
     __syncthreads();
   }
+  if (!BIG && (w.skipped & SKIP_CAND_BIG)) tier_unlaunched<CTR_CAND_BIG, CTR_GROW_CAND, DONE_CAND_WAVE>(w, lane, false);
 }
 
 __global__ __launch_bounds__(256) void k_links(DevBatch b, DevParams P, DevWork w) {
@@ -1038,17 +1079,6 @@
   if (w.colrec && (P.order_mask & ORDER_TRANS) && w.is_col[p])
     w.colrec[w.colrec_pos[p]] = make_int4((int32_t)p, cp, kq | (w.ncand[p] << 8), __float_as_int(w.gc[p]));
   w.vmeta[p] = (uint8_t)((w.is_col[p] ? (w.ncand[p] | 0x40) : 0) | (cp >= 0 ? 0x80 : 0));
-}
-
-__global__ void k_status(const int32_t* abort, const int64_t* ttotal, const int32_t* counters, BatchStatus* out) {
-  if (threadIdx.x == 0) {
-    out->abort = *abort;
-    out->grow = (counters[CTR_GROW_HUGE] != 0 ? GROW_HUGE : 0) | (counters[CTR_GROW_CAND] != 0 ? GROW_CAND : 0);
-    out->ttotal = *ttotal;
-    out->pool_used = counters[CTR_POOL_USED];
-    out->pool_over = counters[CTR_POOL_OVER];
-    out->route_huge = counters[CTR_ROUTE_HUGE];
-  }
 }
 
 struct Table {
@@ -1769,7 +1799,11 @@
 template <int TIER>
 __global__ __launch_bounds__(TB) void k_transitions(DevGraph g, DevBatch b, DevParams P, DevWork w) {
   constexpr bool BIG = TIER > 0;
-  if (*w.abort || trans_over_cap(b, w)) return;
+  if (*w.abort || trans_over_cap(b, w)) {
+    if (TIER == 1 && (w.skipped & SKIP_TRANS_HUGE))
+      tier_unlaunched<CTR_TRANS_HUGE, CTR_GROW_HUGE, DONE_TRANS_GLOBAL>(w, threadIdx.x, true);
+    return;
+  }
   __shared__ uint32_t lkey[BIG ? 1 : LDS_TABLE_CAP];
   __shared__ unsigned long long llab[BIG ? 1 : LDS_TABLE_CAP];
   __shared__ uint32_t linq[BIG ? 1 : LDS_TABLE_CAP];
@@ -1894,6 +1928,8 @@
     }
     __syncthreads();
   }
+  if (TIER == 1 && (w.skipped & SKIP_TRANS_HUGE))
+    tier_unlaunched<CTR_TRANS_HUGE, CTR_GROW_HUGE, DONE_TRANS_GLOBAL>(w, lane, true);
 }
 
 __device__ __forceinline__ void wave_argmin(float v, int idx, float& bv, int& bi) {
@@ -2841,7 +2877,11 @@
 template <int TIER>
 __global__ __launch_bounds__(TB) void k_route(DevGraph g, DevBatch b, DevParams P, DevWork w) {
   constexpr bool BIG = TIER > 0;
-  if (*w.abort) return;
+  if (*w.abort) {
+    if (TIER == 1 && (w.skipped & SKIP_ROUTE_HUGE))
+      tier_unlaunched<CTR_ROUTE_HUGE, CTR_GROW_HUGE, DONE_ROUTE_GLOBAL>(w, threadIdx.x, true);
+    return;
+  }
   __shared__ uint32_t lkey[BIG ? 1 : LDS_TABLE_CAP];
   __shared__ unsigned long long llab[BIG ? 1 : LDS_TABLE_CAP];
   __shared__ uint32_t linq[BIG ? 1 : LDS_TABLE_CAP];
@@ -2862,6 +2902,7 @@
   const int32_t* list = work.list;
   const int64_t nwork = (int64_t)*work.count;
   if (TIER == 2 && huge_unready(w, nwork, list)) return;
+  bool aborted = false;
   __syncthreads();
   for (int64_t it = blockIdx.x; it < nwork; it += gridDim.x) {
     const int64_t p = (int64_t)list[it];
@@ -2908,6 +2949,7 @@
         if (off + n > w.pool_cap) {
           w.counters_i32[CTR_POOL_OVER] = 1;
           *w.abort = 1;
+          aborted = true;
           w.path_len[p] = -1;
         } else {
           int k = n;
@@ -2927,6 +2969,10 @@
       }
     }
     __syncthreads();
+  }
+  if (TIER == 1 && (w.skipped & SKIP_ROUTE_HUGE)) {
+    if (aborted) __builtin_amdgcn_fence(__ATOMIC_RELEASE, "agent");
+    tier_unlaunched<CTR_ROUTE_HUGE, CTR_GROW_HUGE, DONE_ROUTE_GLOBAL>(w, lane, true);
   }
 }
 
@@ -3863,7 +3909,18 @@
   if (o.pairs.key) report_pair(o, seg_off, seg_cnt, ps, rep);
 }
 
-__global__ __launch_bounds__(256, OTM_REPORT_WAVES) void k_report(DevBatch b, DevReportCfg rc, DevWork w, DevOut o, int32_t n_seg_total) {
+__device__ __forceinline__ void write_status(const DevBatch& b, const DevWork& w, BatchStatus* out) {
+  const int32_t* counters = w.counters_i32;
+  out->abort = *w.abort;
+  out->grow = (counters[CTR_GROW_HUGE] != 0 ? GROW_HUGE : 0) | (counters[CTR_GROW_CAND] != 0 ? GROW_CAND : 0);
+  out->ttotal = w.trans_off[b.n_points];
+  out->pool_used = counters[CTR_POOL_USED];
+  out->pool_over = counters[CTR_POOL_OVER];
+  out->route_huge = counters[CTR_ROUTE_HUGE];
+}
+
+__global__ __launch_bounds__(256, OTM_REPORT_WAVES) void k_report(DevBatch b, DevReportCfg rc, DevWork w, DevOut o, BatchStatus* status) {
+  if (status && blockIdx.x == 0 && threadIdx.x == 0) write_status(b, w, status);
   if (*w.abort) return;
   const int32_t t = blockIdx.x * blockDim.x + threadIdx.x;
   if (t >= b.n_traces) return;
@@ -3885,7 +3942,8 @@
 }
 
 constexpr int REPW_CAP = 64;
-__global__ __launch_bounds__(TB) void k_report_wave(DevBatch b, DevReportCfg rc, DevWork w, DevOut o, int32_t n_seg_total) {
+__global__ __launch_bounds__(TB) void k_report_wave(DevBatch b, DevReportCfg rc, DevWork w, DevOut o, BatchStatus* status) {
+  if (status && blockIdx.x == 0 && threadIdx.x == 0) write_status(b, w, status);
   if (*w.abort) return;
   __shared__ unsigned long long sSeg[REPW_CAP * sizeof(otm_segment) / 8];
   __shared__ int32_t sN;
@@ -4838,11 +4896,11 @@
     mk.end(k, s);        \
   } while (0)
 
-void launch_columns(const DevGraph& g, const DevBatch& b, const DevParams& p, DevWork& w, hipStream_t s,
-                    const Marks& mk) {
+void launch_columns(const DevGraph& g, const DevBatch& b, const DevParams& p, DevWork& w, int64_t* seg_base,
+                    hipStream_t s, const Marks& mk) {
   if (w.ord.tile_cnt) (void)hipMemsetAsync(w.ord.tile_cnt, 0, ORDER_TILES * 4, s);
   TIMED(KN_COLUMNS, hipLaunchKernelGGL(k_columns, dim3(grid_for(b.n_traces, 1, WAVE_GRID_CAP)), dim3(TB), 0, s, g,
-                                       b, p, w));
+                                       b, p, w, seg_base));
 }
 static int order_grid(int64_t n, int per_block, int cap) {
   const int64_t per_group = (n + ORDER_GROUPS - 1) / ORDER_GROUPS;
@@ -4877,7 +4935,8 @@
 #endif
   if (from < RESUME_CAND_BIG)
     hipLaunchKernelGGL(k_candidates<false>, dim3(OTM_CAND_WAVE_GRID), dim3(TB), 0, s, g, b, p, w);
-  hipLaunchKernelGGL(k_candidates<true>, dim3(CAND_BIG_SLOTS), dim3(TB), 0, s, g, b, p, w);
+  if (!(w.skipped & SKIP_CAND_BIG))
+    hipLaunchKernelGGL(k_candidates<true>, dim3(CAND_BIG_SLOTS), dim3(TB), 0, s, g, b, p, w);
   mk.end(KN_CAND_WAVE, s);
 }
 void launch_links(const DevBatch& b, const DevParams& p, DevWork& w, hipStream_t s, const Marks& mk) {
@@ -4902,10 +4961,6 @@
   hipLaunchKernelGGL(k_expand_compact, dim3(grid_for(((int64_t)n_traces + 3) / 4, 1, 1 << 20)), dim3(256), 0, s,
                      trace_off, tbase, dt, acc16, time, acc, n_traces);
 }
-void launch_status(const int32_t* abort, const int64_t* ttotal, const int32_t* counters, BatchStatus* out,
-                   hipStream_t s) {
-  hipLaunchKernelGGL(k_status, dim3(1), dim3(64), 0, s, abort, ttotal, counters, out);
-}
 void launch_transitions(const DevGraph& g, const DevBatch& b, const DevParams& p, DevWork& w, hipStream_t s,
                         const Marks& mk, int sub, int from) {
   if (from >= RESUME_TRANS_HUGE) {
@@ -4927,7 +4982,8 @@
   TIMED(KN_TRANS_WAVE, hipLaunchKernelGGL(k_transitions<0>, dim3(SPILL_GRID), dim3(TB), 0, s, g, b, p, w));
   mk.begin(KN_TRANS_GLOBAL, s);
   hipLaunchKernelGGL(k_transitions<1>, dim3(BIG_SLOTS), dim3(TB), 0, s, g, b, p, w);
-  hipLaunchKernelGGL(k_transitions<2>, dim3(HUGE_SLOTS), dim3(TB), 0, s, g, b, p, w);
+  if (!(w.skipped & SKIP_TRANS_HUGE))
+    hipLaunchKernelGGL(k_transitions<2>, dim3(HUGE_SLOTS), dim3(TB), 0, s, g, b, p, w);
   mk.end(KN_TRANS_GLOBAL, s);
 }
 void launch_viterbi(const DevBatch& b, DevWork& w, hipStream_t s, const Marks& mk) {
@@ -4988,7 +5044,8 @@
   TIMED(KN_ROUTE_WAVE, hipLaunchKernelGGL(k_route<0>, dim3(SPILL_GRID), dim3(TB), 0, s, g, b, p, w));
   mk.begin(KN_ROUTE_GLOBAL, s);
   hipLaunchKernelGGL(k_route<1>, dim3(BIG_SLOTS), dim3(TB), 0, s, g, b, p, w);
-  hipLaunchKernelGGL(k_route<2>, dim3(HUGE_SLOTS), dim3(TB), 0, s, g, b, p, w);
+  if (!(w.skipped & SKIP_ROUTE_HUGE))
+    hipLaunchKernelGGL(k_route<2>, dim3(HUGE_SLOTS), dim3(TB), 0, s, g, b, p, w);
   mk.end(KN_ROUTE_GLOBAL, s);
 }
 void launch_segments(const DevGraph& g, const DevBatch& b, DevWork& w, DevOut& o, hipStream_t s, const Marks& mk) {
@@ -5054,15 +5111,15 @@
   hipLaunchKernelGGL(k_compact, dim3(grid_for(n_traces, 1, WAVE_GRID_CAP)), dim3(TB), 0, s, n_traces, o, seg_off, way_off,
                      rep_off, segs_out, ways_out, reps_out, traces_out);
 }
-void launch_report(const DevBatch& b, const DevReportCfg& rc, DevWork& w, DevOut& o, hipStream_t s,
-                   const Marks& mk) {
+void launch_report(const DevBatch& b, const DevReportCfg& rc, DevWork& w, DevOut& o, BatchStatus* status,
+                   hipStream_t s, const Marks& mk) {
   constexpr int tb = 16;
   if (b.n_traces <= REPW_MAX_TRACES)
     TIMED(KN_REPORT, hipLaunchKernelGGL(k_report_wave, dim3(grid_for(b.n_traces, 1, WAVE_GRID_CAP)), dim3(TB), 0, s,
-                                        b, rc, w, o, 0));
+                                        b, rc, w, o, status));
   else
     TIMED(KN_REPORT, hipLaunchKernelGGL(k_report, dim3(grid_for(b.n_traces, tb, 1 << 30)), dim3(tb), 0, s, b, rc, w,
-                                        o, 0));
+                                        o, status));
 }
 #undef TIMED
 
```

Result: no change. 1.741 billion (median of 4 runs) (+0.4%).
